# mbortolon97/6dgs

Hardware: AMD Instinct MI355X
Metric: poses/sec (higher is better)
Workload: dtype f32

## Files before the change

### 6dgs_amd/_lib.py

```python
from __future__ import annotations

import ctypes as C
import os

_HERE = os.path.dirname(os.path.abspath(__file__))
LIB_PATH = os.path.join(_HERE, "csrc", "lib6dgs_hip.so")
if os.environ.get("SIXDGS_LIB"):
    LIB_PATH = os.path.abspath(os.environ["SIXDGS_LIB"])

vp = C.c_void_p
i64 = C.c_int64
i32 = C.c_int
sz = C.c_size_t


PROFILE_SLOTS = 128
ABI_VERSION = 10


class Profile(C.Structure):
    _fields_ = [("count", i32), ("start", vp * PROFILE_SLOTS), ("stop", vp * PROFILE_SLOTS),
                ("flops", C.c_double * PROFILE_SLOTS), ("bytes", C.c_double * PROFILE_SLOTS)]


class ScorerWeights(C.Structure):
    _fields_ = [(n, vp) for n in ("w1", "b1", "w2", "b2", "w3", "b3", "w4", "b4", "wk", "bk", "wq", "bq", "m1", "m2", "m3", "m4", "mk", "w4k", "b4k", "m4k", "planes")]


SIGNATURES = {
    "sixdgs_abi_version": (i32, []),
    "sixdgs_error_string": (C.c_char_p, [i32]),
    "sixdgs_mask_degraded": (i32, [vp, i64, i32, vp, vp]),
    "sixdgs_sym_eig_3x3": (i32, [vp, i64, vp, vp, vp]),
    "sixdgs_normals_knn": (i32, [vp, i64, vp, i64, i32, vp, vp, vp]),
    "sixdgs_normals_knn_grid_workspace_bytes": (sz, [i64]),
    "sixdgs_normals_knn_grid": (i32, [vp, i64, vp, i64, i32, vp, vp, vp, sz, vp]),
    "sixdgs_emit_quadricell_count": (i32, [vp, vp, i32, vp, vp, i64, vp, i32, i32, vp, vp, vp, vp]),
    "sixdgs_emit_quadricell_write": (i32, [vp, vp, i32, vp, vp, vp, i32, i32, vp, i64, vp, i32, i32, vp, vp, vp, vp, vp, vp]),
    "sixdgs_quadricell_cell_counts": (i32, [vp, i64, i32, vp, vp, vp, vp]),
    "sixdgs_quadricell_centers": (i32, [vp, i64, i32, i32, vp, vp, vp, vp]),
    "sixdgs_isocell_distribution": (i32, [i32, i32, vp, C.POINTER(i64), vp]),
    "sixdgs_rotate_isocell": (i32, [vp, i64, vp, i64, vp, vp]),
    "sixdgs_emit_isocell": (i32, [vp, vp, i32, vp, vp, vp, i32, i32, vp, i64, vp, vp, i64, vp, vp, vp, vp, vp]),
    "sixdgs_eval_sh_color": (i32, [vp, i32, vp, i64, i32, vp, vp]),
    "sixdgs_splat_views_workspace_bytes": (sz, [i64, i32, i32, i32]),
    "sixdgs_splat_views": (i32, [vp, vp, i32, vp, vp, i32, i32, i64, vp, i32, i32, i32, i32, C.c_float, C.c_float, vp, vp, vp, vp, sz, vp]),
    "sixdgs_packed_weights_floats": (sz, []),
    "sixdgs_pack_weights": (i32, [vp] * 13 + [C.POINTER(ScorerWeights), vp]),
    "sixdgs_ray_encode": (i32, [vp, vp, vp, i64, vp, vp]),
    "sixdgs_ray_keys_workspace_bytes": (sz, [i64, i64]),
    "sixdgs_ray_keys": (i32, [vp, vp, vp, i64, C.POINTER(ScorerWeights), vp, vp, vp, sz, vp]),
    "sixdgs_ray_keys_ex": (i32, [vp, vp, vp, i64, C.POINTER(ScorerWeights), vp, vp, vp, vp, vp, vp, sz, vp, C.POINTER(Profile), i32]),
    "sixdgs_key_planes_f16_bytes": (sz, [i64]),
    "sixdgs_split_planes_f16": (i32, [vp, i64, i64, vp, vp, vp]),
    "sixdgs_score_pass1": (i32, [vp, vp, vp, i32, vp, vp, vp, i64, i32, vp, vp, sz, vp, C.POINTER(Profile), i32]),
    "sixdgs_score_pass2": (i32, [vp, vp, i32, i32, i64, i32, vp, vp, vp, vp, sz, vp, i32]),
    "sixdgs_score_backward_workspace_bytes": (sz, [i32]),
    "sixdgs_score_backward": (i32, [vp, vp, i32, vp, i64, vp, vp, vp, vp, vp, sz, vp]),
    "sixdgs_score_backward_split_workspace_bytes": (sz, [i32, i64, i32]),
    "sixdgs_score_backward_split": (i32, [vp, vp, i32, vp, i64, vp, vp, vp, vp, i32, vp, sz, vp]),
    "sixdgs_score_topk_ex": (i32, [vp, vp, vp, i32, vp, vp, vp, i64, i32, vp, vp, vp, vp, vp, sz, vp, C.POINTER(Profile), i32]),
    "sixdgs_score_select_workspace_bytes": (sz, [i64, i32, i32, i32]),
    "sixdgs_score_select": (i32, [vp, vp, vp, i32, vp, vp, vp, i64, vp, vp, i64, i32, i32, vp, vp, vp, vp, sz, vp, C.POINTER(Profile)]),
    "sixdgs_tok_attention": (i32, [vp, i64, i32, i32, i32, vp, i64, vp]),
    "sixdgs_im2col": (i32, [vp, i64, i64, i64, i64, i32, i32, i32, i32, i32, i32, vp, vp]),
    "sixdgs_u8_to_planar": (i32, [vp, i32, i64, vp, vp, vp]),
    "sixdgs_image_prep": (i32, [vp, i32, i32, i32, vp, i32, i32, i32, i32, i32, vp, vp, vp, vp]),
    "sixdgs_tok_pack_bytes": (sz, [i32, i32]),
    "sixdgs_tok_pack": (i32, [vp, i32, i32, i64, vp, vp, vp]),
    "sixdgs_tok_linear": (i32, [vp, i64, i32, i64, i32, vp, vp, C.c_float, vp, vp, vp, i32, i32, vp, i64, vp, vp, i64, vp]),
    "sixdgs_key_planes_norm_max": (i32, [vp, vp, i64, vp, vp]),
    "sixdgs_select_workspace_bytes": (sz, [i64, i32, i32, i32]),
    "sixdgs_select_candidates_workspace_bytes": (sz, [i64, i32, i32, i32]),
    "sixdgs_select_begin": (i32, [vp, vp, vp, i32, vp, vp, i64, i64, vp, vp, vp, sz, vp]),
    "sixdgs_select_sweep_plan": (i32, [vp, i32, vp, vp, i32]),
    "sixdgs_select_sweep": (i32, [vp, vp, vp, i32, vp, vp, i64, vp, vp, vp, i64, vp, vp, sz, vp, C.POINTER(Profile)]),
    "sixdgs_select_candidates": (i32, [vp, i64, i64, vp, vp, vp, i32, vp, vp, vp, i32, i32, vp, vp, vp, sz, vp]),
    "sixdgs_select_rescore": (i32, [vp, vp, i32, vp, vp, i32, vp, vp, vp, vp, i64, i32, i32, i32, vp, vp, vp, vp, sz, vp]),
    "sixdgs_select_sample_stats": (i32, [vp, vp, vp, i32, vp, vp, i64, vp, vp, sz, vp]),
    "sixdgs_select_prepare": (i32, [vp, vp, i32, i64, i64, vp, vp, vp]),
    "sixdgs_select_topk_u": (i32, [vp, i64, i64, vp, i32, i32, vp, vp, sz, vp]),
    "sixdgs_linear_splitk_workspace_bytes": (sz, [i64, i32, i32]),
    "sixdgs_linear_splitk": (i32, [vp, i64, i32, i64, vp, i64, vp, i32, i32, vp, i64, i32, vp, sz, vp, i32]),
    "sixdgs_linear_ex": (i32, [vp, i64, i32, i64, vp, i64, vp, i32, i32, vp, i64, vp, i32]),
    "sixdgs_profile_collect": (i32, [C.POINTER(Profile), C.POINTER(C.c_double), C.POINTER(C.c_double), C.POINTER(C.c_double),
                                    C.POINTER(i32)]),
    "sixdgs_linear": (i32, [vp, i64, i32, i64, vp, i64, vp, i32, i32, vp, i64, vp]),
    "sixdgs_q_proj": (i32, [vp, vp, i32, C.POINTER(ScorerWeights), vp, vp]),
    "sixdgs_score_topk_workspace_bytes": (sz, [i64, i32, i32]),
    "sixdgs_score_topk_workspace_bytes_ex": (sz, [i64, i32, i32, i32, i32]),
    "sixdgs_score_topk": (i32, [vp, vp, i32, vp, i64, i32, vp, vp, vp, vp, vp, sz, vp]),
    "sixdgs_topk_workspace_bytes": (sz, [i64, i32, i32]),
    "sixdgs_topk": (i32, [vp, i64, i32, i32, vp, vp, vp, sz, vp]),
    "sixdgs_distance_target_workspace_bytes": (sz, [i64]),
    "sixdgs_distance_target": (i32, [vp, vp, i64, vp, i32, vp, vp, vp, sz, vp]),
    "sixdgs_solve_pose": (i32, [vp, vp, i64, vp, vp, i32, vp, vp, i32, vp, vp, vp, vp, vp, vp, vp]),
    "sixdgs_solve_pose_consensus_workspace_bytes": (sz, [i32, i32]),
    "sixdgs_solve_pose_consensus": (i32, [vp, vp, i64, vp, vp, i32, vp, vp, i32, C.c_float, i32] + [vp] * 10 + [vp, sz, vp]),
}

_lib = None


def load():
    global _lib
    if _lib is not None:
        return _lib
    import torch

    if not os.path.exists(LIB_PATH):
        raise RuntimeError(
            f"6dgs_amd: {LIB_PATH} is missing -- build it with `python -m 6dgs_amd.build` / __graft_entry__.build(); "
            "there is no CPU fallback for the product path")
    try:
        lib = C.CDLL(LIB_PATH)
    except OSError as e:
        raise RuntimeError(f"6dgs_amd: cannot load {LIB_PATH}: {e}") from e
    for name, (res, args) in SIGNATURES.items():
        try:
            fn = getattr(lib, name)
        except AttributeError as e:
            raise RuntimeError(f"6dgs_amd: {LIB_PATH} does not export {name}") from e
        fn.restype = res
        fn.argtypes = args
    if lib.sixdgs_abi_version() != ABI_VERSION:
        raise RuntimeError(f"6dgs_amd: ABI version mismatch (library {lib.sixdgs_abi_version()}, binding {ABI_VERSION})")
    _lib = lib
    return lib


def check(status: int, what: str = ""):
    if status != 0:
        msg = load().sixdgs_error_string(int(status)).decode()
        raise RuntimeError(f"6dgs_amd: {what or 'call'} failed: {msg} (status {status})")
```

### 6dgs_amd/build.py

```python
from __future__ import annotations

import os
import subprocess
import sys

HERE = os.path.dirname(os.path.abspath(__file__))
CSRC = os.path.join(HERE, "csrc")
LIB = os.path.join(CSRC, "lib6dgs_hip.so")
HOSTCHECK = os.path.join(CSRC, "libsixdgs_hostcheck.so")
SOURCES = ["geometry.hip", "gemm.hip", "dense.hip", "score.hip", "score_bwd.hip", "pose.hip", "pose_consensus.hip", "vit.hip", "splat.hip"]
HEADERS = ["common.h", "device_math.h", "gemm_kernel.h", "dense.h", os.path.join("..", "..", "include", "sixdgs.h"), "dense_layout.h", "sweep_plan.h", "sweep_layout.h"]
HIPCC = os.environ.get("HIPCC", "/opt/rocm/bin/hipcc")
FLAGS = ["--offload-arch=gfx950", "-O3", "-std=c++17", "-fPIC", "-ffp-contract=off", "-Wall", "-Wno-unused-function"]
FLAGS += os.environ.get("SIXDGS_EXTRA_FLAGS", "").split()


def _stale(target, deps):
    if not os.path.exists(target):
        return True
    t = os.path.getmtime(target)
    return any(os.path.getmtime(d) > t for d in deps)


def build(force: bool = False, verbose: bool = False) -> str:
    deps = [os.path.join(CSRC, s) for s in SOURCES + HEADERS]
    if force or _stale(LIB, deps):
        objs = []
        procs = []
        for s in SOURCES:
            o = os.path.join(CSRC, s.replace(".hip", ".o"))
            objs.append(o)
            cmd = [HIPCC, *FLAGS, "-c", os.path.join(CSRC, s), "-o", o]
            if verbose:
                print(" ".join(cmd))
            procs.append((cmd, subprocess.Popen(cmd, stdout=subprocess.PIPE, stderr=subprocess.STDOUT, text=True)))
        for cmd, p in procs:
            out, _ = p.communicate()
            if p.returncode != 0:
                sys.stderr.write(out)
                raise RuntimeError("hipcc failed: " + " ".join(cmd))
            if verbose and out.strip():
                print(out)
        cmd = [HIPCC, "--offload-arch=gfx950", "-shared", "-fPIC", *objs, "-o", LIB]
        subprocess.check_call(cmd)
    return LIB


def build_hostcheck(force: bool = False) -> str:
    src = os.path.join(CSRC, "hostcheck.cpp")
    deps = [src, os.path.join(CSRC, "device_math.h"), os.path.join(CSRC, "dense_layout.h"), os.path.join(CSRC, "sweep_plan.h"),
            os.path.join(CSRC, "sweep_layout.h")]
    if force or _stale(HOSTCHECK, deps):
        cmd = [HIPCC, "-x", "hip", "--offload-arch=gfx950", "-O2", "-std=c++17", "-fPIC", "-ffp-contract=off", "-shared", src,
               "-o", HOSTCHECK]
        subprocess.check_call(cmd)
    return HOSTCHECK


if __name__ == "__main__":
    print(build(force="--force" in sys.argv, verbose=True))
    print(build_hostcheck(force="--force" in sys.argv))
```

### 6dgs_amd/csrc/hostcheck.cpp

```cpp
#include <stdlib.h>

#include "device_math.h"
#include "sweep_plan.h"
#include "dense_layout.h"
#include "sweep_layout.h"
using namespace sdg;

extern "C" {

void hc_mask_degraded(const float* scale, long long n, int P, unsigned char* mask) {
  for (long long i = 0; i < n; ++i) {
    float side;
    mask[i] = total_rings(scale[3 * i], scale[3 * i + 1], scale[3 * i + 2], (float)P, &side) < (long long)P;
  }
}

long long hc_quadricell_centers(const float* scale, long long E, int P, int res, float* points, long long* eid) {
  long long C = 0;
  float* table = (float*)malloc(sizeof(float) * res);
  for (long long e = 0; e < E; ++e) {
    float a = scale[3 * e], b = scale[3 * e + 1], c = scale[3 * e + 2], side;
    long long rings = total_rings(a, b, c, (float)P, &side);
    for (long long ring = 0; ring < rings; ++ring) {
      Ring rg = ring_params(a, b, c, side, (float)rings, (float)ring);
      int npts = ring_cells(rg);
      if (!npts) continue;
      if (points) {
        double acc = 0.0;
        table[0] = 0.f;
        for (int j = 0; j < res - 1; ++j) { acc += (double)ring_table_increment(rg, j); table[j + 1] = (float)acc; }
        float last = table[res - 1];
        for (int j = 0; j < res; ++j) table[j] = kTwoPi * (table[j] / last);
        for (int j = 0; j < npts; ++j) {
          int pick = ring_table_pick(table, res, (float)j * rg.dtheta);
          V3 p = ring_point(rg, table[pick]);
          points[3 * (C + j)] = p.x; points[3 * (C + j) + 1] = p.y; points[3 * (C + j) + 2] = p.z;
          eid[C + j] = e;
        }
      }
      C += npts;
    }
  }
  free(table);
  return C;
}

long long hc_emit_rays(const float* points, const long long* eid, long long C, const float* normals, const float* centers,
                       const float* rot4, float* ori, float* dir, long long* mid) {
  long long r = 0;
  for (long long i = 0; i < C; ++i) {
    long long e = eid[i];
    float R[9];
    quat_to_rotmat(rot4 + 4 * e, R);
    V3 pw = rotate(R, v3(points[3 * i], points[3 * i + 1], points[3 * i + 2]));
    if (!hemisphere_keep(normals[3 * e], pw)) continue;
    V3 d = normalize_eps(pw);
    ori[3 * r] = pw.x + centers[3 * e]; ori[3 * r + 1] = pw.y + centers[3 * e + 1]; ori[3 * r + 2] = pw.z + centers[3 * e + 2];
    dir[3 * r] = d.x; dir[3 * r + 1] = d.y; dir[3 * r + 2] = d.z;
    mid[r++] = e;
  }
  return r;
}

void hc_sym_eig(const float* mats, long long n, float* vals, float* vecs) {
  for (long long i = 0; i < n; ++i) sym_eig_3x3(mats + 9 * i, vals + 3 * i, vecs ? vecs + 9 * i : nullptr);
}

void hc_normals_from_knn(const float* cloud, const long long* knn, long long nq, int k, float* normals) {
  float* nb = (float*)malloc(sizeof(float) * 3 * k);
  for (long long q = 0; q < nq; ++q) {
    for (int j = 0; j < k; ++j)
      for (int c = 0; c < 3; ++c) nb[3 * j + c] = cloud[3 * knn[q * k + j] + c];
    V3 n = normal_from_neighbours(nb, k);
    normals[3 * q] = n.x; normals[3 * q + 1] = n.y; normals[3 * q + 2] = n.z;
  }
  free(nb);
}

long long hc_isocell_dirs(int target, int n0, float* dirs) {
  int n = isocell_rings(target, n0);
  long long o = 0;
  for (int ring = 1; ring <= n; ++ring)
    for (int j = 0; j < n0 * (2 * ring - 1); ++j, ++o)
      if (dirs) { V3 d = isocell_dir(n, n0, ring, j); dirs[3 * o] = d.x; dirs[3 * o + 1] = d.y; dirs[3 * o + 2] = d.z; }
  return o;
}

void hc_rotate_isocell(const float* dirs, long long K, const float* normals, long long E, float* out) {
  for (long long e = 0; e < E; ++e) {
    float Rm[9];
    isocell_rotation(v3(normals[3 * e], normals[3 * e + 1], normals[3 * e + 2]), Rm);
    for (long long k = 0; k < K; ++k) {
      V3 d = isocell_apply(Rm, v3(dirs[3 * k], dirs[3 * k + 1], dirs[3 * k + 2]));
      float* o = out + 3 * (e * K + k);
      o[0] = d.x; o[1] = d.y; o[2] = d.z;
    }
  }
}

void hc_sh_color(const float* sh, int ncoef, const float* dirs, long long R, int deg, float* rgb) {
  for (long long i = 0; i < R; ++i)
    for (int ch = 0; ch < 3; ++ch)
      rgb[3 * i + ch] = sh_channel(sh + (3 * i + ch) * ncoef, 1, deg, -dirs[3 * i], -dirs[3 * i + 1], -dirs[3 * i + 2]);
}

void hc_ray_input(const float* ori, const float* dir, const float* rgb, long long R, float* x) {
  for (long long i = 0; i < R; ++i)
    for (int c = 0; c < 144; ++c) x[144 * i + c] = ray_input_element(ori + 3 * i, dir + 3 * i, rgb + 3 * i, c);
}

void hc_make_rotation_mat(const float* d, const float* up, float* Rm) { make_rotation_mat(v3(d[0], d[1], d[2]), v3(up[0], up[1], up[2]), Rm); }

int hc_solve_centre(const float* Rm, const float* q, float* c) { return solve_centre(Rm, q, c) ? 1 : 0; }

void hc_pose_errors(const float* gt, const float* pr, float* out2) { pose_errors(gt, pr, out2, out2 + 1); }

void hc_distance_target(const float* pose, const float* ori, const float* dir, long long r, float* out) {
  for (long long i = 0; i < r; ++i)
    out[i] = distance_target(pose, v3(ori[3 * i], ori[3 * i + 1], ori[3 * i + 2]), v3(dir[3 * i], dir[3 * i + 1], dir[3 * i + 2]));
}

int hc_dl_row_perm(int m) { return dl::row_perm(m); }
int hc_dl_acc_row(int lane, int r) { return dl::acc_row(lane, r); }
int hc_dl_acc_feature(int permuted, int lane, int r) { return dl::acc_feature(permuted != 0, lane, r); }
long long hc_dl_plane_offset(int chunk_major, long long ray, int nslab, int slab, int plane, int c) {
  return chunk_major ? dl::cm_offset(ray, nslab, slab, plane, c) : dl::rm_offset(ray, nslab, slab, plane, c);
}
unsigned hc_dl_lds_offset(unsigned row, unsigned plane, unsigned c) { return dl::lds_offset(row, plane, c); }
unsigned hc_dl_frag_offset(unsigned row0, unsigned lane, unsigned ks, unsigned plane) { return dl::frag_offset(row0, lane, ks, plane); }
unsigned hc_dl_load_ray(int chunk_major, unsigned tid, unsigned jp) { return dl::load_ray(chunk_major != 0, tid, jp); }
unsigned hc_dl_load_chunk8(int chunk_major, unsigned tid) { return dl::load_chunk8(chunk_major != 0, tid); }
unsigned hc_dl_cm_src_offset(unsigned ray_in_tile, unsigned chunk8, unsigned granule_stride) {
  return dl::cm_src_offset(ray_in_tile, chunk8 * (unsigned)dl::kChunkRun, granule_stride);
}
int hc_sweep_launch_images(int left, int cap) { return sdg::sweep_launch_images(left, cap); }
int hc_sweep_pack_ints() { return 2 + 2 * sdg::kSweepMaxSlots * sdg::kSlotQuarters + (2 + sdg::kSlotQuarters) * sdg::kSweepMaxLaunchImages; }
int hc_sweep_max_slots() { return sdg::kSweepMaxSlots; }
int hc_sweep_pack(const int* h_n_tok, int batch, int cap, int* out, int max_launches) {
  const std::vector<sdg::SweepSlots> plan = sdg::sweep_pack(h_n_tok, batch, cap);
  const int per = hc_sweep_pack_ints();
  for (size_t l = 0; l < plan.size() && (int)l < max_launches; ++l) {
    const sdg::SweepSlots& t = plan[l];
    int* o = out + (size_t)l * per;
    *o++ = t.n_slots;
    *o++ = t.n_images;
    for (int s = 0; s < sdg::kSweepMaxSlots; ++s)
      for (int w = 0; w < sdg::kSlotQuarters; ++w) *o++ = t.q_img[s][w];
    for (int s = 0; s < sdg::kSweepMaxSlots; ++s)
      for (int w = 0; w < sdg::kSlotQuarters; ++w) *o++ = t.q_lq[s][w];
    for (int i = 0; i < sdg::kSweepMaxLaunchImages; ++i) *o++ = t.img[i];
    for (int i = 0; i < sdg::kSweepMaxLaunchImages; ++i) *o++ = t.img_nq[i];
    for (int i = 0; i < sdg::kSweepMaxLaunchImages; ++i)
      for (int w = 0; w < sdg::kSlotQuarters; ++w) *o++ = t.img_q[i][w];
  }
  return (int)plan.size();
}
int hc_sw_const(int which) {
  const int v[] = {sw::kTokBlocks, sw::kRayBlocks, sw::kBlockBytes, sw::kBflySteps};
  return which >= 0 && which < 4 ? v[which] : -1;
}
int hc_sw_frag_row(int lane) { return sw::frag_row(lane); }
int hc_sw_frag_chunk(int lane, int plane) { return sw::frag_chunk(lane, plane); }
unsigned hc_sw_frag_offset(int row0, int lane, int plane) { return sw::frag_offset(row0, lane, plane); }
int hc_sw_acc_token(int lane, int tb) { return sw::acc_token(lane, tb); }
int hc_sw_acc_ray(int lane, int rb, int reg) { return sw::acc_ray(lane, rb, reg); }
int hc_sw_bfly_partner(int lane, int step) { return sw::bfly_partner(lane, step); }
int hc_sw_bfly_keeps(int lane, int step, int i) { return sw::bfly_keeps(lane, step, i) ? 1 : 0; }
int hc_sw_out_index(int lane, int x) { return sw::out_index(lane, x); }
int hc_sw_out_ray(int lane, int x) { return sw::out_ray(lane, x); }
int hc_sw_part_writes(int lane) { return sw::part_writes(lane) ? 1 : 0; }
int hc_sw_part_row(int wn, int lane) { return sw::part_row(wn, lane); }
int hc_dl_const(int which) {
  const int v[] = {dl::kSlabB, dl::kPRow, dl::kGran, dl::kGranSlab, dl::kChunkRun};
  return which >= 0 && which < 5 ? v[which] : -1;
}

}
```

### 6dgs_amd/csrc/score.hip

```cpp
#include <stdlib.h>

#include <cstdlib>
#include <cstdio>
#include "gemm_kernel.h"
#include "sweep_plan.h"
#include "sweep_layout.h"

using namespace sdg;

namespace {

constexpr int kT = SIXDGS_MAX_TOKENS;
constexpr float kSqrtD = 19.595917942265423f;

struct LogitsArgs {
  const float* q;
  const int* n_tok;
  const float* key;
  float* logits;
  float* partial;
  int64_t r, ldl;
  int tiles_per_group, n_tiles, n_groups;
  int b0;
};

template <int MMA>
__global__ void __launch_bounds__(256, 2) k_logits(LogitsArgs A) {
  __shared__ __attribute__((aligned(16))) char smem[TileSmem<MMA>::kBytes];
  __shared__ float part[2][128][2];
  const int bl = blockIdx.y;
  const int b = A.b0 + bl;
  const unsigned w = xcd_remap(blockIdx.x, gridDim.x);
  const int grp = (int)(w >> 1), m_tile = (int)(w & 1u);
  const int M = A.n_tok[b];
  const int row0 = m_tile * 128;
  float* pout = A.partial + (((int64_t)bl * A.n_groups + grp) * kT + row0) * 2;
  const int tid = threadIdx.x, lane = tid & 63, wave = tid >> 6;
  const int wm = wave >> 1, wn = wave & 1;
  float m_run = -INFINITY, s_run = 0.f;
  if (row0 < M) {
    GemmOperands g = {A.q + (int64_t)b * kT * SIXDGS_D, nullptr, A.key, SIXDGS_D, 0, SIXDGS_D, M, A.r, SIXDGS_D, SIXDGS_D};
    float* lg = A.logits + (int64_t)bl * kT * A.ldl;
    const int t_begin = grp * A.tiles_per_group;
    const int t_end = min(t_begin + A.tiles_per_group, A.n_tiles);
    for (int tile = t_begin; tile < t_end; ++tile) {
      const int64_t col0 = (int64_t)tile * kBN;
      f32x16 acc[2][2];
      gemm_tile<MMA>(g, row0, col0, smem, acc);
      const int64_t c0 = col0 + acc_col(wn, 0, lane), c1 = col0 + acc_col(wn, 1, lane);
      const bool v0 = c0 < A.r, v1 = c1 < A.r;
#pragma unroll
      for (int tm = 0; tm < 2; ++tm)
#pragma unroll
        for (int r = 0; r < 16; ++r) {
          const int row = row0 + acc_row(wm, tm, r, lane);
          const float l0 = acc[tm][0][r] / kSqrtD, l1 = acc[tm][1][r] / kSqrtD;
          if (row < M) {
            if (v0) lg[(int64_t)row * A.ldl + c0] = l0;
            if (v1) lg[(int64_t)row * A.ldl + c1] = l1;
          }
          float mx = fmaxf(v0 ? l0 : -INFINITY, v1 ? l1 : -INFINITY);
#pragma unroll
          for (int o = 16; o > 0; o >>= 1) mx = fmaxf(mx, __shfl_xor(mx, o, 64));
          float sm = 0.f;
          if (mx > -INFINITY) sm = (v0 ? expf(l0 - mx) : 0.f) + (v1 ? expf(l1 - mx) : 0.f);
#pragma unroll
          for (int o = 16; o > 0; o >>= 1) sm += __shfl_xor(sm, o, 64);
          if ((lane & 31) == 0) {
            const int lr = acc_row(wm, tm, r, lane);
            part[wn][lr][0] = mx;
            part[wn][lr][1] = sm;
          }
        }
      __syncthreads();
      if (tid < 128) {
#pragma unroll
        for (int h = 0; h < 2; ++h) {
          const float mt = part[h][tid][0], st = part[h][tid][1];
          if (mt > -INFINITY) {
            const float mn = fmaxf(m_run, mt);
            s_run = s_run * expf(m_run - mn) + st * expf(mt - mn);
            m_run = mn;
          }
        }
      }
    }
  }
  if (tid < 128) {
    pout[2 * tid] = m_run;
    pout[2 * tid + 1] = s_run;
  }
}

typedef __attribute__((address_space(3))) void* lds_ptr_t;
typedef const __attribute__((address_space(1))) void* gbl_ptr_t;
constexpr int kRowBytes = 12 * 3 * 64;
constexpr float kInvSqrtD = 0.05103103630798288f;

typedef _Float16 f16x8 __attribute__((ext_vector_type(8)));
constexpr int kRowF = 12 * 2 * 64;
constexpr int kSlabF = 128;

struct LogitsF16Args {
  const char* qp;
  const int* n_tok;
  const char* kp;
  const float* qinv;
  const float* kinv;
  float* logits;
  float* partial;
  int64_t r, ldl;
  int tiles_per_group, n_tiles, n_groups, b0, nb;
  const float* ctok;
  float* ub;
  int64_t ub_stride;
  int n_sets;
  unsigned* sib_sync;
  int sib_period;
  unsigned sib_extra;
  int q_quarter_scales;
};
constexpr int kOutF32 = 0;
constexpr int kOutL24 = 1;
constexpr int kOutStats = 2;
constexpr int kOutUB = 3;
constexpr int kAllTerms = 3;
constexpr int kOneTerm = 1;

__device__ __forceinline__ float load_uniform(const float* p) {
  return *reinterpret_cast<const __attribute__((address_space(4))) float*>((uintptr_t)p);
}

__device__ __forceinline__ f16x8 lds_read_frag_h_off(unsigned addr, const int imm) {
  f16x8 v;
  asm volatile("ds_read_b128 %0, %1 offset:%2" : "=v"(v) : "v"(addr), "n"(imm));
  return v;
}

constexpr int kBNX = 256;
constexpr int kSiblingSyncDefault = 1;
constexpr int kSibSpinLimit = 1 << 14;
constexpr unsigned kSibReleased = 0x40000000u;
constexpr int kSweepMaxImages = 8;
constexpr bool kPrepassOneTermDefault = true;
constexpr int kPrepassReserveCusOneSlot = 160;
constexpr int kPrepassReserveCus = 64;
constexpr int kSibPeriod = 1;
constexpr int kTileBytes24 = 98304 + 2048;
constexpr int kQStageX = 256 * 64;
constexpr int kKBaseX = 4 * kQStageX;
constexpr int kLdsX = kKBaseX + 6 * kQStageX;

constexpr int kMfma32 = 0;
constexpr int kMfma16 = 1;

template <int TERMS, int OUT, bool PERS = false, int SHAPE = kMfma32>
__global__ void __launch_bounds__(512, 1) k_logits_f16x(LogitsF16Args A) {
  static_assert(TERMS == kAllTerms || TERMS == kOneTerm, "k_logits_f16x: TERMS is 3 or 1");
  static_assert(SHAPE == kMfma32 || (SHAPE == kMfma16 && OUT == kOutUB && TERMS == kAllTerms), "k_logits_f16x: 16x16x32 is the select sweep's shape");
// ... 412 lines not shown
              const f32x2 uu = e0 + e1;
              u[r] = uu.x;
              u[r + 1] = uu.y;
            }
            float v8[8], v4[4], v2[2];
#pragma unroll
            for (int i = 0; i < 8; ++i) {
              const float keep = lb0 ? u[i + 8] : u[i], send = lb0 ? u[i] : u[i + 8];
              v8[i] = keep + __builtin_bit_cast(float, __builtin_amdgcn_mov_dpp(__builtin_bit_cast(int, send), 0xB1, 0xF, 0xF, true));
            }
#pragma unroll
            for (int i = 0; i < 4; ++i) {
              const float keep = lb1 ? v8[i + 4] : v8[i], send = lb1 ? v8[i] : v8[i + 4];
              v4[i] = keep + __builtin_bit_cast(float, __builtin_amdgcn_mov_dpp(__builtin_bit_cast(int, send), 0x4E, 0xF, 0xF, true));
            }
#pragma unroll
            for (int i = 0; i < 2; ++i) {
              const float keep = lb2 ? v4[i + 2] : v4[i], send = lb2 ? v4[i] : v4[i + 2];
              v2[i] = keep + __builtin_bit_cast(float, __builtin_amdgcn_ds_swizzle(__builtin_bit_cast(int, send), 0x101F));
            }
            {
              const float keep = lb3 ? v2[1] : v2[0], send = lb3 ? v2[0] : v2[1];
              fin[tn] = keep + __builtin_bit_cast(float, __builtin_amdgcn_ds_swizzle(__builtin_bit_cast(int, send), 0x201F));
            }
          }
          float o[2];
#pragma unroll
          for (int x = 0; x < 2; ++x) {
            const float keep = lb4 ? fin[2 + x] : fin[x], send = lb4 ? fin[x] : fin[2 + x];
            o[x] = keep + __builtin_bit_cast(float, __builtin_amdgcn_ds_swizzle(__builtin_bit_cast(int, send), 0x401F));
          }
          const int rrev = ((lane & 1) << 3) | ((lane & 2) << 1) | ((lane & 4) >> 1) | ((lane & 8) >> 3);
          const int inhalf = ((lane & 16) << 2) + 8 * (rrev >> 2) + 4 * (lane >> 5) + (rrev & 3);
          float* up = A.ub + ((int64_t)bl * 4 + wm) * A.ub_stride + ((int64_t)tile * kBNX + wn * 128 + inhalf);
          __builtin_nontemporal_store(o[0], up);
          __builtin_nontemporal_store(o[1], up + 32);
        }
      } else if (active) {
        const int t128 = min(2 * tile + wn, n_tiles128 - 1);
        const float cf = (cq * load_uniform(A.kinv + t128)) * kInvSqrtD;
        float* tb = lg + (int64_t)(2 * tile + wn) * (kT * 128);
        const bool ragged = lim_cur < kBNX - 1;
#pragma unroll
        for (int tm = 0; tm < 2; ++tm) {
          float mx = -INFINITY;
#pragma unroll
          for (int tn = 0; tn < 4; ++tn)
#pragma unroll
            for (int rg = 0; rg < 4; ++rg) {
              float4 v;
              v.x = acc[tm][tn][4 * rg + 0] * cf;
              v.y = acc[tm][tn][4 * rg + 1] * cf;
              v.z = acc[tm][tn][4 * rg + 2] * cf;
              v.w = acc[tm][tn][4 * rg + 3] * cf;
              acc[tm][tn][4 * rg + 0] = v.x;
              acc[tm][tn][4 * rg + 1] = v.y;
              acc[tm][tn][4 * rg + 2] = v.z;
              acc[tm][tn][4 * rg + 3] = v.w;
              if (OUT == kOutF32) {
                typedef float f32x4 __attribute__((ext_vector_type(4)));
                __builtin_nontemporal_store(f32x4{v.x, v.y, v.z, v.w}, reinterpret_cast<f32x4*>(tb + tm * 4096 + tn * 1024 + rg * 256));
              }
              mx = fmaxf(mx, fmaxf(fmaxf(v.x, v.y), fmaxf(v.z, v.w)));
            }
          if (L24) {
            typedef unsigned u32x3 __attribute__((ext_vector_type(3)));
            char* t24 = lg24 + (int64_t)(2 * tile + wn) * kTileBytes24 + ((wm * 2 + tm) * 12288 + lane * 12);
#pragma unroll
            for (int tn = 0; tn < 4; ++tn)
#pragma unroll
              for (int rg = 0; rg < 4; ++rg) {
                unsigned d[4];
#pragma unroll
                for (int j = 0; j < 4; ++j)
                  d[j] = (unsigned)__float2uint_rn(fminf((mx - acc[tm][tn][4 * rg + j]) * 524288.f, 16777215.f));
                const u32x3 w3 = {d[0] | (d[1] << 24), (d[1] >> 8) | (d[2] << 16), (d[2] >> 16) | (d[3] << 8)};
                __builtin_nontemporal_store(w3, reinterpret_cast<u32x3*>(t24 + (tn * 8 + 2 * rg) * 384));
                __builtin_amdgcn_sched_barrier(0);
              }
            reinterpret_cast<float*>(lg24 + (int64_t)(2 * tile + wn) * kTileBytes24 + 98304)[((wm * 2 + tm) * 2 + (lane >> 5)) * 32 + (lane & 31)] = mx;
          }
          const float mn = fmaxf(m_run[tm], mx);
          float sum[4] = {0.f, 0.f, 0.f, 0.f};
          if (!ragged) {
#pragma unroll
            for (int tn = 0; tn < 4; ++tn)
#pragma unroll
              for (int r = 0; r < 16; ++r) sum[r & 3] += __expf(acc[tm][tn][r] - mn);
          } else {
            int ray0 = wn * 128 + 4 * (lane >> 5);
            asm volatile("" : "+v"(ray0));
#pragma unroll
            for (int tn = 0; tn < 4; ++tn)
#pragma unroll
              for (int r = 0; r < 16; ++r)
                sum[r & 3] += (ray0 + tn * 32 + 8 * (r >> 2) + (r & 3) <= lim_cur) ? __expf(acc[tm][tn][r] - mn) : 0.f;
          }
          s_run[tm] = s_run[tm] * __expf(m_run[tm] - mn) + ((sum[0] + sum[1]) + (sum[2] + sum[3]));
          m_run[tm] = mn;
        }
      }
      kcur = knext;
      lim_cur = lim_next;
    }
    asm volatile("s_waitcnt vmcnt(0)" ::: "memory");
  }
  __syncthreads();
  float(*part)[256][2] = reinterpret_cast<float(*)[256][2]>(lds);
  if (S16) {
    int lm = lane;
    if (PERS) asm volatile("" : "+v"(lm));
#pragma unroll
    for (int tb = 0; tb < sw::kTokBlocks; ++tb) {
      float z = zs16[tb];
      z += __builtin_bit_cast(float, __builtin_amdgcn_ds_swizzle(__builtin_bit_cast(int, z), 0x401F));
      if (sw::part_writes(lm)) {
        float* pp = part[sw::part_row(wn, lm)][wm * 64 + sw::acc_token(lm, tb)];
        pp[0] = 0.f;
        pp[1] = z;
      }
    }
  } else {
#pragma unroll
  for (int tm = 0; tm < 2; ++tm) {
    float* pp = part[wn * 2 + (lane >> 5)][wm * 64 + tm * 32 + (lane & 31)];
    if (OUT == kOutUB) {
      pp[0] = 0.f;
      pp[1] = (zs[tm][0].x + zs[tm][0].y) + (zs[tm][1].x + zs[tm][1].y);
    } else {
      pp[0] = m_run[tm];
      pp[1] = s_run[tm];
    }
  }
  }
  __syncthreads();
  if (tid < 256) {
    float m = -INFINITY, sres = 0.f;
#pragma unroll
    for (int h = 0; h < 4; ++h) {
      const float mt = part[h][tid][0], st2 = part[h][tid][1];
      if (mt > -INFINITY) {
        const float mn = fmaxf(m, mt);
        sres = sres * __expf(m - mn) + st2 * __expf(mt - mn);
        m = mn;
      }
    }
    pout[2 * tid] = m;
    pout[2 * tid + 1] = sres;
  }
  if (PERS) __syncthreads();
  } while (PERS && (grp += A.n_sets) < A.n_groups);
}

__global__ void __launch_bounds__(256) k_split_tiles_f16(const float* __restrict__ src, int64_t rows, int64_t ld, char* __restrict__ dst,
                                                         float* __restrict__ inv_scale) {
  __shared__ float wmax[4];
  const int64_t row0 = (int64_t)blockIdx.x * 128;
  const int n = (int)min((int64_t)128, rows - row0);
  const float* base = src + row0 * ld;
  float m = 0.f;
  for (int i = threadIdx.x; i < n * 96; i += 256) {
    const int row = i / 96;
    const float4 v = *reinterpret_cast<const float4*>(base + (int64_t)row * ld + (i - row * 96) * 4);
    m = fmaxf(m, fmaxf(fmaxf(fabsf(v.x), fabsf(v.y)), fmaxf(fabsf(v.z), fabsf(v.w))));
  }
  m = sdg_wave_max(m);
  if (sdg_lane() == 0) wmax[sdg_wave()] = m;
  __syncthreads();
  m = fmaxf(fmaxf(wmax[0], wmax[1]), fmaxf(wmax[2], wmax[3]));
  int sh = 0;
  if (m > 0.f && m < INFINITY) {
    int e;
    frexpf(m, &e);
    sh = 14 - e;
    sh = sh > 100 ? 100 : (sh < -100 ? -100 : sh);
  }
  const float sc = ldexpf(1.f, sh);
  if (threadIdx.x == 0) inv_scale[blockIdx.x] = ldexpf(1.f, -sh);
  for (int i = threadIdx.x; i < n * 48; i += 256) {
    const int row = i / 48, k8 = i - row * 48;
    const float* sp = base + (int64_t)row * ld + k8 * 8;
    const float4 lo = *reinterpret_cast<const float4*>(sp);
    const float4 hi = *reinterpret_cast<const float4*>(sp + 4);
    const float x[8] = {lo.x * sc, lo.y * sc, lo.z * sc, lo.w * sc, hi.x * sc, hi.y * sc, hi.z * sc, hi.w * sc};
    f16x8 h, l;
#pragma unroll
    for (int e = 0; e < 8; ++e) {
      const _Float16 hh = (_Float16)x[e];
      h[e] = hh;
      l[e] = (_Float16)(x[e] - (float)hh);
    }
    char* d = dst + (row0 + row) * kRowF + (k8 >> 2) * kSlabF + (k8 & 3) * 16;
    *reinterpret_cast<f16x8*>(d) = h;
    *reinterpret_cast<f16x8*>(d + 64) = l;
  }
}


__global__ void __launch_bounds__(1024) k_merge_stats(const float* __restrict__ partial, int n_groups, float* __restrict__ stats) {
  __shared__ float sm[16][64][2];
  const int bl = blockIdx.x, tl = threadIdx.x & 63, j = threadIdx.x >> 6, t = blockIdx.y * 64 + tl;
  const float* p = partial + (int64_t)bl * n_groups * kT * 2;
  float m = -INFINITY, s = 0.f;
  for (int g = j; g < n_groups; g += 16) {
    const float mt = p[((int64_t)g * kT + t) * 2], st = p[((int64_t)g * kT + t) * 2 + 1];
    if (mt > -INFINITY) {
      const float mn = fmaxf(m, mt);
      s = s * expf(m - mn) + st * expf(mt - mn);
      m = mn;
    }
  }
  sm[j][tl][0] = m;
  sm[j][tl][1] = s;
  __syncthreads();
  if (j == 0) {
    m = -INFINITY;
    s = 0.f;
#pragma unroll
    for (int q = 0; q < 16; ++q) {
      const float mt = sm[q][tl][0], st = sm[q][tl][1];
      if (mt > -INFINITY) {
        const float mn = fmaxf(m, mt);
        s = s * expf(m - mn) + st * expf(mt - mn);
        m = mn;
      }
    }
    stats[((int64_t)bl * kT + t) * 2] = m;
    stats[((int64_t)bl * kT + t) * 2 + 1] = s;
  }
}

__global__ void __launch_bounds__(256) k_score_reduce(const float* __restrict__ logits, int64_t ldl, const float* __restrict__ stats,
                                                       const int* __restrict__ n_tok, int b0, int64_t R, float* __restrict__ scores,
                                                       int64_t score_stride) {
  __shared__ float st[kT][2];
  const int bl = blockIdx.y;
  const int T = n_tok[b0 + bl];
  for (int i = threadIdx.x; i < kT * 2; i += blockDim.x) {
    const float v = stats[(int64_t)bl * kT * 2 + i];
    (&st[0][0])[i] = (i & 1) ? 1.f / v : v;
  }
  __syncthreads();
  const int64_t j = (int64_t)blockIdx.x * blockDim.x + threadIdx.x;
  if (j >= R) return;
  const float* l = logits + (int64_t)bl * kT * ldl + j;
  float s = 0.f;
#pragma unroll 8
  for (int t = 0; t < T; ++t) s += __expf(l[(int64_t)t * ldl] - st[t][0]) * st[t][1];
  scores[(int64_t)bl * score_stride + j] = s;
}

#define FASTEXP(x) __expf(x)
__global__ void __launch_bounds__(256) k_score_reduce_blocked(const float* __restrict__ logits, int64_t ldl, const float* __restrict__ stats,
                                                               const int* __restrict__ n_tok, int b0, int64_t R,
                                                               float* __restrict__ scores, int64_t score_stride) {
  const int bl = blockIdx.y;
  const int T = n_tok[b0 + bl];
  const int lane = threadIdx.x & 63, wave = threadIdx.x >> 6, l31 = lane & 31;
  float mt[8], st[8];
#pragma unroll
  for (int g = 0; g < 8; ++g) {
    const int t = g * 32 + l31;
    mt[g] = stats[((int64_t)bl * kT + t) * 2];
    st[g] = 1.f / stats[((int64_t)bl * kT + t) * 2 + 1];
  }
  const int64_t tile = blockIdx.x;
  const float* tb = logits + (int64_t)bl * kT * ldl + tile * (kT * kBN) + lane * 4;
  float* out = scores + (int64_t)bl * score_stride + tile * kBN;
#pragma unroll
  for (int u = 0; u < 4; ++u) {
    const int p = u * 4 + wave;
    float4 acc = {0.f, 0.f, 0.f, 0.f};
#pragma unroll
    for (int g = 0; g < 8; ++g)
      if (g * 32 + l31 < T) {
        const float4 v = *reinterpret_cast<const float4*>(tb + g * 4096 + p * 256);
        acc.x += FASTEXP(v.x - mt[g]) * st[g];
        acc.y += FASTEXP(v.y - mt[g]) * st[g];
        acc.z += FASTEXP(v.z - mt[g]) * st[g];
        acc.w += FASTEXP(v.w - mt[g]) * st[g];
      }
#pragma unroll
    for (int o = 16; o > 0; o >>= 1) {
      acc.x += __shfl_xor(acc.x, o, 64);
      acc.y += __shfl_xor(acc.y, o, 64);
      acc.z += __shfl_xor(acc.z, o, 64);
      acc.w += __shfl_xor(acc.w, o, 64);
    }
    if (l31 == 0) {
      const int64_t r0 = tile * kBN + p * 8 + (lane >> 5) * 4;
      float* o4 = out + p * 8 + (lane >> 5) * 4;
      if (r0 + 3 < R && ((uintptr_t)o4 & 15) == 0) *reinterpret_cast<float4*>(o4) = acc;
      else {
        if (r0 < R) o4[0] = acc.x;
        if (r0 + 1 < R) o4[1] = acc.y;
        if (r0 + 2 < R) o4[2] = acc.z;
        if (r0 + 3 < R) o4[3] = acc.w;
      }
    }
  }
}

__global__ void __launch_bounds__(256) k_score_reduce_blocked24(const float* __restrict__ logits, int64_t ldl, const float* __restrict__ stats,
                                                               const int* __restrict__ n_tok, int b0, int64_t R,
                                                               float* __restrict__ scores, int64_t score_stride) {
  const int bl = blockIdx.y;
// ... 67 lines not shown
  unsigned remain;
};
__device__ SelectState select_state(const unsigned* hist , int passes, unsigned k, unsigned* sm ) {
  SelectState st = {0u, k};
  for (int p = 0; p < passes; ++p) {
    __syncthreads();
    for (int i = threadIdx.x; i < 256; i += blockDim.x) sm[i] = hist[p * 256 + i];
    __syncthreads();
    unsigned acc = 0, digit = 0, rem = st.remain;
    for (int d = 255; d >= 0; --d) {
      const unsigned c = sm[d];
      if (acc + c >= st.remain) { digit = (unsigned)d; rem = st.remain - acc; break; }
      acc += c;
    }
    st.prefix |= digit << (24 - 8 * p);
    st.remain = rem;
  }
  return st;
}

template <int PASS>
__global__ void __launch_bounds__(256) k_topk_hist(const float* __restrict__ scores, int64_t stride, int64_t R, unsigned k,
                                                    unsigned* __restrict__ hist_all, const int* __restrict__ only) {
  __shared__ unsigned sm[256];
  __shared__ unsigned lh[256];
  const int b = blockIdx.y;
  if (only != nullptr && only[b] == 0) return;
  unsigned* hist = hist_all + (int64_t)b * 4 * 256;
  const SelectState st = select_state(hist, PASS, k, sm);
  for (int i = threadIdx.x; i < 256; i += blockDim.x) lh[i] = 0;
  __syncthreads();
  const float* s = scores + (int64_t)b * stride;
  constexpr unsigned hi_mask = PASS == 0 ? 0u : (0xffffffffu << (32 - 8 * PASS));
  constexpr int shift = 24 - 8 * PASS;
  for (int64_t i = (int64_t)blockIdx.x * blockDim.x + threadIdx.x; i < R; i += (int64_t)gridDim.x * blockDim.x) {
    const unsigned key = score_key(s[i]);
    if ((key & hi_mask) == st.prefix) atomicAdd(&lh[(key >> shift) & 255u], 1u);
  }
  __syncthreads();
  for (int i = threadIdx.x; i < 256; i += blockDim.x)
    if (lh[i]) atomicAdd(&hist[PASS * 256 + i], lh[i]);
}

template <bool WRITE>
__global__ void __launch_bounds__(256) k_topk_gather(const float* __restrict__ scores, int64_t stride, int64_t R, unsigned k,
                                                      const unsigned* __restrict__ hist_all, int64_t span,
                                                      unsigned* __restrict__ counts ,
                                                      const unsigned* __restrict__ offs ,
                                                      unsigned* __restrict__ cand_key, int64_t* __restrict__ cand_idx, int topk,
                                                      const int* __restrict__ only) {
  __shared__ unsigned sm[256];
  __shared__ int sc[2][5];
  const int b = blockIdx.y;
  if (only != nullptr && only[b] == 0) return;
  const SelectState st = select_state(hist_all + (int64_t)b * 4 * 256, 4, k, sm);
  const unsigned thr = st.prefix;
  const float* s = scores + (int64_t)b * stride;
  const int64_t i0 = (int64_t)blockIdx.x * span, i1 = min(i0 + span, R);
  unsigned run_g = 0, run_e = 0;
  unsigned base_g = 0, base_e = 0, n_greater = 0;
  if (WRITE) {
    base_g = offs[((int64_t)b * gridDim.x + blockIdx.x) * 2];
    base_e = offs[((int64_t)b * gridDim.x + blockIdx.x) * 2 + 1];
    n_greater = k - st.remain;
  }
  for (int64_t c0 = i0; c0 < i1; c0 += 256) {
    const int64_t i = c0 + threadIdx.x;
    unsigned key = 0;
    bool gt = false, eq = false;
    if (i < i1) {
      key = score_key(s[i]);
      gt = key > thr;
      eq = key == thr;
    }
    const unsigned long long bg = __ballot(gt), be = __ballot(eq);
    const int lane = sdg_lane(), wv = sdg_wave();
    if (lane == 0) { sc[0][wv] = __popcll(bg); sc[1][wv] = __popcll(be); }
    __syncthreads();
    unsigned og = 0, oe = 0, tg = 0, te = 0;
    for (int w2 = 0; w2 < 4; ++w2) {
      if (w2 < wv) { og += sc[0][w2]; oe += sc[1][w2]; }
      tg += sc[0][w2];
      te += sc[1][w2];
    }
    __syncthreads();
    if (WRITE) {
      const unsigned long long below = (1ull << lane) - 1ull;
      if (gt) {
        const unsigned pos = base_g + run_g + og + __popcll(bg & below);
        if (pos < (unsigned)topk) { cand_key[(int64_t)b * topk + pos] = key; cand_idx[(int64_t)b * topk + pos] = i; }
      } else if (eq) {
        const unsigned re = base_e + run_e + oe + __popcll(be & below);
        if (re < st.remain) {
          const unsigned pos = n_greater + re;
          if (pos < (unsigned)topk) { cand_key[(int64_t)b * topk + pos] = key; cand_idx[(int64_t)b * topk + pos] = i; }
        }
      }
    }
    run_g += tg;
    run_e += te;
  }
  if (!WRITE && threadIdx.x == 0) {
    counts[((int64_t)b * gridDim.x + blockIdx.x) * 2] = run_g;
    counts[((int64_t)b * gridDim.x + blockIdx.x) * 2 + 1] = run_e;
  }
}

__global__ void __launch_bounds__(1024) k_topk_scan(const unsigned* __restrict__ counts, int nb, unsigned* __restrict__ offs, const int* __restrict__ only) {
  __shared__ unsigned sm[17];
  const int b = blockIdx.x;
  if (only != nullptr && only[b] == 0) return;
  for (int comp = 0; comp < 2; ++comp) {
    unsigned base = 0;
    for (int c0 = 0; c0 < nb; c0 += 1024) {
      const int i = c0 + threadIdx.x;
      const unsigned v = i < nb ? counts[((int64_t)b * nb + i) * 2 + comp] : 0u;
      unsigned tot;
      const unsigned ex = sdg_block_exclusive_scan<unsigned, 16>(v, sm, &tot);
      if (i < nb) offs[((int64_t)b * nb + i) * 2 + comp] = base + ex;
      base += tot;
    }
  }
}

__global__ void __launch_bounds__(1024) k_topk_sort(const unsigned* __restrict__ cand_key, const int64_t* __restrict__ cand_idx,
                                                     int topk, int k_eff, int64_t* __restrict__ idx, float* __restrict__ val, const int* __restrict__ only) {
  __shared__ unsigned sk[1024];
  __shared__ long long si[1024];
  const int b = blockIdx.x, t = threadIdx.x;
  if (only != nullptr && only[b] == 0) return;
  if (t < k_eff) { sk[t] = cand_key[(int64_t)b * topk + t]; si[t] = cand_idx[(int64_t)b * topk + t]; }
  else { sk[t] = 0u; si[t] = 0x7fffffffffffffffll; }
  __syncthreads();
  for (int size = 2; size <= 1024; size <<= 1)
    for (int strd = size >> 1; strd > 0; strd >>= 1) {
      const int p = t ^ strd;
      if (p > t) {
        const bool up = (t & size) == 0;
        const unsigned ka = sk[t], kb = sk[p];
        const long long ia = si[t], ib = si[p];
        const bool a_first = ka > kb || (ka == kb && ia < ib);
        if (up ? !a_first : a_first) { sk[t] = kb; sk[p] = ka; si[t] = ib; si[p] = ia; }
      }
      __syncthreads();
    }
  if (t < topk) {
    if (t < k_eff) { idx[(int64_t)b * topk + t] = si[t]; val[(int64_t)b * topk + t] = key_score(sk[t]); }
    else { idx[(int64_t)b * topk + t] = -1; val[(int64_t)b * topk + t] = NAN; }
  }
}

constexpr float kLog2e = 1.4426950408889634f;

__global__ void __launch_bounds__(kT) k_sel_prepare(const float* __restrict__ stats_s, const int* __restrict__ n_tok, int b0, float log2_frac,
                                                    float* __restrict__ ctok) {
  const int bl = blockIdx.x, t = threadIdx.x;
  const float m = stats_s[((int64_t)bl * kT + t) * 2], z = stats_s[((int64_t)bl * kT + t) * 2 + 1];
  const bool ok = t < n_tok[b0 + bl] && z > 0.f && m > -INFINITY && m < INFINITY;
  ctok[(int64_t)bl * kT + t] = ok ? -(m * kLog2e) - (log2f(z) + log2_frac) : -INFINITY;
}

__global__ void __launch_bounds__(256) k_split_q_slots(const float* __restrict__ q, const int* __restrict__ n_tok, const SweepSlots T, char* __restrict__ dst,
                                                       float* __restrict__ inv_scale, const float* __restrict__ ctok, float* __restrict__ ctok_slot,
                                                       int* __restrict__ slot_rows) {
  __shared__ float wmax[4];
  const int slot = blockIdx.x >> 2, w = blockIdx.x & 3;
  const int img = T.q_img[slot][w], lq = T.q_lq[slot][w];
  const int n = img < 0 ? 0 : min(64, max(0, n_tok[img] - 64 * lq));
  const float* base = q + ((int64_t)(img < 0 ? 0 : img) * kT + 64 * (lq < 0 ? 0 : lq)) * SIXDGS_D;
  float m = 0.f;
  for (int i = threadIdx.x; i < n * 96; i += 256) {
    const float4 v = *reinterpret_cast<const float4*>(base + (int64_t)i * 4);
    m = fmaxf(m, fmaxf(fmaxf(fabsf(v.x), fabsf(v.y)), fmaxf(fabsf(v.z), fabsf(v.w))));
  }
  m = sdg_wave_max(m);
  if (sdg_lane() == 0) wmax[sdg_wave()] = m;
  __syncthreads();
  m = fmaxf(fmaxf(wmax[0], wmax[1]), fmaxf(wmax[2], wmax[3]));
  int sh = 0;
  if (m > 0.f && m < INFINITY) {
    int e;
    frexpf(m, &e);
    sh = 14 - e;
    sh = sh > 100 ? 100 : (sh < -100 ? -100 : sh);
  }
  const float sc = ldexpf(1.f, sh);
  if (threadIdx.x == 0) inv_scale[blockIdx.x] = ldexpf(1.f, -sh);
  char* const drow = dst + ((int64_t)slot * kT + 64 * w) * kRowF;
  for (int i = threadIdx.x; i < 64 * 48; i += 256) {
    const int row = i / 48, k8 = i - row * 48;
    f16x8 h, l;
    if (row < n) {
      const float* sp = base + (int64_t)row * SIXDGS_D + k8 * 8;
      const float4 lo = *reinterpret_cast<const float4*>(sp);
      const float4 hi = *reinterpret_cast<const float4*>(sp + 4);
      const float x[8] = {lo.x * sc, lo.y * sc, lo.z * sc, lo.w * sc, hi.x * sc, hi.y * sc, hi.z * sc, hi.w * sc};
#pragma unroll
      for (int e = 0; e < 8; ++e) {
        const _Float16 hh = (_Float16)x[e];
        h[e] = hh;
        l[e] = (_Float16)(x[e] - (float)hh);
      }
    } else {
#pragma unroll
      for (int e = 0; e < 8; ++e) h[e] = l[e] = (_Float16)0.f;
    }
    char* d = drow + (int64_t)row * kRowF + (k8 >> 2) * kSlabF + (k8 & 3) * 16;
    *reinterpret_cast<f16x8*>(d) = h;
    *reinterpret_cast<f16x8*>(d + 64) = l;
  }
  if (ctok_slot != nullptr && threadIdx.x < 64) {
    const int t = threadIdx.x;
    ctok_slot[(int64_t)slot * kT + 64 * w + t] = t < n ? ctok[(int64_t)img * kT + 64 * lq + t] : -INFINITY;
  }
  if (w == 0 && threadIdx.x == 0) {
    int rows = 0;
    for (int x = 0; x < kSlotQuarters; ++x) {
      const int im = T.q_img[slot][x];
      const int nx = im < 0 ? 0 : min(64, max(0, n_tok[im] - 64 * T.q_lq[slot][x]));
      if (nx > 0) rows = 64 * x + nx;
    }
    slot_rows[slot] = rows;
  }
}

__global__ void __launch_bounds__(1024) k_merge_stats_slots(const float* __restrict__ partial, int n_groups, const SweepSlots T, float* __restrict__ stats,
                                                            float* __restrict__ gsum) {
  __shared__ float sm[16][64][2];
  const int k = blockIdx.x, y = blockIdx.y, tl = threadIdx.x & 63, j = threadIdx.x >> 6;
  const int img = T.img[k], sq = y < T.img_nq[k] ? T.img_q[k][y] : -1;
  float m = -INFINITY, s = 0.f;
  if (sq >= 0) {
    const float* p = partial + (int64_t)(sq >> 2) * n_groups * kT * 2;
    const int row = 64 * (sq & 3) + tl;
    for (int g = j; g < n_groups; g += 16) {
      const float mt = p[((int64_t)g * kT + row) * 2], st = p[((int64_t)g * kT + row) * 2 + 1];
      if (mt > -INFINITY) {
        const float mn = fmaxf(m, mt);
        s = s * expf(m - mn) + st * expf(mt - mn);
        m = mn;
      }
    }
  }
  sm[j][tl][0] = m;
  sm[j][tl][1] = s;
  __syncthreads();
  if (j == 0) {
    m = -INFINITY;
    s = 0.f;
#pragma unroll
    for (int qd = 0; qd < 16; ++qd) {
      const float mt = sm[qd][tl][0], st = sm[qd][tl][1];
      if (mt > -INFINITY) {
        const float mn = fmaxf(m, mt);
        s = s * expf(m - mn) + st * expf(mt - mn);
        m = mn;
      }
    }
    const int64_t o = (int64_t)img * kT + 64 * y + tl;
    if (gsum != nullptr) {
      gsum[o] += s;
    } else {
      stats[o * 2] = m;
      stats[o * 2 + 1] = s;
    }
  }
}

__global__ void __launch_bounds__(256) k_sel_finish_slots(const float* __restrict__ ub, int64_t stride, int64_t u_stride, const int* __restrict__ n_tok, const SweepSlots T,
                                                          int64_t R, float* __restrict__ U, float* __restrict__ tmax, int64_t tmax_stride) {
  const int k = blockIdx.y, img = T.img[k];
  const int nq_dev = (min(max(n_tok[img], 0), kT) + 63) >> 6;
  const int nq = min(nq_dev, (int)T.img_nq[k]);
  const int64_t i = ((int64_t)blockIdx.x * blockDim.x + threadIdx.x) * 4;
  float m = -INFINITY;
  if (i < R) {
    float4 a = {0.f, 0.f, 0.f, 0.f};
    const int64_t row[kSlotQuarters] = {T.img_q[k][0], T.img_q[k][1], T.img_q[k][2], T.img_q[k][3]};
#pragma unroll
    for (int y = 0; y < kSlotQuarters; ++y)
      if (y < nq) {
        const float4 v = *reinterpret_cast<const float4*>(ub + row[y] * stride + i);
        a.x += v.x; a.y += v.y; a.z += v.z; a.w += v.w;
      }
    *reinterpret_cast<float4*>(U + (int64_t)img * u_stride + i) = a;
    m = a.x;
    if (i + 1 < R) m = fmaxf(m, a.y);
    if (i + 2 < R) m = fmaxf(m, a.z);
    if (i + 3 < R) m = fmaxf(m, a.w);
  }
  if (tmax != nullptr) {
    m = sdg_wave_max(m);
    const int64_t tile = (i - 4 * sdg_lane()) >> 8;
    if (sdg_lane() == 0 && tile * 256 < R) tmax[(int64_t)img * tmax_stride + tile] = m;
  }
}

__global__ void __launch_bounds__(256) k_plane_norm_max(const char* __restrict__ planes, const float* __restrict__ inv_scale, int64_t rows,
                                                        unsigned* __restrict__ out) {
  const int lane = sdg_lane();
  const int64_t wave0 = (int64_t)blockIdx.x * 4 + sdg_wave(), nw = (int64_t)gridDim.x * 4;
  float best = 0.f;
  for (int64_t row = wave0; row < rows; row += nw) {
    float ss = 0.f;
    if (lane < 48) {
      const char* p = planes + row * kRowF + (lane >> 2) * kSlabF + (lane & 3) * 16;
      const f16x8 h = *reinterpret_cast<const f16x8*>(p), l = *reinterpret_cast<const f16x8*>(p + 64);
#pragma unroll
      for (int e = 0; e < 8; ++e) {
        const float x = (float)h[e] + (float)l[e];
        ss = __builtin_fmaf(x, x, ss);
      }
    }
    ss = sdg_wave_sum(ss);
    best = fmaxf(best, sqrtf(ss) * inv_scale[row >> 7]);
  }
  if (lane == 0 && best > 0.f) atomicMax(out, __float_as_uint(best * 1.000244140625f));
}

constexpr float kEpsPerX = 1.4e-4f, kEpsConst = 1.3e-5f;
__global__ void __launch_bounds__(kT) k_sel_bounds(const float* __restrict__ gsum, const int* __restrict__ n_tok, const float* __restrict__ valU,
                                                   const float* __restrict__ q, const float* __restrict__ key_norm_max, int topk, int k_eff,
                                                   float* __restrict__ info, const int* __restrict__ only) {
  __shared__ float smin[4], smax[4], sq[4];
  const int bl = blockIdx.x, t = threadIdx.x, M = n_tok[bl];
  if (only != nullptr && only[bl] == 0) return;
  const float g = gsum[(int64_t)bl * kT + t];
  float lo = t < M ? g : INFINITY, hi = t < M ? g : -INFINITY;
  bool bad = t < M && !(g > 0.f && g < INFINITY);
  float qn = 0.f;
  if (t < M) {
    const float4* qr = reinterpret_cast<const float4*>(q + ((int64_t)bl * kT + t) * SIXDGS_D);
    float ss = 0.f;
    for (int i = 0; i < SIXDGS_D / 4; ++i) {
      const float4 v = qr[i];
      ss = __builtin_fmaf(v.x, v.x, ss); ss = __builtin_fmaf(v.y, v.y, ss); ss = __builtin_fmaf(v.z, v.z, ss); ss = __builtin_fmaf(v.w, v.w, ss);
    }
    qn = sqrtf(ss) * 1.000244140625f;
  }
#pragma unroll
  for (int o = 32; o > 0; o >>= 1) {
    lo = fminf(lo, __shfl_xor(lo, o, 64));
    hi = fmaxf(hi, __shfl_xor(hi, o, 64));
    qn = fmaxf(qn, __shfl_xor(qn, o, 64));
  }
  const unsigned long long anybad = __ballot(bad);
  if (sdg_lane() == 0) { smin[sdg_wave()] = anybad ? NAN : lo; smax[sdg_wave()] = hi; sq[sdg_wave()] = qn; }
  __syncthreads();
  if (t == 0) {
    float flag = 0.f, thr = INFINITY, eps = 0.f, x = 0.f;
    if (M <= 0) flag = 1.f;
    else {
      float a = smin[0], b = smax[0], qm = sq[0];
      bool nan = a != a;
      for (int w = 1; w < 4; ++w) { nan = nan || smin[w] != smin[w]; a = fminf(a, smin[w]); b = fmaxf(b, smax[w]); qm = fmaxf(qm, sq[w]); }
      const float uk = valU[(int64_t)bl * topk + (k_eff - 1)];
      x = qm * key_norm_max[0] * kInvSqrtD * 1.0000002f;
      eps = x * kEpsPerX + kEpsConst;
      if (nan || !(uk >= 0.f && uk < INFINITY) || !(a > 0.f) || !(eps < 0.25f)) flag = 2.f;
      else thr = (uk * (a / b)) * ((1.f - eps) / (1.f + eps)) * 0.9999998f;
    }
    info[bl * 4 + 0] = thr;
    info[bl * 4 + 1] = flag;
    info[bl * 4 + 2] = eps;
    info[bl * 4 + 3] = x;
  }
}

__global__ void k_sel_need_exact(const int* __restrict__ total, const float* __restrict__ info, int nb, int cmax, int* __restrict__ need) {
  const int bl = blockIdx.x * blockDim.x + threadIdx.x;
  if (bl >= nb) return;
  need[bl] = (info[bl * 4 + 1] == 0.f && total[bl] > cmax) ? 1 : 0;
}

__global__ void k_sel_count(const int* __restrict__ total, const float* __restrict__ info, int nb, int* __restrict__ d_count) {
  const int bl = blockIdx.x * blockDim.x + threadIdx.x;
  if (bl >= nb) return;
  const float flag = info[bl * 4 + 1];
  d_count[bl] = flag == 1.f ? -2 : (flag != 0.f ? -1 : total[bl]);
}

template <bool WRITE>
__global__ void __launch_bounds__(256) k_sel_candidates(const float* __restrict__ U, int64_t stride, int64_t R, const float* __restrict__ info,
                                                        int64_t span, unsigned* __restrict__ counts, const unsigned* __restrict__ offs,
                                                        int64_t* __restrict__ cand, int cmax, const int* __restrict__ only,
                                                        const float* __restrict__ tmax_all) {
  __shared__ int sc[4];
  const int bl = blockIdx.y;
  if (only != nullptr && only[bl] == 0) return;
  const float thr = info[bl * 4 + 0];
  const float* u = U + (int64_t)bl * stride;
  const float* tmax = tmax_all ? tmax_all + (int64_t)bl * (stride >> 8) : nullptr;
  const int64_t i0 = (int64_t)blockIdx.x * span, i1 = min(i0 + span, R);
  unsigned run = 0;
  const unsigned base = WRITE ? offs[(int64_t)bl * gridDim.x + blockIdx.x] : 0u;
  for (int64_t c0 = i0; c0 < i1; c0 += 256) {
    if (tmax != nullptr && !(tmax[c0 >> 8] >= thr)) continue;
    const int64_t i = c0 + threadIdx.x;
    const bool in = i < i1 && u[i] >= thr;
    const unsigned long long bm = __ballot(in);
    const int lane = sdg_lane(), wv = sdg_wave();
    if (lane == 0) sc[wv] = __popcll(bm);
    __syncthreads();
    unsigned before = 0, tot = 0;
    for (int w2 = 0; w2 < 4; ++w2) {
      if (w2 < wv) before += sc[w2];
      tot += sc[w2];
    }
    __syncthreads();
    if (WRITE && in) {
      const unsigned pos = base + run + before + __popcll(bm & ((1ull << lane) - 1ull));
      if (pos < (unsigned)cmax) cand[(int64_t)bl * cmax + pos] = i;
    }
    run += tot;
  }
  if (!WRITE && threadIdx.x == 0) counts[(int64_t)bl * gridDim.x + blockIdx.x] = run;
}
// ... 539 lines not shown
  }
  prof->count = 0;
  if (ms_total) *ms_total = ms;
  if (flops_total) *flops_total = fl;
  if (bytes_total) *bytes_total = by;
  if (launches) *launches = n;
  return rc;
}

}

namespace {
struct SelectPlan {
  int64_t stride;
  int nbc;
  int64_t span;
  size_t o_partial, o_stats, o_qpl, o_ub, o_idxu, o_valu, o_lidx, o_lval, o_info, o_counts, o_offs, o_total, o_cscore, o_slot, per_image, topk_bytes;
};
SelectPlan select_plan(int64_t r, int batch, int topk, int cmax, bool with_ub = true) {
  SelectPlan p;
  p.stride = sdg_cdiv(r > 0 ? r : 1, 256) * 256;
  const TopkPlan tp = topk_plan(r, batch, topk);
  p.nbc = tp.nb;
  p.span = tp.span;
  size_t o = 0;
  auto take = [&](size_t bytes) { const size_t at = o; o += sdg_align(bytes); return at; };
  p.o_partial = take((size_t)1024 * kT * 2 * sizeof(float));
  p.o_stats = take((size_t)kT * 2 * sizeof(float));
  p.o_qpl = take(sdg_align((size_t)kT * kRowF, 1024) + 256);
  p.o_ub = take(with_ub ? (size_t)4 * p.stride * sizeof(float) : 16);
  p.o_idxu = take((size_t)topk * sizeof(int64_t));
  p.o_valu = take((size_t)topk * sizeof(float));
  p.o_lidx = take((size_t)topk * sizeof(int64_t));
  p.o_lval = take((size_t)topk * sizeof(float));
  p.o_info = take(16);
  p.o_counts = take((size_t)p.nbc * sizeof(unsigned));
  p.o_offs = take((size_t)p.nbc * sizeof(unsigned));
  p.o_total = take(16);
  p.o_cscore = take((size_t)cmax * sizeof(float));
  p.o_slot = take((size_t)kT * sizeof(float) + 256);
  p.per_image = o;
  const size_t t2 = topk_plan(cmax, batch, topk).bytes;
  p.topk_bytes = tp.bytes > t2 ? tp.bytes : t2;
  return p;
}
struct SelectWs {
  SelectPlan p;
  char *topk_ws, *qplanes;
  float *partial, *stats, *qinv, *ub, *valU, *lval, *info, *cscore, *ctok_slot;
  int* slot_rows;
  int64_t *idxU, *lidx;
  unsigned *counts, *offs;
  int* total;
  size_t qpl_img;
};
bool select_ws(void* ws, size_t ws_bytes, int64_t r, int nb, int topk, int cmax, SelectWs* w, bool with_ub = true) {
  w->p = select_plan(r, nb, topk, cmax, with_ub);
  if (w->p.topk_bytes + (size_t)nb * w->p.per_image > ws_bytes) return false;
  w->topk_ws = (char*)ws;
  char* img0 = (char*)ws + w->p.topk_bytes;
  auto field = [&](size_t off) { return img0 + off * (size_t)nb; };
  w->partial = (float*)field(w->p.o_partial);
  w->stats = (float*)field(w->p.o_stats);
  w->qplanes = field(w->p.o_qpl);
  w->qpl_img = sdg_align((size_t)kT * kRowF, 1024);
  w->qinv = (float*)(w->qplanes + (size_t)nb * w->qpl_img);
  w->ub = (float*)field(w->p.o_ub);
  w->idxU = (int64_t*)field(w->p.o_idxu);
  w->valU = (float*)field(w->p.o_valu);
  w->lidx = (int64_t*)field(w->p.o_lidx);
  w->lval = (float*)field(w->p.o_lval);
  w->info = (float*)field(w->p.o_info);
  w->counts = (unsigned*)field(w->p.o_counts);
  w->offs = (unsigned*)field(w->p.o_offs);
  w->total = (int*)field(w->p.o_total);
  w->cscore = (float*)field(w->p.o_cscore);
  w->ctok_slot = (float*)field(w->p.o_slot);
  w->slot_rows = (int*)(field(w->p.o_slot) + (size_t)nb * kT * sizeof(float));
  return true;
}

int f16x_groups(int64_t r) {
  const int n_tiles_x = (int)sdg_cdiv(r > 0 ? r : 1, kBNX);
  int g = 1024;
  while (g > 256 && n_tiles_x / g < 16) g -= 256;
  if (g > n_tiles_x) g = n_tiles_x;
  return g;
}

int sibling_sync_mode() {
  static int mode = -1;
  if (mode < 0) {
    const char* e = getenv("SIXDGS_SIBLING_SYNC");
    mode = e ? atoi(e) : kSiblingSyncDefault;
  }
  return mode;
}
bool sweep_mfma16() {
  const char* e = getenv("SIXDGS_SWEEP_MFMA");
  return !(e && atoi(e) == 32);
}
int sibling_sync_cus() {
  static int cus = -1;
  if (cus < 0) {
    const bool on = sibling_sync_mode() != 0;
    int dev = 0;
    hipDeviceProp_t prop;
    cus = (on && hipGetDevice(&dev) == hipSuccess && hipGetDeviceProperties(&prop, dev) == hipSuccess && prop.multiProcessorCount > 0) ? prop.multiProcessorCount : 0;
  }
  return cus;
}

void select_q_planes(const float* q, int nb, const SelectWs& w, hipStream_t s) {
  hipLaunchKernelGGL(k_split_tiles_f16, dim3((unsigned)(2 * nb)), dim3(256), 0, s, q, (int64_t)nb * kT, (int64_t)SIXDGS_D, w.qplanes, w.qinv);
}
LogitsF16Args select_args(const int32_t* d_n_tok, int nb, const SelectWs& w, const void* planes, const float* scale, int64_t r) {
  LogitsF16Args V = {w.qplanes, d_n_tok, (const char*)planes, w.qinv, scale, nullptr, w.partial, r, w.p.stride, 0, 0, 0, 0, nb, nullptr, nullptr, 0};
  V.n_tiles = (int)sdg_cdiv(r, kBNX);
  V.n_groups = f16x_groups(r);
  V.tiles_per_group = (int)sdg_cdiv(V.n_tiles, V.n_groups);
  return V;
}
}

extern "C" {

size_t sixdgs_select_workspace_bytes(int64_t r, int batch, int topk, int max_candidates) {
  if (batch < 1) batch = 1;
  const SelectPlan p = select_plan(r, batch, topk, max_candidates);
  return p.topk_bytes + (size_t)batch * p.per_image;
}

size_t sixdgs_select_candidates_workspace_bytes(int64_t r, int batch, int topk, int max_candidates) {
  if (batch < 1) batch = 1;
  const SelectPlan p = select_plan(r, batch, topk, max_candidates, false);
  return p.topk_bytes + (size_t)batch * p.per_image;
}

static int sweep_slot_cap() {
  static const int cap = [] {
    const char* e = getenv("SIXDGS_SWEEP_MAX_IMAGES");
    const int v = e ? atoi(e) : kSweepMaxImages;
    if (e && v <= 0) fprintf(stderr, "6dgs_amd: SIXDGS_SWEEP_MAX_IMAGES=%s: launches of %d slots (the slot table's limit), a last one of up to %d -- not one launch per batch\n", e, kSweepMaxSlots * 2 / 3, kSweepMaxSlots * 2 / 3 + kSweepMaxSlots / 3);
    return v;
  }();
  return cap;
}

static bool prepass_one_term(int ) {
  static const int forced = [] { const char* e = getenv("SIXDGS_PREPASS_TERMS"); return e ? atoi(e) : 0; }();
  return forced == 1 || (forced != 3 && kPrepassOneTermDefault);
}

int sixdgs_select_sweep_plan(const int32_t* h_n_tok, int batch, int32_t* slots_per_launch, int32_t* images_per_launch, int max_launches) {
  if (batch < 0 || batch > 32767 || max_launches < 0 || (max_launches > 0 && (!slots_per_launch || !images_per_launch))) return SIXDGS_E_BADARG;
  const std::vector<SweepSlots> plan = sweep_pack(h_n_tok, batch, sweep_slot_cap());
  for (size_t l = 0; l < plan.size() && (int)l < max_launches; ++l) {
    slots_per_launch[l] = plan[l].n_slots;
    images_per_launch[l] = plan[l].n_images;
  }
  return (int)plan.size();
}

int sixdgs_select_sample_stats(const float* q, const int32_t* d_n_tok, const int32_t* h_n_tok, int batch, const void* sample_planes,
                               const float* d_sample_scale, int64_t r_sample, float* row_stats, void* ws, size_t ws_bytes, sixdgs_stream_t stream) {
  SDG_CHECK_ARG(batch >= 0 && batch <= 32767 && r_sample >= 1);
  if (batch == 0) return 0;
  SDG_CHECK_ARG(q && d_n_tok && sample_planes && d_sample_scale && row_stats && ws && ((uintptr_t)sample_planes % 16) == 0 &&
                ((uintptr_t)q % 16) == 0 && ((uintptr_t)ws % 256) == 0);
  hipStream_t s = sdg_stream(stream);
  SelectWs w;
  if (!select_ws(ws, ws_bytes, r_sample, batch, 1, 8, &w)) return SIXDGS_E_WORKSPACE;
  const int n_groups = f16x_groups(r_sample);
  for (const SweepSlots& T : sweep_pack(h_n_tok, batch, sweep_slot_cap())) {
    if (T.n_slots > 0) {
      hipLaunchKernelGGL(k_split_q_slots, dim3((unsigned)(4 * T.n_slots)), dim3(256), 0, s, q, d_n_tok, T, w.qplanes, w.qinv, (const float*)nullptr,
                         (float*)nullptr, w.slot_rows);
      LogitsF16Args V = select_args(w.slot_rows, T.n_slots, w, sample_planes, d_sample_scale, r_sample);
      V.q_quarter_scales = 1;
      static const int reserve_env = [] { const char* e = getenv("SIXDGS_PREPASS_RESERVE_CUS"); return e ? atoi(e) : -2; }();
      const int reserve = reserve_env != -2 ? reserve_env : (T.n_slots == 1 ? kPrepassReserveCusOneSlot : kPrepassReserveCus);
      const int cus = sibling_sync_cus();
      if (reserve >= 0 && cus > reserve && (cus - reserve) / T.n_slots >= 1) {
        V.n_sets = (cus - reserve) / T.n_slots < V.n_groups ? (cus - reserve) / T.n_slots : V.n_groups;
        V.sib_sync = nullptr;
        V.sib_extra = 0u;
        V.sib_period = kSibPeriod;
        if (prepass_one_term(T.n_slots)) hipLaunchKernelGGL((k_logits_f16x<kOneTerm, kOutStats, true>), dim3((unsigned)(V.n_sets * T.n_slots)), dim3(512), 0, s, V);
        else hipLaunchKernelGGL((k_logits_f16x<kAllTerms, kOutStats, true>), dim3((unsigned)(V.n_sets * T.n_slots)), dim3(512), 0, s, V);
      } else {
        if (prepass_one_term(T.n_slots)) hipLaunchKernelGGL((k_logits_f16x<kOneTerm, kOutStats>), dim3((unsigned)(V.n_groups * T.n_slots)), dim3(512), 0, s, V);
        else hipLaunchKernelGGL((k_logits_f16x<kAllTerms, kOutStats>), dim3((unsigned)(V.n_groups * T.n_slots)), dim3(512), 0, s, V);
      }
    }
    hipLaunchKernelGGL(k_merge_stats_slots, dim3((unsigned)T.n_images, 4), dim3(1024), 0, s, w.partial, n_groups, T, row_stats, (float*)nullptr);
  }
  SDG_LAUNCH_OK();
  return 0;
}

int sixdgs_select_prepare(const float* row_stats, const int32_t* d_n_tok, int batch, int64_t r_sample, int64_t r_total, float* ctok, float* gsum,
                          sixdgs_stream_t stream) {
  SDG_CHECK_ARG(batch >= 0 && r_sample >= 1 && r_total >= r_sample);
  if (batch == 0) return 0;
  SDG_CHECK_ARG(row_stats && d_n_tok && ctok && gsum);
  hipStream_t s = sdg_stream(stream);
  hipLaunchKernelGGL(k_sel_prepare, dim3((unsigned)batch), dim3(kT), 0, s, row_stats, d_n_tok, 0, log2f((float)((double)r_total / (double)r_sample)), ctok);
  hipError_t e = hipMemsetAsync(gsum, 0, (size_t)batch * kT * sizeof(float), s);
  if (e != hipSuccess) return (int)e;
  SDG_LAUNCH_OK();
  return 0;
}

int sixdgs_select_begin(const float* q, const int32_t* d_n_tok, const int32_t* h_n_tok, int batch, const void* sample_planes, const float* d_sample_scale,
                        int64_t r_sample, int64_t r_total, float* ctok, float* gsum, void* ws, size_t ws_bytes, sixdgs_stream_t stream) {
  SDG_CHECK_ARG(batch >= 0 && r_sample >= 1 && r_total >= r_sample);
  if (batch == 0) return 0;
  SDG_CHECK_ARG(ws && ((uintptr_t)ws % 256) == 0);
  SelectWs w;
  if (!select_ws(ws, ws_bytes, r_sample, batch, 1, 8, &w)) return SIXDGS_E_WORKSPACE;
  const int st = sixdgs_select_sample_stats(q, d_n_tok, h_n_tok, batch, sample_planes, d_sample_scale, r_sample, w.stats, ws, ws_bytes, stream);
  if (st) return st;
  return sixdgs_select_prepare(w.stats, d_n_tok, batch, r_sample, r_total, ctok, gsum, stream);
}

int sixdgs_select_sweep(const float* q, const int32_t* d_n_tok, const int32_t* h_n_tok, int batch, const void* key_planes,
                        const float* d_key_scale, int64_t r, const float* ctok, float* gsum, float* u, int64_t u_stride, float* u_tile_max,
                        void* ws, size_t ws_bytes, sixdgs_stream_t stream, sixdgs_profile* prof) {
  SDG_CHECK_ARG(batch >= 0 && batch <= 32767 && r >= 1 && u_stride >= sdg_cdiv(r, 256) * 256 && (u_stride % 4) == 0 && (!u_tile_max || (u_stride % 256) == 0));
  if (batch == 0) return 0;
  SDG_CHECK_ARG(q && d_n_tok && key_planes && d_key_scale && ctok && gsum && u && ws && ((uintptr_t)key_planes % 16) == 0 &&
                ((uintptr_t)q % 16) == 0 && ((uintptr_t)u % 16) == 0 && ((uintptr_t)ws % 256) == 0);
  hipStream_t s = sdg_stream(stream);
  SelectWs w;
  if (!select_ws(ws, ws_bytes, r, batch, 1, 8, &w)) return SIXDGS_E_WORKSPACE;
  const int n_groups = f16x_groups(r);
  for (const SweepSlots& T : sweep_pack(h_n_tok, batch, sweep_slot_cap())) {
    const int ns = T.n_slots;
    double tok = 0.0;
    for (int k = 0; k < T.n_images; ++k) tok += h_n_tok ? (double)(h_n_tok[T.img[k]] < 0 ? 0 : (h_n_tok[T.img[k]] > kT ? kT : h_n_tok[T.img[k]])) : (double)kT;
    if (ns > 0) {
      hipLaunchKernelGGL(k_split_q_slots, dim3((unsigned)(4 * ns)), dim3(256), 0, s, q, d_n_tok, T, w.qplanes, w.qinv, ctok, w.ctok_slot, w.slot_rows);
      LogitsF16Args V = select_args(w.slot_rows, ns, w, key_planes, d_key_scale, r);
      V.q_quarter_scales = 1;
      V.ctok = w.ctok_slot;
      V.ub = w.ub;
      V.ub_stride = w.p.stride;
      unsigned grid = (unsigned)(V.n_groups * ns);
      const int cus = sibling_sync_cus();
      if (cus > 0 && ns >= 2 && cus / ns >= 1 && (cus % ns) * 16 <= cus && w.p.topk_bytes >= (size_t)(cus / ns) * sizeof(unsigned)) {
        V.n_sets = cus / ns < V.n_groups ? cus / ns : V.n_groups;
        V.sib_sync = sibling_sync_mode() == 2 ? nullptr : reinterpret_cast<unsigned*>(w.topk_ws);
        V.sib_extra = sibling_sync_mode() == 3 ? 1u : 0u;
        V.sib_period = kSibPeriod;
        if (V.sib_sync && hipMemsetAsync(V.sib_sync, 0, (size_t)V.n_sets * sizeof(unsigned), s) != hipSuccess) return (int)hipGetLastError();
        grid = (unsigned)(V.n_sets * ns);
      }
      SdgProfileScope scope(prof, s, 2.0 * tok * SIXDGS_D * (double)r, (double)r * (kRowF + T.n_images * 16.0));
      auto kern = sweep_mfma16() ? (V.n_sets > 0 ? k_logits_f16x<kAllTerms, kOutUB, true, kMfma16> : k_logits_f16x<kAllTerms, kOutUB, false, kMfma16>)
                                 : (V.n_sets > 0 ? k_logits_f16x<kAllTerms, kOutUB, true> : k_logits_f16x<kAllTerms, kOutUB, false>);
      hipLaunchKernelGGL(kern, dim3(grid), dim3(512), 0, s, V);
    }
    hipLaunchKernelGGL(k_merge_stats_slots, dim3((unsigned)T.n_images, 4), dim3(1024), 0, s, w.partial, n_groups, T, (float*)nullptr, gsum);
    hipLaunchKernelGGL(k_sel_finish_slots, dim3((unsigned)sdg_cdiv(r, 1024), (unsigned)T.n_images), dim3(256), 0, s, w.ub, w.p.stride, u_stride, d_n_tok, T, r, u,
                       u_tile_max, u_stride / 256);
  }
  SDG_LAUNCH_OK();
  return 0;
}

int sixdgs_key_planes_norm_max(const void* planes, const float* d_scale, int64_t rows, float* d_norm_max, sixdgs_stream_t stream) {
  SDG_CHECK_ARG(rows >= 0);
  if (rows == 0) return 0;
  SDG_CHECK_ARG(planes && d_scale && d_norm_max && ((uintptr_t)planes % 16) == 0);
  const int64_t blocks = sdg_cdiv(rows, 4);
  hipLaunchKernelGGL(k_plane_norm_max, dim3((unsigned)(blocks < 8192 ? blocks : 8192)), dim3(256), 0, sdg_stream(stream), (const char*)planes, d_scale,
                     rows, reinterpret_cast<unsigned*>(d_norm_max));
  SDG_LAUNCH_OK();
  return 0;
}

int sixdgs_select_topk_u(const float* u, int64_t u_stride, int64_t r, const float* u_tile_max, int batch, int topk, float* val, void* ws,
                         size_t ws_bytes, sixdgs_stream_t stream) {
  SDG_CHECK_ARG(batch >= 0 && r >= 1 && u_stride >= r && topk >= 1 && topk <= 1024);
  if (batch == 0) return 0;
  SDG_CHECK_ARG(u && val && ws && ((uintptr_t)ws % 256) == 0);
  SelectWs w;
  if (!select_ws(ws, ws_bytes, r, batch, topk, 8, &w, false)) return SIXDGS_E_WORKSPACE;
  const int64_t nt = sdg_cdiv(r, 256);
  if (u_tile_max && nt >= 2 * (int64_t)topk) return run_topk(u_tile_max, u_stride / 256, nt, batch, topk, w.idxU, val, w.topk_ws, sdg_stream(stream));
  return run_topk(u, u_stride, r, batch, topk, w.idxU, val, w.topk_ws, sdg_stream(stream));
}

int sixdgs_select_candidates(const float* u, int64_t u_stride, int64_t r, const float* u_tile_max, const float* q, const int32_t* d_n_tok, int batch,
                             const float* gsum, const float* d_key_norm_max, const float* d_uk, int topk, int max_candidates, int64_t* cand,
                             int32_t* d_count, void* ws, size_t ws_bytes, sixdgs_stream_t stream) {
  SDG_CHECK_ARG(batch >= 0 && r >= 1 && u_stride >= r && topk >= 1 && topk <= 1024 && max_candidates >= topk && (max_candidates % 8) == 0);
  if (batch == 0) return 0;
  SDG_CHECK_ARG(u && q && d_n_tok && gsum && d_key_norm_max && cand && d_count && ws && ((uintptr_t)ws % 256) == 0 && ((uintptr_t)q % 16) == 0);
  hipStream_t s = sdg_stream(stream);
  SelectWs w;
  if (!select_ws(ws, ws_bytes, r, batch, topk, max_candidates, &w, false)) return SIXDGS_E_WORKSPACE;
  const int k_eff = (int)(r < topk ? r : topk);
  const dim3 cg((unsigned)w.p.nbc, (unsigned)batch);
  const int64_t nt = sdg_cdiv(r, 256);
  const bool tiles = !d_uk && u_tile_max && nt >= 2 * (int64_t)topk;
  const int* none = nullptr;
  if (d_uk) {
    hipLaunchKernelGGL(k_sel_bounds, dim3((unsigned)batch), dim3(kT), 0, s, gsum, d_n_tok, d_uk, q, d_key_norm_max, 1, 1, w.info, none);
  } else if (!tiles) {
    int st = run_topk(u, u_stride, r, batch, topk, w.idxU, w.valU, w.topk_ws, s);
    if (st) return st;
    hipLaunchKernelGGL(k_sel_bounds, dim3((unsigned)batch), dim3(kT), 0, s, gsum, d_n_tok, w.valU, q, d_key_norm_max, topk, k_eff, w.info, none);
  } else {
    int* need = w.total + batch;
    int st = run_topk(u_tile_max, u_stride / 256, nt, batch, topk, w.idxU, w.valU, w.topk_ws, s);
    if (st) return st;
    hipLaunchKernelGGL(k_sel_bounds, dim3((unsigned)batch), dim3(kT), 0, s, gsum, d_n_tok, w.valU, q, d_key_norm_max, topk, topk, w.info, none);
    hipLaunchKernelGGL(k_sel_candidates<false>, cg, dim3(256), 0, s, u, u_stride, r, w.info, w.p.span, w.counts, w.offs, cand, max_candidates, none, u_tile_max);
    hipLaunchKernelGGL(k_sel_scan, dim3((unsigned)batch), dim3(1024), 0, s, w.counts, w.p.nbc, w.offs, w.total);
    hipLaunchKernelGGL(k_sel_need_exact, dim3((unsigned)sdg_cdiv(batch, 64)), dim3(64), 0, s, w.total, w.info, batch, max_candidates, need);
    st = run_topk(u, u_stride, r, batch, topk, w.idxU, w.valU, w.topk_ws, s, need);
    if (st) return st;
    hipLaunchKernelGGL(k_sel_bounds, dim3((unsigned)batch), dim3(kT), 0, s, gsum, d_n_tok, w.valU, q, d_key_norm_max, topk, k_eff, w.info, need);
    hipLaunchKernelGGL(k_sel_candidates<false>, cg, dim3(256), 0, s, u, u_stride, r, w.info, w.p.span, w.counts, w.offs, cand, max_candidates, need, u_tile_max);
    hipLaunchKernelGGL(k_sel_scan, dim3((unsigned)batch), dim3(1024), 0, s, w.counts, w.p.nbc, w.offs, w.total);
    hipLaunchKernelGGL(k_sel_candidates<true>, cg, dim3(256), 0, s, u, u_stride, r, w.info, w.p.span, w.counts, w.offs, cand, max_candidates, none, u_tile_max);
  }
  if (!tiles) {
    hipLaunchKernelGGL(k_sel_candidates<false>, cg, dim3(256), 0, s, u, u_stride, r, w.info, w.p.span, w.counts, w.offs, cand, max_candidates, none, u_tile_max);
    hipLaunchKernelGGL(k_sel_scan, dim3((unsigned)batch), dim3(1024), 0, s, w.counts, w.p.nbc, w.offs, w.total);
    hipLaunchKernelGGL(k_sel_candidates<true>, cg, dim3(256), 0, s, u, u_stride, r, w.info, w.p.span, w.counts, w.offs, cand, max_candidates, none, u_tile_max);
  }
  hipLaunchKernelGGL(k_sel_count, dim3((unsigned)sdg_cdiv(batch, 64)), dim3(64), 0, s, w.total, w.info, batch, d_count);
  SDG_LAUNCH_OK();
  return 0;
}

int sixdgs_select_rescore(const float* q, const int32_t* d_n_tok, int batch, const void* planes, const float* d_scale, int compact,
                          const float* ctok, const float* gsum, const int64_t* cand, const int32_t* d_count, int64_t r, int topk,
                          int max_candidates, int allow_fewer, int64_t* idx, float* val, int32_t* d_status, void* ws, size_t ws_bytes,
                          sixdgs_stream_t stream) {
  SDG_CHECK_ARG(batch >= 0 && r >= 1 && topk >= 1 && topk <= 1024 && max_candidates >= topk && (max_candidates % 8) == 0);
  if (batch == 0) return 0;
  SDG_CHECK_ARG(q && d_n_tok && planes && d_scale && ctok && gsum && cand && d_count && idx && val && d_status && ws &&
                ((uintptr_t)planes % 16) == 0 && ((uintptr_t)q % 16) == 0 && ((uintptr_t)ws % 256) == 0);
  hipStream_t s = sdg_stream(stream);
  const int cmax = max_candidates;
  SelectWs w;
  if (!select_ws(ws, ws_bytes, cmax, batch, topk, cmax, &w, false)) return SIXDGS_E_WORKSPACE;
  const int k_eff = (int)(r < topk ? r : topk);
  select_q_planes(q, batch, w, s);
  hipLaunchKernelGGL(k_sel_rescore, dim3((unsigned)(cmax / 8), (unsigned)batch), dim3(kT), 0, s, w.qplanes, w.qinv, (const char*)planes, d_scale,
                     d_n_tok, 0, ctok, gsum, cand, d_count, cmax, compact, w.cscore);
  const int st = run_topk(w.cscore, cmax, cmax, batch, topk, w.lidx, w.lval, w.topk_ws, s);
  if (st) return st;
  hipLaunchKernelGGL(k_sel_emit, dim3((unsigned)batch), dim3(1024), 0, s, w.lidx, w.lval, cand, d_count, cmax, topk, k_eff, allow_fewer, idx, val, d_status);
  SDG_LAUNCH_OK();
  return 0;
}

size_t sixdgs_score_select_workspace_bytes(int64_t r, int batch, int topk, int max_candidates) {
  if (batch < 1) batch = 1;
  const size_t stride = (size_t)sdg_cdiv(r > 0 ? r : 1, 256) * 256;
  return sdg_align(sixdgs_select_workspace_bytes(r, batch, topk, max_candidates)) +
         (size_t)batch * (2 * sdg_align(kT * sizeof(float)) + sdg_align(stride * sizeof(float)) + sdg_align(stride / 256 * sizeof(float)) +
                          sdg_align((size_t)max_candidates * sizeof(int64_t)) + 256);
}

int sixdgs_score_select(const float* q, const int32_t* d_n_tok, const int32_t* h_n_tok, int batch, const void* key_planes,
                        const float* d_key_scale, const float* d_key_norm_max, int64_t r, const void* sample_planes, const float* d_sample_scale,
                        int64_t r_sample, int topk, int max_candidates, int64_t* idx, float* val, int32_t* d_status, void* ws, size_t ws_bytes,
                        sixdgs_stream_t stream, sixdgs_profile* prof) {
  SDG_CHECK_ARG(r >= 1 && r_sample >= 1 && r_sample <= r && batch >= 0 && topk >= 1 && topk <= 1024 && max_candidates >= topk &&
                max_candidates <= (1 << 20) && (max_candidates % 8) == 0);
  if (batch == 0) return 0;
  SDG_CHECK_ARG(q && d_n_tok && d_key_norm_max && idx && val && d_status && ws && ((uintptr_t)ws % 256) == 0);
  int64_t bg = batch > 4096 ? 4096 : batch;
  while (bg >= 1 && sixdgs_score_select_workspace_bytes(r, (int)bg, topk, max_candidates) > ws_bytes) --bg;
  if (bg < 1) return SIXDGS_E_WORKSPACE;
  bg = sdg_cdiv(batch, sdg_cdiv(batch, bg));
  const size_t stride = (size_t)sdg_cdiv(r, 256) * 256;
  const size_t stage = sdg_align(sixdgs_select_workspace_bytes(r, (int)bg, topk, max_candidates));
  char* base = (char*)ws + stage;
  float* ctok = (float*)base;                        base += (size_t)bg * sdg_align(kT * sizeof(float));
  float* gsum = (float*)base;                        base += (size_t)bg * sdg_align(kT * sizeof(float));
  float* u = (float*)base;                           base += (size_t)bg * sdg_align(stride * sizeof(float));
  float* utm = (float*)base;                         base += (size_t)bg * sdg_align(stride / 256 * sizeof(float));
  int64_t* cand = (int64_t*)base;                    base += (size_t)bg * sdg_align((size_t)max_candidates * sizeof(int64_t));
  int32_t* count = (int32_t*)base;
  for (int b0 = 0; b0 < batch; b0 += (int)bg) {
    const int nb = (int)((batch - b0) < bg ? (batch - b0) : bg);
    const float* qg = q + (int64_t)b0 * kT * SIXDGS_D;
    const int32_t* ng = d_n_tok + b0;
    int st = sixdgs_select_begin(qg, ng, h_n_tok ? h_n_tok + b0 : nullptr, nb, sample_planes, d_sample_scale, r_sample, r, ctok, gsum, ws, stage, stream);
    if (st) return st;
    st = sixdgs_select_sweep(qg, ng, h_n_tok ? h_n_tok + b0 : nullptr, nb, key_planes, d_key_scale, r, ctok, gsum, u, (int64_t)stride, utm, ws, stage,
                             stream, prof);
    if (st) return st;
    st = sixdgs_select_candidates(u, (int64_t)stride, r, utm, qg, ng, nb, gsum, d_key_norm_max, nullptr, topk, max_candidates, cand, count, ws, stage, stream);
    if (st) return st;
    st = sixdgs_select_rescore(qg, ng, nb, key_planes, d_key_scale, 0, ctok, gsum, cand, count, r, topk, max_candidates, 0,
                               idx + (int64_t)b0 * topk, val + (int64_t)b0 * topk, d_status + b0, ws, stage, stream);
    if (st) return st;
  }
  return 0;
}

}
```

### 6dgs_amd/identification_module.py

```python
from __future__ import annotations

from typing import List, Optional, Sequence

import torch

from . import ops
from .backbone import BackboneWrapper, BatchedTokens
from .camera_direction_network import CameraDirectionPredictor


def _lib_ray_keys_ws(r: int, max_chunk: int = ops.RAY_KEYS_CHUNK) -> int:
    from . import _lib
    return int(_lib.load().sixdgs_ray_keys_workspace_bytes(int(r), int(max_chunk)))


class RayPreprocessor(torch.nn.Module):

    def __init__(self, viewpe=8, pospe=8, rgbpe=6, featureC=128, fea_output=128):
        super().__init__()
        self.in_mlpC = 2 * viewpe * 3 + 3 + 2 * pospe * 3 + 3 + 2 * rgbpe * 3 + 3
        self.mlp = torch.nn.Sequential(torch.nn.Linear(self.in_mlpC, featureC), torch.nn.ReLU(inplace=True),
                                       torch.nn.Linear(featureC, featureC), torch.nn.ReLU(inplace=True))
        self.mlp2 = torch.nn.Sequential(torch.nn.Linear(featureC + self.in_mlpC, featureC), torch.nn.ReLU(inplace=True),
                                        torch.nn.Linear(featureC, fea_output))
        self.viewpe, self.pospe, self.rgbpe = viewpe, pospe, rgbpe


class MultiHeadAttention(torch.nn.Module):

    def __init__(self, ray_fea_size, img_fea_size, embed_dim, num_heads=1):
        super().__init__()
        assert embed_dim % num_heads == 0
        self.embed_dim, self.num_heads, self.head_dim = embed_dim, num_heads, embed_dim // num_heads
        self.q_proj = torch.nn.Linear(img_fea_size, embed_dim)
        self.k_proj = torch.nn.Linear(ray_fea_size, embed_dim)
        torch.nn.init.xavier_uniform_(self.q_proj.weight)
        self.q_proj.bias.data.fill_(0)
        torch.nn.init.xavier_uniform_(self.k_proj.weight)
        self.k_proj.bias.data.fill_(0)


class AttentionMapProxy:

    def __init__(self, n_tokens: int, n_rays: int, builder=None):
        self.shape = torch.Size((n_tokens, n_rays))
        self._builder = builder

    def materialize(self) -> torch.Tensor:
        if self._builder is None:
            raise RuntimeError("attention map not retained")
        return self._builder()


class IdentificationModule(torch.nn.Module):
    def __init__(self, backbone_type: str = "dino", camera_up_output_augmentation=None,
                 target_rays_dirs: Optional[torch.Tensor] = None, augmentation_channels: int = 10,
                 backbone: Optional[torch.nn.Module] = None):
        super().__init__()
        if camera_up_output_augmentation not in (None, 0, "NONE") and getattr(camera_up_output_augmentation, "name", "NONE") != "NONE":
            raise NotImplementedError("camera-up output augmentations are not on the accelerated path "
                                      "(reference default is NONE, identification_module.py:11,35-36)")
        self.backbone_wrapper = BackboneWrapper(backbone_type=backbone_type, backbone=backbone)
        nf = self.backbone_wrapper.img_num_features
        self.ray_preprocessor = RayPreprocessor(featureC=512, fea_output=nf)
        self.camera_up_out_augmentation = None
        self.camera_direction_prediction_network = CameraDirectionPredictor(nf, self.backbone_wrapper.backbone_wh, fea_output=3)
        self.attention = MultiHeadAttention(nf, nf + 14, nf, 1)
        self.hip_autograd = True
        self._packed = None
        self._packed_key = None
        self._key_cache = None
        self._key_cache_id = None
        self._key_cache_rays = None

    def _scorer_params(self):
        rp, at = self.ray_preprocessor, self.attention
        return {
            "ray_preprocessor.mlp.0.weight": rp.mlp[0].weight, "ray_preprocessor.mlp.0.bias": rp.mlp[0].bias,
            "ray_preprocessor.mlp.2.weight": rp.mlp[2].weight, "ray_preprocessor.mlp.2.bias": rp.mlp[2].bias,
            "ray_preprocessor.mlp2.0.weight": rp.mlp2[0].weight, "ray_preprocessor.mlp2.0.bias": rp.mlp2[0].bias,
            "ray_preprocessor.mlp2.2.weight": rp.mlp2[2].weight, "ray_preprocessor.mlp2.2.bias": rp.mlp2[2].bias,
            "attention.k_proj.weight": at.k_proj.weight, "attention.k_proj.bias": at.k_proj.bias,
            "attention.q_proj.weight": at.q_proj.weight, "attention.q_proj.bias": at.q_proj.bias,
        }

    def packed_weights(self, device) -> ops.PackedWeights:
        params = self._scorer_params()
        key = (str(device),) + tuple((p.data_ptr(), p._version) for p in params.values())
        if self._packed is None or self._packed_key != key:
            self._packed = ops.PackedWeights(params, device)
            self._packed_key = key
            self._key_cache = None
        return self._packed

    KEEP_FP32_KEYS_BELOW = 4_000_000

    def _ensure_keys(self, rays_ori, rays_dir, rays_rgb, profile=None, sample_min_rays: Optional[int] = None):
        w = self.packed_weights(rays_ori.device)
        mode = ops.effective_mma_mode()
        fmt = "f16-planes" if mode in ops.F16_MODES else f"f32-keys-mma{mode}"
        smin = ops.SELECT_MIN_RAYS if sample_min_rays is None else int(sample_min_rays)
        ident = (rays_ori.shape[0], rays_ori._version, rays_dir._version, rays_rgb._version, self._packed_key, fmt, rays_ori.shape[0] >= smin)
        held = self._key_cache_rays
        same = (self._key_cache is not None and self._key_cache_id == ident and held is not None
                and all(h is t or (h.data_ptr() == t.data_ptr() and h.shape == t.shape and h.stride() == t.stride())
                        for h, t in zip(held, (rays_ori, rays_dir, rays_rgb))))
        if not same:
            self._key_cache = self._key_cache_rays = None
            if ops.get_arena() is not None:
                self._select_ws = self._stream_sample = None
                ops.get_arena().reset(self)
            r = rays_ori.shape[0]
            planes_mode = mode in ops.F16_MODES
            keep_fp32 = (not planes_mode) or r <= self.KEEP_FP32_KEYS_BELOW
            scale = None
            norm = torch.zeros(1, device=rays_ori.device) if planes_mode else None
            if planes_mode:
                _, key, (planes, scale) = ops.ray_keys(rays_ori, rays_dir, rays_rgb, w, want_key=keep_fp32, profile=profile, want_planes=True, norm_out=norm)
            else:
                _, key = ops.ray_keys(rays_ori, rays_dir, rays_rgb, w, profile=profile)
                planes = None
            sample = None
            if planes_mode and r >= smin:
                si = ops.select_sample_indices(r, rays_ori.device)
                _, _, (s_planes, s_scale) = ops.ray_keys(rays_ori[si], rays_dir[si], rays_rgb[si], w, want_key=False, want_planes=True)
                sample = (s_planes, s_scale)
            self._key_cache, self._key_cache_id = {"key": key, "planes": planes, "scale": scale, "sample": sample, "norm": norm}, ident
            self._key_cache_rays = (rays_ori, rays_dir, rays_rgb)
        return self._key_cache

    def ray_keys(self, rays_ori, rays_dir, rays_rgb, profile=None) -> torch.Tensor:
        c = self._ensure_keys(rays_ori, rays_dir, rays_rgb, profile)
        if c["key"] is None:
            _, key = ops.ray_keys(rays_ori, rays_dir, rays_rgb, self.packed_weights(rays_ori.device))
            return key
        return c["key"]

    def ray_features(self, rays_ori, rays_dir, rays_rgb) -> torch.Tensor:
        feat, _ = ops.ray_keys(rays_ori, rays_dir, rays_rgb, self.packed_weights(rays_ori.device), want_feat=True, want_key=False)
        return feat

    def _full_ntok(self, b, device):
        c = getattr(self, "_ntok_cache", None)
        if c is None or c.shape[0] < b or c.device != device:
            self._ntok_cache = c = torch.full((max(b, 64),), ops.MAX_TOKENS, dtype=torch.int32, device=device)
        return c[:b]

    def _tokens_to_q(self, token_list, device):
        w = self.packed_weights(device)
        if isinstance(token_list, BatchedTokens):
            b, t = token_list.shape[0], token_list.shape[1]
            if t != ops.MAX_TOKENS:
                token_list = token_list.dense()
            else:
                wq, bq = self.attention.q_proj.weight, self.attention.q_proj.bias
                pe = token_list.pe
                c = getattr(self, "_peq", None)
                if c is None or c[0] != self._packed_key or c[1] is not pe or c[2] != pe._version:
                    self._peq = c = (self._packed_key, pe, pe._version, torch.addmm(bq.detach(), pe, wq.detach()[:, ops.D:].t()).contiguous(),
                                     wq.detach()[:, :ops.D].contiguous())
                q = ops.linear(token_list.feats.reshape(b * t, ops.D), c[4]).view(b, t, ops.D)
                q += c[3]
                return q, self._full_ntok(b, device), [t] * b
        if torch.is_tensor(token_list):
            tokens = token_list.contiguous()
            n_host = [tokens.shape[1]] * tokens.shape[0]
            n_tok = self._full_ntok(tokens.shape[0], tokens.device)
        else:
            tokens, n_tok = ops.pad_tokens(token_list, device)
            n_host = [int(t.shape[0]) for t in token_list]
        return ops.q_proj(tokens, n_tok, w), n_tok, n_host

    def invalidate_caches(self):
        self._packed = self._key_cache = self._key_cache_rays = self._select_ws = self._stream_sample = self._peq = None
        if ops.get_arena() is not None:
            ops.get_arena().reset(self)

    @torch.no_grad()
    def image_tokens_u8(self, imgs_u8: torch.Tensor, table256: torch.Tensor):
        bw = self.backbone_wrapper
        norm = bw.preprocess_batch_u8(imgs_u8, table256)
        if norm is None:
            return None
        return bw.assemble_batch(bw.features_from_norm(norm))

    @torch.no_grad()
    def image_tokens(self, imgs: Sequence[torch.Tensor], masks: Sequence[Optional[torch.Tensor]]):
        bw = self.backbone_wrapper
        if all(m is None for m in masks) and all(i.shape == imgs[0].shape for i in imgs):
            stacked = imgs if isinstance(imgs, torch.Tensor) and imgs.dim() == 4 else torch.stack(list(imgs))
            feats = bw.features_from_norm(bw.preprocess_batch(stacked))
            return bw.assemble_batch(feats)
        pre = [bw.preprocess(i, m) for i, m in zip(imgs, masks)]
        feats = bw.features_from_norm(torch.cat([p[0] for p in pre], dim=0))
        toks, fmaps = [], []
        for f, (_, mimg) in zip(feats, pre):
            t_pe, _, fmap = bw.assemble(f, mimg)
            toks.append(t_pe)
            fmaps.append(fmap)
        return toks, torch.stack(fmaps)

    @torch.no_grad()
    def camera_up(self, fmaps: torch.Tensor) -> torch.Tensor:
        up = self.camera_direction_prediction_network(fmaps)
        return torch.nn.functional.normalize(up, dim=-1)

    @torch.no_grad()
    def score_tokens(self, token_list: List[torch.Tensor], rays_ori, rays_dir, rays_rgb, rays_to_output: int = 100,
                     want_scores: bool = True, workspace: Optional[torch.Tensor] = None, images_in_flight: Optional[int] = None,
                     profile=None, defer_status: bool = False):
        rays_to_output = ops.check_topk(rays_to_output)
        kc = self._ensure_keys(rays_ori, rays_dir, rays_rgb)
        w = self.packed_weights(rays_ori.device)
        q, n_tok, n_host = self._tokens_to_q(token_list, rays_ori.device)
        self.last_scoring_path = "two-pass"
        self.pending_select = None
        capturing = torch.cuda.is_current_stream_capturing()
        if (not want_scores and kc.get("sample") is not None and ops.select_enabled() and ops.effective_mma_mode() in ops.F16_MODES
                and rays_to_output <= ops.SELECT_MAX_CANDIDATES and (defer_status or not capturing)):
            b, r = q.shape[0], rays_ori.shape[0]
            need = ops.score_select_workspace_bytes(r, b, rays_to_output, ops.SELECT_MAX_CANDIDATES)
            sw = getattr(self, "_select_ws", None)
            if sw is None or sw.numel() < need or sw.device != q.device:
                if capturing:
                    raise RuntimeError("6dgs_amd: the select workspace must exist before a hipGraph capture (run the batch once eagerly)")
                self._select_ws = sw = None
                self._select_ws = sw = ops.big_empty(need, torch.uint8, q.device)
            idx, val, status = ops.score_select(q, n_tok, kc["planes"], kc["scale"], kc["sample"][0], kc["sample"][1], rays_to_output,
                                                max_candidates=ops.SELECT_MAX_CANDIDATES, workspace=sw, profile=profile, n_tok_host=n_host,
                                                key_norm=kc["norm"])
            self.last_select_launches = ops.select_sweep_plan(n_host)
            self.last_scoring_path = "select"
            pend = dict(status=status, q=q, n_tok=n_tok, k=rays_to_output, workspace=workspace, images_in_flight=images_in_flight,
                        rays=(rays_ori, rays_dir, rays_rgb))
            if defer_status:
                self.pending_select = pend
                return idx, val, None
            idx, val, _ = self.finish_select(idx, val, pend)
            return idx, val, None
        idx, val, scores, _ = ops.score_topk(q, n_tok, kc["key"], rays_to_output, want_scores=want_scores, workspace=workspace,
                                             images_in_flight=images_in_flight, profile=profile, n_tok_host=n_host,
                                             key_planes=kc["planes"], key_scale=kc["scale"])
        return idx, val, scores

    @torch.no_grad()
    def finish_select(self, idx, val, pending=None, status_host=None):
        pend = pending if pending is not None else self.pending_select
        self.pending_select = None
        if pend is None:
            return idx, val, []
        st = pend["status"].tolist() if status_host is None else [int(v) for v in status_host]
        self.last_select_candidates = st
        redo = [i for i, v in enumerate(st) if v < 0]
        self.last_scoring_path = "select" if not redo else f"select+two-pass({len(redo)})"
        if redo:
            kc = self._ensure_keys(*pend["rays"])
            q, n_tok = pend["q"], pend["n_tok"]
            sel = torch.tensor(redo, device=q.device)
            i2, v2, _, _ = ops.score_topk(q[sel].contiguous(), n_tok[sel].contiguous(), kc["key"], pend["k"], want_scores=False,
                                          workspace=pend["workspace"], images_in_flight=pend["images_in_flight"], key_planes=kc["planes"],
                                          key_scale=kc["scale"])
            idx[sel], val[sel] = i2, v2
        return idx, val, redo

    @torch.no_grad()
    def score_tokens_ray_sharded(self, token_list, rays_ori, rays_dir, rays_rgb, ray_offset: int, r_total: int, rays_to_output: int = 100,
                                 group=None, profile=None, use_select: bool = True):
        from . import distributed as dd
        dev, k = rays_ori.device, ops.check_topk(rays_to_output)
        world = dd.world()
        kc = self._ensure_keys(rays_ori, rays_dir, rays_rgb, sample_min_rays=max(4096, ops.SELECT_MIN_RAYS // max(world, 1)))
        q, n_tok, n_host = self._tokens_to_q(token_list, dev)
        f16 = ops.effective_mma_mode() in ops.F16_MODES
        have = torch.tensor([1 if (kc.get("sample") is not None and f16 and use_select and ops.select_enabled()
                                  and k <= ops.SELECT_MAX_CANDIDATES) else 0,
                             0 if kc.get("sample") is None else int(kc["sample"][0].shape[0])], dtype=torch.int64, device=dev)
        if dd.is_dist():
            flag, cnt = have[:1].clone(), have[1:].clone()
            dd._all_reduce(flag, torch.distributed.ReduceOp.MIN, group)
            dd._all_reduce(cnt, torch.distributed.ReduceOp.SUM, group)
            have = torch.cat([flag, cnt])
        use, r_sample_total = bool(int(have[0])), int(have[1])
        b = q.shape[0]
        idx = torch.full((b, k), -1, dtype=torch.int64, device=dev)
        val = torch.full((b, k), float("nan"), device=dev)
        redo = list(range(b))
        self.last_scoring_path = f"ray-sharded x{world} two-pass"
        if use:
            idx, val, st = dd.score_select_ray_sharded(q, n_tok, kc["planes"], kc["scale"], kc["sample"][0], kc["sample"][1], ray_offset, r_total,
                                                       r_sample_total, k, n_tok_host=n_host, profile=profile, group=group, key_norm=kc["norm"])
            self.last_select_candidates = st
            redo = [i for i, v in enumerate(st) if v < 0]
            self.last_scoring_path = f"ray-sharded x{world} select" + (f"+two-pass({len(redo)})" if redo else "")
        if redo:
            sel = torch.tensor(redo, device=dev)
            i2, v2, _ = dd.score_topk_ray_sharded(q[sel].contiguous(), n_tok[sel].contiguous(), kc["key"], ray_offset, k, key_planes=kc["planes"],
                                                  key_scale=kc["scale"], group=group)
            idx[sel], val[sel] = i2, v2
        return idx, val

    @torch.no_grad()
    def score_tokens_streamed(self, token_list, rays_ori, rays_dir, rays_rgb, rays_to_output: int = 100, chunk_rays: int = 8_388_608,
                              profile=None, key_cache_bytes: Optional[int] = None, return_stats: bool = False, use_select: bool = True):
        rays_to_output = ops.check_topk(rays_to_output)
        dev = rays_ori.device
        w = self.packed_weights(dev)
        q, n_tok, n_host = self._tokens_to_q(token_list, dev)
        b, r, k = q.shape[0], rays_ori.shape[0], rays_to_output
        chunk = max(256, (min(chunk_rays, max(r, 1)) + 255) // 256 * 256)
        mode = ops.effective_mma_mode()
        f16 = planes_mode = mode in ops.F16_MODES
        self.last_scoring_path = "streamed two-pass"
        if (f16 and use_select and not return_stats and ops.select_enabled() and r >= ops.SELECT_MIN_RAYS and k <= ops.SELECT_MAX_CANDIDATES
                and not torch.cuda.is_current_stream_capturing()):
            cmax = ops.SELECT_MAX_CANDIDATES
            held = getattr(self, "_stream_sample", None)
            ident = (r, rays_ori._version, rays_dir._version, rays_rgb._version, self._packed_key)
            if not (held is not None and held[0] == ident and all(h.data_ptr() == t.data_ptr() for h, t in zip(held[1], (rays_ori, rays_dir, rays_rgb)))):
                self._stream_sample = held = None
                if ops.get_arena() is not None:
                    self._key_cache = self._key_cache_rays = self._select_ws = None
                    ops.get_arena().reset(self)
                si = ops.select_sample_indices(r, dev)
                _, _, (sp, sscale) = ops.ray_keys(rays_ori[si], rays_dir[si], rays_rgb[si], w, want_key=False, want_planes=True)
                self._stream_sample = held = (ident, (rays_ori, rays_dir, rays_rgb), sp, sscale)
            with ops.arena_scope():
                ss = ops.SelectStream(q, n_tok, r, k, cmax, n_host)
                ss.reserve(max(min(chunk, r), int(held[2].shape[0])))
                ss.begin(held[2], held[3])
                for r0 in range(0, r, chunk):
                    r1 = min(r0 + chunk, r)
                    with ops.arena_scope():
                        _, _, (planes, scale) = ops.ray_keys(rays_ori[r0:r1], rays_dir[r0:r1], rays_rgb[r0:r1], w, want_key=False, want_planes=True,
                                                             norm_out=ss.key_norm)
                        ss.sweep(planes, scale, r0, profile, update_norm=False)
                        del planes, scale
                cand, count = ss.candidates()
                inside = torch.arange(cmax, device=dev)[None, :] < count.clamp(min=0, max=cmax)[:, None]
                ci = torch.where(inside, cand, torch.zeros_like(cand)).reshape(-1)
                _, _, (cp, cs) = ops.ray_keys(rays_ori[ci], rays_dir[ci], rays_rgb[ci], w, want_key=False, want_planes=True)
                idx, val, status = ss.rescore(cp, cs, cand, count, compact=True)
            st = status.tolist()
            self.last_select_candidates = st
            redo = [i for i, v in enumerate(st) if v < 0]
            self.last_scoring_path = "streamed select" if not redo else f"streamed select+two-pass({len(redo)})"
            if redo:
                del ss
                sub = token_list[torch.tensor(redo, device=dev)] if (torch.is_tensor(token_list) or isinstance(token_list, BatchedTokens)) else [token_list[i] for i in redo]
                i2, v2 = self.score_tokens_streamed(sub, rays_ori, rays_dir, rays_rgb, k, chunk_rays, profile, key_cache_bytes, use_select=False)
                sel = torch.tensor(redo, device=dev)
                idx[sel], val[sel] = i2, v2
                self.last_scoring_path = f"streamed select+two-pass({len(redo)})"
            return idx, val
        with ops.arena_scope():
            ws = ops.big_empty(ops.score_topk_workspace_bytes(min(chunk, r), b, k, planes=planes_mode), torch.uint8, dev)
            n_c = min(chunk, r)
            per_ray = 1536 if f16 else 4 * ops.D
            if key_cache_bytes is None:
                transient = n_c * per_ray + int(_lib_ray_keys_ws(n_c, ops.RAY_KEYS_CHUNK_MIN if ops.get_arena() is not None else ops.RAY_KEYS_CHUNK))
                arena = ops.get_arena()
                from_arena = arena is not None and planes_mode and arena.buf.device == dev
                room = (arena.capacity - arena.mark()) if from_arena else torch.cuda.mem_get_info(dev)[0]
                key_cache_bytes = max(0, int(0.7 * (room - transient)))
            kept, kept_bytes = {}, 0

            def chunk_keys(r0):
                r1 = min(r0 + chunk, r)
                o, d, c = rays_ori[r0:r1], rays_dir[r0:r1], rays_rgb[r0:r1]
                if not planes_mode:
                    _, key = ops.ray_keys(o, d, c, w)
                    return (key, None, None)
                _, _, (planes, scale) = ops.ray_keys(o, d, c, w, want_key=False, want_planes=True)
                return (None, planes, scale)

            def chunk_pass1(r0, may_keep):
                nonlocal kept_bytes
                run = lambda ent: ops.score_pass1(q, n_tok, ent[0], ws, k, key_planes=ent[1], key_scale=ent[2], profile=profile, n_tok_host=n_host)
                if r0 in kept:
                    return run(kept.pop(r0))
                nbytes = (min(r0 + chunk, r) - r0) * per_ray
                if may_keep and kept_bytes + nbytes <= key_cache_bytes:
                    kept[r0], kept_bytes = chunk_keys(r0), kept_bytes + nbytes
                    return run(kept[r0])
# ... 122 lines not shown
```

### 6dgs_amd/ops.py

```python
from __future__ import annotations

import ctypes as C
import functools
import os
import threading
from typing import Optional, Tuple

import torch

from . import _lib
from ._lib import Profile, ScorerWeights, check

D = 384
MMA_DEFAULT, MMA_F32, MMA_BF16X6, MMA_F16X3, MMA_F16X3_L32 = -1, 0, 1, 2, 3
F16_MODES = (MMA_F16X3, MMA_F16X3_L32)
MMA_LIBRARY_DEFAULT = MMA_F16X3
_mma_mode = MMA_DEFAULT


def set_mma_mode(mode: int):
    global _mma_mode
    assert mode in (MMA_DEFAULT, MMA_F32, MMA_BF16X6, MMA_F16X3, MMA_F16X3_L32)
    _mma_mode = mode

# ... 588 lines not shown


def ray_keys_workspace_bytes(r: int, max_chunk: int = RAY_KEYS_CHUNK) -> int:
    return int(_lib.load().sixdgs_ray_keys_workspace_bytes(int(r), int(max_chunk)))


@_on_device
def ray_keys(ori, dr, rgb, weights: PackedWeights, want_feat: bool = False, want_key: bool = True, max_chunk: int = RAY_KEYS_CHUNK,
             workspace: Optional[torch.Tensor] = None, profile: Optional["KernelProfile"] = None, want_planes: bool = False,
             norm_out: Optional[torch.Tensor] = None):
    ori, dr, rgb = _f32(ori), _f32(dr), _f32(rgb)
    _need_gpu(ori, dr, rgb)
    lib = _lib.load()
    r = ori.shape[0]
    dev = ori.device
    feat = torch.empty(r, D, device=dev) if want_feat else None
    key = torch.empty(r, D, device=dev) if want_key else None
    mode = effective_mma_mode()
    f16 = want_planes and mode in F16_MODES
    if want_planes and not f16:
        raise RuntimeError("6dgs_amd: key planes exist in the fp16 x 3 modes only (MMA_F32 / MMA_BF16X6 score on fp32 keys)")
    planes = big_empty((r, 1536), torch.uint8, dev) if want_planes else None
    inv = torch.empty((r + 127) // 128, device=dev) if f16 else None
    nbytes = lib.sixdgs_ray_keys_workspace_bytes(r, int(max_chunk))
    if workspace is None or workspace.numel() < nbytes:
        chunk = int(max_chunk)
        room = (_arena.capacity - _arena.off) if (_arena is not None and _arena.buf.device == dev) else 0.5 * _free_bytes(dev)
        while chunk > RAY_KEYS_CHUNK_MIN and nbytes > room:
            chunk //= 2
            nbytes = lib.sixdgs_ray_keys_workspace_bytes(r, chunk)
    if norm_out is not None and not f16:
        raise RuntimeError("6dgs_amd: norm_out needs scaled fp16 key planes (want_planes in MMA_F16X3 mode)")
    with arena_scope():
        ws = workspace if workspace is not None and workspace.numel() >= nbytes else big_empty(nbytes, torch.uint8, dev)
        check(lib.sixdgs_ray_keys_ex(_p(ori), _p(dr), _p(rgb), r, weights.ref, _p(feat), _p(key), _p(planes), _p(inv), _p(norm_out), _p(ws), ws.numel(),
                                     _stream(), profile.ref if profile is not None else None, mode), "ray_keys")
    if want_planes:
        return feat, key, (planes, inv)
    return feat, key


@_on_device
def pad_tokens(token_list, device) -> Tuple[torch.Tensor, torch.Tensor]:
    b = len(token_list)
    tok = torch.zeros(b, MAX_TOKENS, TOK_IN, device=device)
    n = torch.empty(b, dtype=torch.int32)
    for i, t in enumerate(token_list):
        if t.shape[0] > MAX_TOKENS or t.shape[1] != TOK_IN:
            raise RuntimeError(f"6dgs_amd: token block {tuple(t.shape)} does not fit [<=256, 398]")
        tok[i, : t.shape[0]] = t
        n[i] = t.shape[0]
    return tok, n.to(device)


@_on_device
def q_proj(tokens: torch.Tensor, n_tok: torch.Tensor, weights: PackedWeights) -> torch.Tensor:
    tokens = _f32(tokens)
    _need_gpu(tokens, n_tok)
    b = tokens.shape[0]
    q = torch.empty(b, MAX_TOKENS, D, device=tokens.device)
    check(_lib.load().sixdgs_q_proj(_p(tokens), _p(n_tok), b, weights.ref, _p(q), _stream()), "q_proj")
    return q


def score_topk_workspace_bytes(r: int, batch: int, topk: int = 100, planes: bool = False) -> int:
    if planes:
        return int(_lib.load().sixdgs_score_topk_workspace_bytes_ex(int(r), int(batch), int(topk), effective_mma_mode(), 1))
    return int(_lib.load().sixdgs_score_topk_workspace_bytes(int(r), int(batch), int(topk)))


@_on_device
def score_topk(q: torch.Tensor, n_tok: torch.Tensor, key: Optional[torch.Tensor], topk: int = 100, want_scores: bool = True,
               want_stats: bool = False, workspace: Optional[torch.Tensor] = None, images_in_flight: Optional[int] = None,
               profile: Optional["KernelProfile"] = None, n_tok_host=None, key_planes: Optional[torch.Tensor] = None,
               key_scale: Optional[torch.Tensor] = None):
    q = _f32(q)
    key = _f32(key) if key is not None else None
    _need_gpu(q, key, n_tok, key_planes)
    lib = _lib.load()
    r = key.shape[0] if key is not None else key_planes.shape[0]
    b, dev = q.shape[0], q.device
    idx = torch.empty(b, topk, dtype=torch.int64, device=dev)
    val = torch.empty(b, topk, device=dev)
    scores = torch.empty(b, r, device=dev) if want_scores else None
    stats = torch.empty(b, MAX_TOKENS, 2, device=dev) if want_stats else None
    if workspace is None:
        inflight = b if images_in_flight is None else max(1, min(b, images_in_flight))
        workspace = torch.empty(score_topk_workspace_bytes(r, inflight, topk, planes=key_planes is not None), dtype=torch.uint8, device=dev)
    h_n = None
    if profile is not None and n_tok_host is not None:
        h_n = (C.c_int32 * b)(*[int(v) for v in n_tok_host])
    mode = effective_mma_mode()
    if key_planes is not None and mode in F16_MODES:
        if key_planes.shape[1] != 1536 or key_scale is None:
            raise RuntimeError("6dgs_amd: key planes are not in the format of the active MMA mode (scaled fp16 planes [R,1536] + key_scale)")
    elif key_planes is not None:
        if key is None:
            raise RuntimeError("6dgs_amd: MMA_F32 / MMA_BF16X6 score on fp32 keys: pass `key` (key planes are the operand of the fp16 x 3 kernels only)")
        key_planes = key_scale = None
    check(lib.sixdgs_score_topk_ex(_p(q), _p(n_tok), h_n, b, _p(key), _p(key_planes), _p(key_scale), r, int(topk), _p(scores), _p(idx), _p(val), _p(stats),
                                   _p(workspace), workspace.numel(), _stream(), profile.ref if profile is not None else None,
                                   _mma_mode), "score_topk")
    return idx, val, scores, stats


MAX_TOPK = 1024


def check_topk(k, what: str = "rays_to_output") -> int:
    if isinstance(k, bool) or int(k) != k or not 1 <= int(k) <= MAX_TOPK:
        raise ValueError(f"6dgs_amd: {what} = {k!r}: the top-k takes 1 <= k <= MAX_TOPK = {MAX_TOPK}")
    return int(k)


SELECT_MAX_CANDIDATES = 4096
SELECT_SAMPLE_STRIDE = 16
SELECT_SAMPLE_STRIDE_LARGE = 32
SELECT_LARGE_RAYS = 16_000_000
SELECT_SAMPLE_STRIDE_HUGE = 64
SELECT_HUGE_RAYS = 32_000_000
SELECT_MIN_RAYS = 1 << 20
_select_enabled = True


def set_select_enabled(on: bool):
    global _select_enabled
    _select_enabled = bool(on)


def select_enabled() -> bool:
    return _select_enabled


@_on_device
def select_sample_indices(r: int, device, stride: Optional[int] = None) -> torch.Tensor:
    if stride is None:
        stride = SELECT_SAMPLE_STRIDE_HUGE if r >= SELECT_HUGE_RAYS else (SELECT_SAMPLE_STRIDE_LARGE if r >= SELECT_LARGE_RAYS else SELECT_SAMPLE_STRIDE)
    n = r // stride
    i = torch.arange(n, dtype=torch.int64, device=device)
    return i * stride + (((i * 2654435761) & 0xFFFFFFFF) >> 13) % stride


@_on_device
def key_norm_max(planes: torch.Tensor, scale: torch.Tensor, out: Optional[torch.Tensor] = None) -> torch.Tensor:
    _need_gpu(planes, scale, out)
    if planes.shape[1] != 1536:
        raise RuntimeError("6dgs_amd: key_norm_max needs scaled fp16 key planes (MMA_F16X3)")
    if out is None:
        out = torch.zeros(1, device=planes.device)
    check(_lib.load().sixdgs_key_planes_norm_max(_p(planes), _p(scale), planes.shape[0], _p(out), _stream()), "key_planes_norm_max")
    return out


def score_select_workspace_bytes(r: int, batch: int, topk: int = 100, max_candidates: int = SELECT_MAX_CANDIDATES) -> int:
    return int(_lib.load().sixdgs_score_select_workspace_bytes(int(r), int(batch), int(topk), int(max_candidates)))


def select_sweep_plan(n_tok_host, batch: Optional[int] = None):
    lib = _lib.load()
    b = len(n_tok_host) if n_tok_host is not None else int(batch)
    h_n = (C.c_int32 * b)(*[int(v) for v in n_tok_host]) if n_tok_host is not None else None
    cap = max(1, b)
    slots, imgs = (C.c_int32 * cap)(), (C.c_int32 * cap)()
    n = lib.sixdgs_select_sweep_plan(h_n, b, slots, imgs, cap)
    if n < 0:
        check(n, "select_sweep_plan")
    return [(int(slots[i]), int(imgs[i])) for i in range(min(n, cap))]


@_on_device
def score_select(q: torch.Tensor, n_tok: torch.Tensor, key_planes: torch.Tensor, key_scale: torch.Tensor, sample_planes: torch.Tensor,
                 sample_scale: torch.Tensor, topk: int = 100, max_candidates: int = SELECT_MAX_CANDIDATES,
                 workspace: Optional[torch.Tensor] = None, profile: Optional["KernelProfile"] = None, n_tok_host=None,
                 key_norm: Optional[torch.Tensor] = None):
    q = _f32(q)
    _need_gpu(q, n_tok, key_planes, key_scale, sample_planes, sample_scale, key_norm)
    if key_norm is None:
        key_norm = key_norm_max(key_planes, key_scale)
    if key_planes.shape[1] != 1536 or sample_planes.shape[1] != 1536:
        raise RuntimeError("6dgs_amd: score_select needs scaled fp16 key planes (MMA_F16X3)")
    lib = _lib.load()
    b, dev, r, rs = q.shape[0], q.device, key_planes.shape[0], sample_planes.shape[0]
    idx = torch.empty(b, topk, dtype=torch.int64, device=dev)
    val = torch.empty(b, topk, device=dev)
    status = torch.empty(b, dtype=torch.int32, device=dev)
    if workspace is None:
        workspace = torch.empty(score_select_workspace_bytes(r, b, topk, max_candidates), dtype=torch.uint8, device=dev)
    h_n = (C.c_int32 * b)(*[int(v) for v in n_tok_host]) if n_tok_host is not None else None
    check(lib.sixdgs_score_select(_p(q), _p(n_tok), h_n, b, _p(key_planes), _p(key_scale), _p(key_norm), r, _p(sample_planes), _p(sample_scale), rs,
                                  int(topk), int(max_candidates), _p(idx), _p(val), _p(status), _p(workspace), workspace.numel(), _stream(),
                                  profile.ref if profile is not None else None), "score_select")
    return idx, val, status


class SelectStream:

    @_on_device
    def __init__(self, q: torch.Tensor, n_tok: torch.Tensor, r_total: int, topk: int = 100, max_candidates: int = SELECT_MAX_CANDIDATES,
                 n_tok_host=None):
        self.q, self.n_tok = _f32(q), n_tok
        _need_gpu(self.q, n_tok)
        self.b, self.dev = self.q.shape[0], self.q.device
        self.device = self.dev
        self.r, self.topk, self.cmax = int(r_total), int(topk), int(max_candidates)
        self.stride = (self.r + 255) // 256 * 256
        self.ctok = torch.empty(self.b, MAX_TOKENS, device=self.dev)
        self.gsum = torch.empty(self.b, MAX_TOKENS, device=self.dev)
        self.u = big_empty((self.b, self.stride), torch.float32, self.dev)
        self.utm = torch.empty(self.b, self.stride // 256, device=self.dev)
        self.key_norm = torch.zeros(1, device=self.dev)
        self.ws = torch.empty(1, dtype=torch.uint8, device=self.dev)
        self.h_n = (C.c_int32 * self.b)(*[int(v) for v in n_tok_host]) if n_tok_host is not None else None

    def _grow(self, need):
        if self.ws.numel() < need:
            self.ws = None
            self.ws = big_empty(need, torch.uint8, self.dev)

    def reserve(self, chunk_rows: int):
        lib = _lib.load()
        self._grow(max(lib.sixdgs_select_workspace_bytes(int(chunk_rows), self.b, self.topk, self.cmax),
                       lib.sixdgs_select_candidates_workspace_bytes(self.r, self.b, self.topk, self.cmax)))

    @_on_device
    def begin(self, sample_planes, sample_scale):
        _need_gpu(self.q, sample_planes, sample_scale)
        lib = _lib.load()
        self._grow(lib.sixdgs_select_workspace_bytes(sample_planes.shape[0], self.b, self.topk, self.cmax))
        check(lib.sixdgs_select_begin(_p(self.q), _p(self.n_tok), self.h_n, self.b, _p(sample_planes), _p(sample_scale), sample_planes.shape[0], self.r,
                                      _p(self.ctok), _p(self.gsum), _p(self.ws), self.ws.numel(), _stream()), "select_begin")

    @_on_device
    def sample_stats(self, sample_planes, sample_scale) -> torch.Tensor:
        _need_gpu(self.q, sample_planes, sample_scale)
        lib = _lib.load()
        self._grow(lib.sixdgs_select_workspace_bytes(sample_planes.shape[0], self.b, self.topk, self.cmax))
        stats = torch.empty(self.b, MAX_TOKENS, 2, device=self.dev)
        check(lib.sixdgs_select_sample_stats(_p(self.q), _p(self.n_tok), self.h_n, self.b, _p(sample_planes), _p(sample_scale), sample_planes.shape[0],
                                             _p(stats), _p(self.ws), self.ws.numel(), _stream()), "select_sample_stats")
        return stats

    @_on_device
    def prepare(self, stats: torch.Tensor, r_sample_total: int, r_total: int):
        stats = _f32(stats)
        _need_gpu(self.q, stats)
        check(_lib.load().sixdgs_select_prepare(_p(stats), _p(self.n_tok), self.b, int(r_sample_total), int(r_total), _p(self.ctok), _p(self.gsum),
                                                _stream()), "select_prepare")

    @_on_device
    def topk_u(self, exact: bool = False) -> torch.Tensor:
        lib = _lib.load()
        _need_gpu(self.q)
        self._grow(lib.sixdgs_select_candidates_workspace_bytes(self.r, self.b, self.topk, self.cmax))
        val = torch.empty(self.b, self.topk, device=self.dev)
        check(lib.sixdgs_select_topk_u(_p(self.u), self.stride, self.r, None if exact else _p(self.utm), self.b, self.topk, _p(val), _p(self.ws),
                                       self.ws.numel(), _stream()),
              "select_topk_u")
        return val

    @_on_device
    def sweep(self, planes, scale, ray_offset: int, profile: Optional["KernelProfile"] = None, update_norm: bool = True):
        if ray_offset % 256:
            raise RuntimeError("6dgs_amd: select sweep chunks must start at a multiple of 256 rays")
        _need_gpu(self.q, planes, scale)
        lib = _lib.load()
        rc = planes.shape[0]
        self._grow(lib.sixdgs_select_workspace_bytes(rc, self.b, self.topk, self.cmax))
        check(lib.sixdgs_select_sweep(_p(self.q), _p(self.n_tok), self.h_n, self.b, _p(planes), _p(scale), rc,
                                      _p(self.ctok), _p(self.gsum), C.c_void_p(self.u.data_ptr() + 4 * int(ray_offset)), self.stride,
                                      C.c_void_p(self.utm.data_ptr() + 4 * (int(ray_offset) // 256)),
                                      _p(self.ws), self.ws.numel(), _stream(), profile.ref if profile is not None else None), "select_sweep")
        if update_norm:
            key_norm_max(planes, scale, out=self.key_norm)

    @_on_device
    def candidates(self, uk: Optional[torch.Tensor] = None):
        lib = _lib.load()
        _need_gpu(self.q)
        self._grow(lib.sixdgs_select_candidates_workspace_bytes(self.r, self.b, self.topk, self.cmax))
        cand = torch.zeros(self.b, self.cmax, dtype=torch.int64, device=self.dev)
        count = torch.empty(self.b, dtype=torch.int32, device=self.dev)
        uk = _f32(uk) if uk is not None else None
        check(lib.sixdgs_select_candidates(_p(self.u), self.stride, self.r, _p(self.utm), _p(self.q), _p(self.n_tok), self.b, _p(self.gsum), _p(self.key_norm),
                                           _p(uk), self.topk, self.cmax, _p(cand), _p(count), _p(self.ws), self.ws.numel(), _stream()), "select_candidates")
        return cand, count

    @_on_device
    def rescore(self, planes, scale, cand, count, compact: bool, allow_fewer: bool = False):
        lib = _lib.load()
        _need_gpu(self.q, planes, scale, cand, count)
        idx = torch.empty(self.b, self.topk, dtype=torch.int64, device=self.dev)
        val = torch.empty(self.b, self.topk, device=self.dev)
        status = torch.empty(self.b, dtype=torch.int32, device=self.dev)
        self._grow(lib.sixdgs_select_candidates_workspace_bytes(self.r, self.b, self.topk, self.cmax))
        check(lib.sixdgs_select_rescore(_p(self.q), _p(self.n_tok), self.b, _p(planes), _p(scale), 1 if compact else 0, _p(self.ctok),
                                        _p(self.gsum), _p(cand), _p(count), self.r, self.topk, self.cmax, 1 if allow_fewer else 0, _p(idx), _p(val), _p(status),
                                        _p(self.ws), self.ws.numel(), _stream()), "select_rescore")
        return idx, val, status


@_on_device
def score_pass1(q: torch.Tensor, n_tok: torch.Tensor, key: Optional[torch.Tensor], workspace: torch.Tensor, topk: int = 100,
                key_planes: Optional[torch.Tensor] = None, key_scale: Optional[torch.Tensor] = None,
                profile: Optional["KernelProfile"] = None, n_tok_host=None) -> torch.Tensor:
    q = _f32(q)
    key = _f32(key) if key is not None else None
    _need_gpu(q, key, n_tok, key_planes, workspace)
    r = key.shape[0] if key is not None else key_planes.shape[0]
    b = q.shape[0]
    stats = torch.empty(b, MAX_TOKENS, 2, device=q.device)
    h_n = (C.c_int32 * b)(*[int(v) for v in n_tok_host]) if (profile is not None and n_tok_host is not None) else None
    check(_lib.load().sixdgs_score_pass1(_p(q), _p(n_tok), h_n, b, _p(key), _p(key_planes), _p(key_scale), r, int(topk), _p(stats),
                                         _p(workspace), workspace.numel(), _stream(), profile.ref if profile is not None else None,
                                         _mma_mode), "score_pass1")
    return stats


@_on_device
def score_pass2(stats: torch.Tensor, n_tok: torch.Tensor, r: int, workspace: torch.Tensor, topk: int = 100, used_planes: bool = True,
                want_scores: bool = True):
    stats = _f32(stats)
    _need_gpu(stats, n_tok, workspace)
    b, dev = stats.shape[0], stats.device
    idx = torch.empty(b, topk, dtype=torch.int64, device=dev)
    val = torch.empty(b, topk, device=dev)
    scores = torch.empty(b, r, device=dev) if want_scores else None
    check(_lib.load().sixdgs_score_pass2(_p(stats), _p(n_tok), b, 1 if used_planes else 0, int(r), int(topk), _p(scores), _p(idx), _p(val),
                                         _p(workspace), workspace.numel(), _stream(), _mma_mode), "score_pass2")
    return idx, val, scores


def _check_scorer_operands(q: torch.Tensor, n_tok: torch.Tensor, k: torch.Tensor):
    _need_gpu(q, n_tok, k)
    if q.dtype != torch.float32 or k.dtype != torch.float32:
        raise RuntimeError(f"6dgs_amd: q and k must be float32 (got {q.dtype}, {k.dtype})")
    if q.dim() != 3 or tuple(q.shape[1:]) != (MAX_TOKENS, D):
        raise RuntimeError(f"6dgs_amd: q must be [B,{MAX_TOKENS},{D}] (got {tuple(q.shape)})")
    if k.dim() != 2 or k.shape[1] != D or k.shape[0] < 1:
        raise RuntimeError(f"6dgs_amd: k must be [R,{D}] with R >= 1 (got {tuple(k.shape)})")
    if n_tok.dtype != torch.int32 or tuple(n_tok.shape) != (q.shape[0],):
        raise RuntimeError(f"6dgs_amd: n_tok must be int32 [{q.shape[0]}] (got {n_tok.dtype} {tuple(n_tok.shape)})")
    if not (q.is_contiguous() and k.is_contiguous() and n_tok.is_contiguous()):
        raise RuntimeError("6dgs_amd: q, n_tok and k must be contiguous")


@_on_device
def score_backward(q: torch.Tensor, n_tok: torch.Tensor, k: torch.Tensor, row_stats: torch.Tensor, g: torch.Tensor, ray_groups: int = 1):
    ray_groups = int(ray_groups)
    if ray_groups < 0:
        raise ValueError(f"6dgs_amd: ray_groups must be >= 0 (got {ray_groups})")
    _check_scorer_operands(q, n_tok, k)
    b, r = q.shape[0], k.shape[0]
    if tuple(row_stats.shape) != (b, MAX_TOKENS, 2) or tuple(g.shape) != (b, r):
        raise RuntimeError(f"6dgs_amd: row_stats must be [{b},{MAX_TOKENS},2] and g [{b},{r}] (got {tuple(row_stats.shape)}, {tuple(g.shape)})")
    row_stats, g = _f32(row_stats), _f32(g)
    _need_gpu(row_stats, g)
    lib = _lib.load()
    dq = torch.empty_like(q)
    dk = torch.empty_like(k)
    if ray_groups == 1:
        ws = torch.empty(max(1, lib.sixdgs_score_backward_workspace_bytes(b)), dtype=torch.uint8, device=q.device)
        check(lib.sixdgs_score_backward(_p(q), _p(n_tok), b, _p(k), r, _p(row_stats), _p(g), _p(dq), _p(dk), _p(ws), ws.numel(), _stream()),
              "score_backward")
    else:
        ws = torch.empty(max(1, lib.sixdgs_score_backward_split_workspace_bytes(b, r, ray_groups)), dtype=torch.uint8, device=q.device)
        check(lib.sixdgs_score_backward_split(_p(q), _p(n_tok), b, _p(k), r, _p(row_stats), _p(g), _p(dq), _p(dk), ray_groups, _p(ws), ws.numel(),
                                              _stream()), "score_backward_split")
    return dq, dk


@_on_device
def _ray_attention_forward(q: torch.Tensor, n_tok: torch.Tensor, k: torch.Tensor):
    _check_scorer_operands(q, n_tok, k)
    b, r = q.shape[0], k.shape[0]
    planes = effective_mma_mode() in F16_MODES
    kp, ks = split_planes_f16(k) if planes else (None, None)
    ws = torch.empty(score_topk_workspace_bytes(r, b, 1, planes=planes), dtype=torch.uint8, device=q.device)
    stats = score_pass1(q, n_tok, k, ws, 1, key_planes=kp, key_scale=ks)
    _, _, scores = score_pass2(stats, n_tok, r, ws, 1, used_planes=planes)
    return scores, stats


class RayAttentionScores(torch.autograd.Function):

    @staticmethod
    def forward(ctx, q, n_tok, k, ray_groups=1):
        q, k = q.detach(), k.detach()
        scores, stats = _ray_attention_forward(q, n_tok, k)
        ctx.save_for_backward(q, n_tok, k, stats)
        ctx.ray_groups = ray_groups
        return scores

# ... 126 lines not shown
```

### include/sixdgs.h

```cpp
#ifndef SIXDGS_H
#define SIXDGS_H

#include <stddef.h>
#include <stdint.h>

#ifdef __cplusplus
extern "C" {
#endif

#define SIXDGS_ABI_VERSION 10
#define SIXDGS_E_BADARG (-1)
#define SIXDGS_E_WORKSPACE (-2)
#define SIXDGS_E_UNSUPPORTED (-3)

#define SIXDGS_D 384
#define SIXDGS_RAY_IN 141
#define SIXDGS_RAY_IN_PAD 144
#define SIXDGS_HID 512
#define SIXDGS_TOK_IN 398
#define SIXDGS_MAX_TOKENS 256

typedef void* sixdgs_stream_t;

#define SIXDGS_MMA_DEFAULT (-1)
// ... 38 lines not shown
                                 int table_res, const int64_t* d_offsets, float* ori, float* dir, float* rgb,
                                 int64_t* src, sixdgs_stream_t stream);
int sixdgs_quadricell_cell_counts(const float* scale , int64_t e, int target_points,
                                  int64_t* d_counts, int64_t* d_offsets, int64_t* d_total, sixdgs_stream_t stream);
int sixdgs_quadricell_centers(const float* scale , int64_t e, int target_points, int table_res,
                              const int64_t* d_cell_offsets , float* points, int64_t* ellipsoid_id,
                              sixdgs_stream_t stream);

int sixdgs_isocell_distribution(int ray_target, int n0, float* dirs , int64_t* h_count,
                                sixdgs_stream_t stream);
int sixdgs_rotate_isocell(const float* dirs, int64_t k, const float* normals, int64_t e, float* out ,
                          sixdgs_stream_t stream);
int sixdgs_emit_isocell(const float* xyz, const float* scale, int scale_is_log, const float* rot, const float* f_dc,
                        const float* f_rest, int sh_degree, int n_coef, const int64_t* sel, int64_t e,
                        const float* normals, const float* dirs, int64_t k, float* ori, float* dir, float* rgb,
                        int64_t* src, sixdgs_stream_t stream);
int sixdgs_eval_sh_color(const float* sh, int n_coef, const float* dirs, int64_t r, int sh_degree, float* rgb,
                         sixdgs_stream_t stream);

size_t sixdgs_splat_views_workspace_bytes(int64_t n, int views, int width, int height);
int sixdgs_splat_views(const float* xyz, const float* scale, int scale_is_log, const float* f_dc, const float* f_rest,
                       int sh_degree, int n_coef, int64_t n,
                       const float* cams , int views, int width,
                       int height, int channels , float extent, float near_z,
                       const float* background , uint8_t* image ,
                       int32_t* winner , void* ws, size_t ws_bytes,
                       sixdgs_stream_t stream);

typedef struct sixdgs_scorer_weights {
  const float* w1;
  const float* b1;
  const float* w2;
  const float* b2;
  const float* w3;
  const float* b3;
  const float* w4;
  const float* b4;
  const float* wk;
  const float* bk;
  const float* wq;
  const float* bq;
  const float* m1;
  const float* m2;
  const float* m3;
  const float* m4;
  const float* mk;
  const float* w4k;
  const float* b4k;
  const float* m4k;
  const void* planes;
} sixdgs_scorer_weights;

size_t sixdgs_packed_weights_floats(void);
int sixdgs_pack_weights(const float* mlp0_w, const float* mlp0_b, const float* mlp2_w, const float* mlp2_b,
                        const float* mlp2_0_w, const float* mlp2_0_b, const float* mlp2_2_w, const float* mlp2_2_b,
                        const float* kproj_w, const float* kproj_b, const float* qproj_w, const float* qproj_b,
                        float* packed, sixdgs_scorer_weights* out, sixdgs_stream_t stream);

int sixdgs_ray_encode(const float* ori, const float* dir, const float* rgb, int64_t r, float* x, sixdgs_stream_t stream);

size_t sixdgs_ray_keys_workspace_bytes(int64_t r, int64_t max_chunk);
int sixdgs_ray_keys(const float* ori, const float* dir, const float* rgb, int64_t r, const sixdgs_scorer_weights* w,
                    float* feat, float* key, void* ws, size_t ws_bytes, sixdgs_stream_t stream);
int sixdgs_ray_keys_ex(const float* ori, const float* dir, const float* rgb, int64_t r, const sixdgs_scorer_weights* w,
                       float* feat, float* key, void* key_planes, float* key_inv_scale, float* d_key_norm_max, void* ws,
                       size_t ws_bytes, sixdgs_stream_t stream, sixdgs_profile* prof, int mma_mode);
size_t sixdgs_key_planes_f16_bytes(int64_t r);
int sixdgs_split_planes_f16(const float* src, int64_t rows, int64_t ld, void* planes, float* d_inv_scale, sixdgs_stream_t stream);

int sixdgs_linear(const float* x, int64_t m, int k, int64_t ldx, const float* w, int64_t ldw, const float* b, int n,
                  int relu, float* y, int64_t ldy, sixdgs_stream_t stream);
int sixdgs_linear_ex(const float* x, int64_t m, int k, int64_t ldx, const float* w, int64_t ldw, const float* b, int n,
                     int relu, float* y, int64_t ldy, sixdgs_stream_t stream, int mma_mode);
size_t sixdgs_linear_splitk_workspace_bytes(int64_t m, int n, int slices);
int sixdgs_linear_splitk(const float* x, int64_t m, int k, int64_t ldx, const float* w, int64_t ldw, const float* b, int n,
                         int relu, float* y, int64_t ldy, int slices, void* ws, size_t ws_bytes, sixdgs_stream_t stream,
                         int mma_mode);

#define SIXDGS_TOK_A_PLAIN 0
#define SIXDGS_TOK_A_LAYERNORM 1
#define SIXDGS_TOK_EPI_BIAS 0
#define SIXDGS_TOK_EPI_GELU 1
#define SIXDGS_TOK_EPI_RESID 2
size_t sixdgs_tok_pack_bytes(int n, int k);
int sixdgs_tok_pack(const float* w , int n, int k, int64_t ldw, void* planes, float* inv_scale , sixdgs_stream_t stream);
int sixdgs_tok_linear(const float* x, int64_t m, int k, int64_t ldx, int a_mode, const float* ln_weight, const float* ln_bias, float ln_eps,
                      const void* w_planes, const float* w_inv_scale, const float* bias , int n, int epilogue, const float* residual,
                      int64_t ldr, const float* gamma, float* y, int64_t ldy, sixdgs_stream_t stream);

int sixdgs_tok_attention(const float* qkv, int64_t ldq, int images, int tokens, int heads, float* y, int64_t ldy, sixdgs_stream_t stream);

int sixdgs_im2col(const float* x, int64_t stride_b, int64_t stride_c, int64_t stride_y, int64_t stride_x, int batch, int channels, int height, int width, int k,
                  int taps_major, float* a, sixdgs_stream_t stream);

int sixdgs_u8_to_planar(const uint8_t* images, int batch, int64_t pixels, const float* table256, float* out, sixdgs_stream_t stream);

int sixdgs_image_prep(const uint8_t* images, int batch, int height, int width, const float* table256, int resized_h, int resized_w, int crop_top, int crop_left,
                      int out_size, const float* mean3, const float* std3, float* out, sixdgs_stream_t stream);

int sixdgs_q_proj(const float* tokens, const int32_t* d_n_tok, int batch,
                  const sixdgs_scorer_weights* w, float* q, sixdgs_stream_t stream);

size_t sixdgs_score_topk_workspace_bytes(int64_t r, int batch, int topk);
size_t sixdgs_score_topk_workspace_bytes_ex(int64_t r, int batch, int topk, int mma_mode, int with_key_planes);
int sixdgs_score_topk(const float* q , const int32_t* d_n_tok, int batch, const float* key ,
                      int64_t r, int topk, float* scores , int64_t* idx ,
                      float* val , float* row_stats , void* ws,
                      size_t ws_bytes, sixdgs_stream_t stream);
int sixdgs_score_topk_ex(const float* q, const int32_t* d_n_tok, const int32_t* h_n_tok ,
                         int batch, const float* key, const void* key_planes, const float* d_key_scale, int64_t r, int topk,
                         float* scores, int64_t* idx, float* val, float* row_stats, void* ws, size_t ws_bytes,
                         sixdgs_stream_t stream, sixdgs_profile* prof, int mma_mode);

int sixdgs_score_pass1(const float* q, const int32_t* d_n_tok, const int32_t* h_n_tok, int batch, const float* key,
                       const void* key_planes, const float* d_key_scale, int64_t r, int topk, float* row_stats, void* ws,
                       size_t ws_bytes, sixdgs_stream_t stream, sixdgs_profile* prof, int mma_mode);
int sixdgs_score_pass2(const float* row_stats, const int32_t* d_n_tok, int batch, int used_planes, int64_t r, int topk,
                       float* scores, int64_t* idx, float* val, void* ws, size_t ws_bytes, sixdgs_stream_t stream, int mma_mode);
size_t sixdgs_score_backward_workspace_bytes(int batch);
int sixdgs_score_backward(const float* q, const int32_t* d_n_tok, int batch, const float* key , int64_t r,
                          const float* row_stats, const float* g, float* dq, float* dk, void* ws, size_t ws_bytes, sixdgs_stream_t stream);
size_t sixdgs_score_backward_split_workspace_bytes(int batch, int64_t r, int ray_groups);
int sixdgs_score_backward_split(const float* q, const int32_t* d_n_tok, int batch, const float* key , int64_t r,
                                const float* row_stats, const float* g, float* dq, float* dk, int ray_groups, void* ws, size_t ws_bytes,
                                sixdgs_stream_t stream);
size_t sixdgs_score_select_workspace_bytes(int64_t r, int batch, int topk, int max_candidates);
int sixdgs_key_planes_norm_max(const void* planes, const float* d_scale, int64_t rows, float* d_norm_max, sixdgs_stream_t stream);
size_t sixdgs_select_workspace_bytes(int64_t r, int batch, int topk, int max_candidates);
size_t sixdgs_select_candidates_workspace_bytes(int64_t r, int batch, int topk, int max_candidates);
int sixdgs_select_sweep_plan(const int32_t* h_n_tok, int batch, int32_t* slots_per_launch, int32_t* images_per_launch, int max_launches);
int sixdgs_select_begin(const float* q, const int32_t* d_n_tok, const int32_t* h_n_tok, int batch, const void* sample_planes, const float* d_sample_scale,
                        int64_t r_sample, int64_t r_total, float* ctok, float* gsum, void* ws, size_t ws_bytes, sixdgs_stream_t stream);
int sixdgs_select_sample_stats(const float* q, const int32_t* d_n_tok, const int32_t* h_n_tok, int batch, const void* sample_planes, const float* d_sample_scale,
                               int64_t r_sample, float* row_stats , void* ws, size_t ws_bytes, sixdgs_stream_t stream);
int sixdgs_select_prepare(const float* row_stats, const int32_t* d_n_tok, int batch, int64_t r_sample, int64_t r_total, float* ctok, float* gsum,
                          sixdgs_stream_t stream);
int sixdgs_select_topk_u(const float* u, int64_t u_stride, int64_t r, const float* u_tile_max , int batch, int topk, float* val ,
                         void* ws, size_t ws_bytes, sixdgs_stream_t stream);
int sixdgs_select_sweep(const float* q, const int32_t* d_n_tok, const int32_t* h_n_tok, int batch, const void* key_planes,
                        const float* d_key_scale, int64_t r, const float* ctok, float* gsum, float* u, int64_t u_stride, float* u_tile_max,
                        void* ws, size_t ws_bytes, sixdgs_stream_t stream, sixdgs_profile* prof);
int sixdgs_select_candidates(const float* u, int64_t u_stride, int64_t r, const float* u_tile_max , const float* q, const int32_t* d_n_tok, int batch, const float* gsum,
                             const float* d_key_norm_max, const float* d_uk ,
                             int topk, int max_candidates, int64_t* cand, int32_t* d_count, void* ws, size_t ws_bytes, sixdgs_stream_t stream);
int sixdgs_select_rescore(const float* q, const int32_t* d_n_tok, int batch, const void* planes, const float* d_scale, int compact,
                          const float* ctok, const float* gsum, const int64_t* cand, const int32_t* d_count, int64_t r, int topk,
                          int max_candidates, int allow_fewer, int64_t* idx, float* val, int32_t* d_status, void* ws, size_t ws_bytes,
                          sixdgs_stream_t stream);
int sixdgs_score_select(const float* q, const int32_t* d_n_tok, const int32_t* h_n_tok ,
                        int batch, const void* key_planes, const float* d_key_scale, const float* d_key_norm_max, int64_t r,
                        const void* sample_planes, const float* d_sample_scale, int64_t r_sample, int topk, int max_candidates, int64_t* idx ,
                        float* val , int32_t* d_status , void* ws, size_t ws_bytes, sixdgs_stream_t stream,
                        sixdgs_profile* prof);
size_t sixdgs_topk_workspace_bytes(int64_t r, int batch, int topk);
int sixdgs_topk(const float* scores, int64_t r, int batch, int topk, int64_t* idx, float* val, void* ws,
                size_t ws_bytes, sixdgs_stream_t stream);

size_t sixdgs_distance_target_workspace_bytes(int64_t r);
int sixdgs_distance_target(const float* rays_ori, const float* rays_dir, int64_t r, const float* d_pose, int n_tokens,
                           float* target , float* d_sum, void* ws, size_t ws_bytes, sixdgs_stream_t stream);

int sixdgs_solve_pose(const float* rays_ori, const float* rays_dir, int64_t r, const int64_t* idx ,
                      const float* val , int k, const float* up , const float* gt_c2w ,
                      int batch, float* c2w, int32_t* status, float* w_final, int32_t* n_kept, float* centre ,
                      float* errors, sixdgs_stream_t stream);

size_t sixdgs_solve_pose_consensus_workspace_bytes(int batch, int k);
int sixdgs_solve_pose_consensus(const float* rays_ori, const float* rays_dir, int64_t r, const int64_t* idx ,
                                const float* val , int k, const float* up , const float* gt_c2w ,
                                int batch, float tau, int prior, float* c2w, int32_t* status, float* w_final, int32_t* n_kept,
                                float* centre , float* errors, float* support, int32_t* n_inliers, float* rms,
                                int32_t* winner, void* ws, size_t ws_bytes, sixdgs_stream_t stream);

#ifdef __cplusplus
}
#endif
#endif
```

Measured before the change: 74.65.

## Add packed fp16 high-plane prepass for select sample statistics

```diff
diff --git a/6dgs_amd/_lib.py b/6dgs_amd/_lib.py
--- a/6dgs_amd/_lib.py
+++ b/6dgs_amd/_lib.py
@@ -62,6 +62,7 @@
     "sixdgs_score_topk_ex": (i32, [vp, vp, vp, i32, vp, vp, vp, i64, i32, vp, vp, vp, vp, vp, sz, vp, C.POINTER(Profile), i32]),
     "sixdgs_score_select_workspace_bytes": (sz, [i64, i32, i32, i32]),
     "sixdgs_score_select": (i32, [vp, vp, vp, i32, vp, vp, vp, i64, vp, vp, i64, i32, i32, vp, vp, vp, vp, sz, vp, C.POINTER(Profile)]),
+    "sixdgs_score_select_h": (i32, [vp, vp, vp, i32, vp, vp, vp, i64, vp, vp, vp, i64, i32, i32, vp, vp, vp, vp, sz, vp, C.POINTER(Profile)]),
     "sixdgs_tok_attention": (i32, [vp, i64, i32, i32, i32, vp, i64, vp]),
     "sixdgs_im2col": (i32, [vp, i64, i64, i64, i64, i32, i32, i32, i32, i32, i32, vp, vp]),
     "sixdgs_u8_to_planar": (i32, [vp, i32, i64, vp, vp, vp]),
@@ -79,6 +80,9 @@
     "sixdgs_select_rescore": (i32, [vp, vp, i32, vp, vp, i32, vp, vp, vp, vp, i64, i32, i32, i32, vp, vp, vp, vp, sz, vp]),
     "sixdgs_select_sample_stats": (i32, [vp, vp, vp, i32, vp, vp, i64, vp, vp, sz, vp]),
     "sixdgs_select_prepare": (i32, [vp, vp, i32, i64, i64, vp, vp, vp]),
+    "sixdgs_pack_h_planes": (i32, [vp, i64, vp, vp]),
+    "sixdgs_select_begin_h": (i32, [vp, vp, vp, i32, vp, vp, vp, i64, i64, vp, vp, vp, sz, vp]),
+    "sixdgs_select_sample_stats_h": (i32, [vp, vp, vp, i32, vp, vp, vp, i64, vp, vp, sz, vp]),
     "sixdgs_select_topk_u": (i32, [vp, i64, i64, vp, i32, i32, vp, vp, sz, vp]),
     "sixdgs_linear_splitk_workspace_bytes": (sz, [i64, i32, i32]),
     "sixdgs_linear_splitk": (i32, [vp, i64, i32, i64, vp, i64, vp, i32, i32, vp, i64, i32, vp, sz, vp, i32]),
diff --git a/6dgs_amd/build.py b/6dgs_amd/build.py
--- a/6dgs_amd/build.py
+++ b/6dgs_amd/build.py
@@ -9,7 +9,7 @@
 LIB = os.path.join(CSRC, "lib6dgs_hip.so")
 HOSTCHECK = os.path.join(CSRC, "libsixdgs_hostcheck.so")
 SOURCES = ["geometry.hip", "gemm.hip", "dense.hip", "score.hip", "score_bwd.hip", "pose.hip", "pose_consensus.hip", "vit.hip", "splat.hip"]
-HEADERS = ["common.h", "device_math.h", "gemm_kernel.h", "dense.h", os.path.join("..", "..", "include", "sixdgs.h"), "dense_layout.h", "sweep_plan.h", "sweep_layout.h"]
+HEADERS = ["common.h", "device_math.h", "gemm_kernel.h", "dense.h", os.path.join("..", "..", "include", "sixdgs.h"), "dense_layout.h", "sweep_plan.h", "sweep_layout.h", "prepass_layout.h"]
 HIPCC = os.environ.get("HIPCC", "/opt/rocm/bin/hipcc")
 FLAGS = ["--offload-arch=gfx950", "-O3", "-std=c++17", "-fPIC", "-ffp-contract=off", "-Wall", "-Wno-unused-function"]
 FLAGS += os.environ.get("SIXDGS_EXTRA_FLAGS", "").split()
@@ -49,7 +49,7 @@
 def build_hostcheck(force: bool = False) -> str:
     src = os.path.join(CSRC, "hostcheck.cpp")
     deps = [src, os.path.join(CSRC, "device_math.h"), os.path.join(CSRC, "dense_layout.h"), os.path.join(CSRC, "sweep_plan.h"),
-            os.path.join(CSRC, "sweep_layout.h")]
+            os.path.join(CSRC, "sweep_layout.h"), os.path.join(CSRC, "prepass_layout.h")]
     if force or _stale(HOSTCHECK, deps):
         cmd = [HIPCC, "-x", "hip", "--offload-arch=gfx950", "-O2", "-std=c++17", "-fPIC", "-ffp-contract=off", "-shared", src,
                "-o", HOSTCHECK]
diff --git a/6dgs_amd/csrc/hostcheck.cpp b/6dgs_amd/csrc/hostcheck.cpp
--- a/6dgs_amd/csrc/hostcheck.cpp
+++ b/6dgs_amd/csrc/hostcheck.cpp
@@ -4,6 +4,7 @@
 #include "sweep_plan.h"
 #include "dense_layout.h"
 #include "sweep_layout.h"
+#include "prepass_layout.h"
 using namespace sdg;
 
 extern "C" {
@@ -170,6 +171,19 @@
 int hc_sw_out_ray(int lane, int x) { return sw::out_ray(lane, x); }
 int hc_sw_part_writes(int lane) { return sw::part_writes(lane) ? 1 : 0; }
 int hc_sw_part_row(int wn, int lane) { return sw::part_row(wn, lane); }
+int hc_pp_const(int which) {
+  const int v[] = {pp::kSlabs, pp::kSlabK, pp::kRowBytes, pp::kStageBytes, pp::kPieceRows, pp::kPieces, pp::kKSteps, pp::kFullRowBytes};
+  return which >= 0 && which < 8 ? v[which] : -1;
+}
+long long hc_pp_packed_offset(long long row, int slab, int chunk) { return pp::packed_offset(row, slab, chunk); }
+long long hc_pp_full_offset(long long row, int slab, int chunk) { return pp::full_offset(row, slab, chunk); }
+int hc_pp_piece_row(int piece, int lane) { return pp::piece_row(piece, lane); }
+int hc_pp_piece_src_chunk(int row, int lane) { return pp::piece_src_chunk(row, lane); }
+unsigned hc_pp_piece_lds_offset(int piece, int lane) { return pp::piece_lds_offset(piece, lane); }
+int hc_pp_frag_row(int lane) { return pp::frag_row(lane); }
+int hc_pp_frag_chunk(int lane, int ks) { return pp::frag_chunk(lane, ks); }
+unsigned hc_pp_frag_offset(int row0, int lane, int ks) { return pp::frag_offset(row0, lane, ks); }
+int hc_pp_frag_k(int lane, int ks, int j) { return pp::frag_k(lane, ks, j); }
 int hc_dl_const(int which) {
   const int v[] = {dl::kSlabB, dl::kPRow, dl::kGran, dl::kGranSlab, dl::kChunkRun};
   return which >= 0 && which < 5 ? v[which] : -1;
diff --git a/6dgs_amd/csrc/prepass_layout.h b/6dgs_amd/csrc/prepass_layout.h
--- /dev/null
+++ b/6dgs_amd/csrc/prepass_layout.h
@@ -0,0 +1,37 @@
+#pragma once
+#include <hip/hip_runtime.h>
+
+namespace sdg {
+namespace pp {
+
+#define SDG_PP __host__ __device__ __forceinline__ constexpr
+
+constexpr int kSlabs = 6, kSlabK = 64, kSlabBytes = 128, kRowBytes = kSlabs * kSlabBytes;
+constexpr int kFullRowBytes = 1536, kFullSlabBytes = 128;
+constexpr int kTileRows = 256, kStageBytes = kTileRows * kSlabBytes;
+constexpr int kPieceRows = 8, kPieceBytes = kPieceRows * kSlabBytes, kPieces = kTileRows / kPieceRows;
+constexpr int kKSteps = 4;
+
+SDG_PP int swizzle(int row) { return (row >> 1) & 7; }
+
+SDG_PP long long packed_offset(long long row, int slab, int chunk) { return row * kRowBytes + slab * kSlabBytes + chunk * 16; }
+SDG_PP long long full_offset(long long row, int slab, int chunk) {
+  const int k = slab * kSlabK + chunk * 8;
+  return row * kFullRowBytes + (k >> 5) * kFullSlabBytes + (k & 31) * 2;
+}
+
+SDG_PP int piece_row(int piece, int lane) { return piece * kPieceRows + (lane >> 3); }
+SDG_PP int piece_src_chunk(int row, int lane) { return (lane & 7) ^ swizzle(row); }
+SDG_PP unsigned piece_lds_offset(int piece, int lane) { return (unsigned)(piece * kPieceBytes + lane * 16); }
+
+SDG_PP int frag_row(int lane) { return lane & 31; }
+SDG_PP int frag_chunk(int lane, int ks) { return 2 * ks + (lane >> 5); }
+SDG_PP unsigned frag_offset(int row0, int lane, int ks) {
+  const int row = row0 + frag_row(lane);
+  return (unsigned)(row * kSlabBytes + ((frag_chunk(lane, ks) ^ swizzle(row)) << 4));
+}
+SDG_PP int frag_k(int lane, int ks, int j) { return 16 * ks + 8 * (lane >> 5) + j; }
+
+#undef SDG_PP
+}
+}
diff --git a/6dgs_amd/csrc/score.hip b/6dgs_amd/csrc/score.hip
--- a/6dgs_amd/csrc/score.hip
+++ b/6dgs_amd/csrc/score.hip
@@ -5,6 +5,7 @@
 #include "gemm_kernel.h"
 #include "sweep_plan.h"
 #include "sweep_layout.h"
+#include "prepass_layout.h"
 
 using namespace sdg;
 
@@ -723,6 +724,251 @@
   } while (PERS && (grp += A.n_sets) < A.n_groups);
 }
 
+template <bool PERS>
+__global__ void __launch_bounds__(512, 1) k_prepass_h(LogitsF16Args A) {
+  static_assert(2 * pp::kStageBytes == kKBaseX && kKBaseX + 3 * pp::kStageBytes == kLdsX, "k_prepass_h: the rings of k_logits_f16x");
+  __shared__ __attribute__((aligned(1024))) char lds[kLdsX];
+  const unsigned w = xcd_remap(blockIdx.x, gridDim.x);
+  const int bl = (int)(w % (unsigned)A.nb);
+  const int set = (int)(w / (unsigned)A.nb);
+  const int b = A.b0 + bl;
+  const int M = A.n_tok[b];
+  const int tid = threadIdx.x, lane = tid & 63;
+  const int wave = __builtin_amdgcn_readfirstlane(tid >> 6);
+  const int wm = wave >> 1, wn = wave & 1;
+  const float cq = A.q_quarter_scales ? A.qinv[4 * b + wm] : A.qinv[2 * b + (wm >> 1)];
+  const bool active = wm * 64 < M;
+  const int t_base = A.n_tiles / A.n_groups, t_rem = A.n_tiles - t_base * A.n_groups;
+  const int n_tiles128 = (int)((A.r + 127) >> 7);
+  int grp = set;
+  do {
+  float* pout = A.partial + ((int64_t)bl * A.n_groups + grp) * kT * 2;
+  float m_run[2] = {-INFINITY, -INFINITY}, s_run[2] = {0.f, 0.f};
+  const int t_begin = grp * t_base + min(grp, t_rem);
+  const int t_end = t_begin + t_base + (grp < t_rem ? 1 : 0);
+  if (M > 0 && t_begin < t_end) {
+    const unsigned lds0 = (unsigned)(uintptr_t)(lds_ptr_t)lds;
+    int lane_p = lane;
+    if (PERS) asm volatile("" : "+v"(lane_p));
+    unsigned offQ[4], offK[4];
+    int rowK[4];
+#pragma unroll
+    for (int i = 0; i < 4; ++i) {
+      const int row = pp::piece_row(wave * 4 + i, lane_p);
+      const unsigned inrow = (unsigned)(pp::piece_src_chunk(row, lane_p) << 4);
+      offQ[i] = (unsigned)min(row, M - 1) * pp::kRowBytes + inrow;
+      offK[i] = inrow;
+      rowK[i] = row;
+    }
+    const char* qbase = A.qp + (int64_t)b * kT * pp::kRowBytes;
+    auto issue_q = [&](const int s, const int qstage, const int i) {
+      __builtin_amdgcn_global_load_lds((gbl_ptr_t)(qbase + (offQ[i] + (unsigned)(s * pp::kSlabBytes))),
+                                       (lds_ptr_t)(lds + qstage * pp::kStageBytes + (wave * 4 + i) * pp::kPieceBytes), 16, 0, 0);
+    };
+    auto issue_k = [&](const char* kbase, int lim, const int s, const int kstage, const int i) {
+      const unsigned ob = (unsigned)min(rowK[i], lim) * pp::kRowBytes + offK[i] + (unsigned)(s * pp::kSlabBytes);
+      __builtin_amdgcn_global_load_lds((gbl_ptr_t)(kbase + ob),
+                                       (lds_ptr_t)(lds + kKBaseX + kstage * pp::kStageBytes + (wave * 4 + i) * pp::kPieceBytes), 16, 0, 2);
+    };
+    auto tile_lim = [&](int tile) {
+      const int64_t left = A.r - (int64_t)tile * kBNX - 1;
+      return left < kBNX - 1 ? (int)left : kBNX - 1;
+    };
+    unsigned fa[pp::kKSteps], fb[pp::kKSteps], fb2[pp::kKSteps];
+#pragma unroll
+    for (int kk = 0; kk < pp::kKSteps; ++kk) {
+      fa[kk] = lds0 + pp::frag_offset(wm * 64, lane_p, kk);
+      fb[kk] = lds0 + kKBaseX + pp::frag_offset(wn * 128, lane_p, kk);
+      fb2[kk] = fb[kk] + 65536u;
+    }
+    auto read_a = [&](const int t, const int kk, const int qstage) { return lds_read_frag_h_off(fa[kk], qstage * pp::kStageBytes + t * 4096); };
+    auto read_b = [&](const int t, const int kk, const int kstage) {
+      const int off = kstage * pp::kStageBytes + t * 4096;
+      return off < 65536 ? lds_read_frag_h_off(fb[kk], off & 65535) : lds_read_frag_h_off(fb2[kk], off & 65535);
+    };
+    const char* kcur = A.kp + (int64_t)t_begin * kBNX * pp::kRowBytes;
+    int lim_cur = tile_lim(t_begin);
+    f16x8 a0[2], a1[2], b0[2], b1[2];
+    auto wait_lds = [&]() {
+      asm volatile("s_waitcnt lgkmcnt(0)" ::: "memory");
+      __builtin_amdgcn_sched_barrier(0);
+    };
+#pragma unroll
+    for (int i = 0; i < 4; ++i) issue_k(kcur, lim_cur, 0, 0, i);
+#pragma unroll
+    for (int i = 0; i < 4; ++i) issue_q(0, 0, i);
+#pragma unroll
+    for (int i = 0; i < 4; ++i) issue_k(kcur, lim_cur, 1, 1, i);
+#pragma unroll
+    for (int i = 0; i < 4; ++i) issue_q(1, 1, i);
+    asm volatile("s_waitcnt vmcnt(8)" ::: "memory");
+    __builtin_amdgcn_s_barrier();
+#pragma unroll
+    for (int t = 0; t < 2; ++t) {
+      a0[t] = read_a(t, 0, 0);
+      b0[t] = read_b(t, 0, 0);
+    }
+    wait_lds();
+
+    for (int tile = t_begin; tile < t_end; ++tile) {
+      const bool has_next = tile + 1 < t_end;
+      const char* knext = has_next ? kcur + (int64_t)kBNX * pp::kRowBytes : kcur;
+      const int lim_next = has_next ? tile_lim(tile + 1) : lim_cur;
+      asm volatile("" : "+v"(offQ[0]), "+v"(offQ[1]), "+v"(offQ[2]), "+v"(offQ[3]), "+v"(offK[0]), "+v"(offK[1]), "+v"(offK[2]), "+v"(offK[3]));
+      if (!active) {
+        int kst = 2;
+#pragma unroll 1
+        for (int sl = 0; sl < pp::kSlabs; ++sl) {
+          const bool nxt = sl + 2 >= pp::kSlabs;
+          const char* kb = nxt ? knext : kcur;
+          const int kl = nxt ? lim_next : lim_cur, sk = nxt ? sl + 2 - pp::kSlabs : sl + 2;
+#pragma unroll
+          for (int i = 0; i < 4; ++i) issue_k(kb, kl, sk, kst, i);
+          kst = kst == 2 ? 0 : kst + 1;
+          asm volatile("s_waitcnt vmcnt(4)" ::: "memory");
+          __builtin_amdgcn_s_barrier();
+          const int sq = sl + 2 < pp::kSlabs ? sl + 2 : sl + 2 - pp::kSlabs;
+#pragma unroll
+          for (int i = 0; i < 4; ++i) issue_q(sq, sl & 1, i);
+        }
+        kcur = knext;
+        lim_cur = lim_next;
+        continue;
+      }
+      f32x16 acc[2][4];
+#pragma unroll
+      for (int i = 0; i < 2; ++i)
+#pragma unroll
+        for (int j = 0; j < 4; ++j)
+#pragma unroll
+          for (int r = 0; r < 16; ++r) acc[i][j][r] = 0.f;
+      auto mfma_step = [&](f16x8 (&xa)[2], f16x8 (&xb)[2], const int h, auto side) {
+#pragma unroll
+        for (int z = 0; z < 4; ++z) {
+          const int tm = z >> 1, tn = z & 1;
+          side(z);
+          acc[tm][2 * h + tn] = __builtin_amdgcn_mfma_f32_32x32x16_f16(xb[tn], xa[tm], acc[tm][2 * h + tn], 0, 0, 0);
+          __builtin_amdgcn_sched_barrier(0);
+        }
+      };
+#pragma unroll
+      for (int sl = 0; sl < pp::kSlabs; ++sl) {
+        const int qs = sl & 1, ks3 = sl % 3;
+        const int qn = (sl + 1) & 1, kn = (sl + 1) % 3;
+        const int ks2 = (sl + 2) % 3;
+#pragma unroll
+        for (int kk = 0; kk < pp::kKSteps; ++kk) {
+          f16x8(&xa)[2] = (kk & 1) ? a1 : a0;
+          f16x8(&na)[2] = (kk & 1) ? a0 : a1;
+          mfma_step(xa, b0, 0, [&](const int z) {
+            if (z < 2) b1[z] = read_b(2 + z, kk, ks3);
+            if (kk == 0) {
+              if (sl + 2 < pp::kSlabs) issue_k(kcur, lim_cur, sl + 2, ks2, z);
+              else issue_k(knext, lim_next, sl + 2 - pp::kSlabs, ks2, z);
+            }
+          });
+          wait_lds();
+          if (kk + 1 < pp::kKSteps) {
+            mfma_step(xa, b1, 1, [&](const int z) {
+              if (z < 2) na[z] = read_a(z, kk + 1, qs);
+              else b0[z - 2] = read_b(z - 2, kk + 1, ks3);
+            });
+          } else {
+            asm volatile("s_waitcnt vmcnt(4)" ::: "memory");
+            __builtin_amdgcn_s_barrier();
+            mfma_step(xa, b1, 1, [&](const int z) {
+              if (z < 2) na[z] = read_a(z, 0, qn);
+              else b0[z - 2] = read_b(z - 2, 0, kn);
+              issue_q((sl + 2) % pp::kSlabs, qs, z);
+            });
+          }
+          wait_lds();
+        }
+      }
+      {
+        const int t128 = min(2 * tile + wn, n_tiles128 - 1);
+        const float cf = (cq * load_uniform(A.kinv + t128)) * kInvSqrtD;
+        const bool ragged = lim_cur < kBNX - 1;
+#pragma unroll
+        for (int tm = 0; tm < 2; ++tm) {
+          float mx = -INFINITY;
+#pragma unroll
+          for (int tn = 0; tn < 4; ++tn)
+#pragma unroll
+            for (int rg = 0; rg < 4; ++rg) {
+              float4 v;
+              v.x = acc[tm][tn][4 * rg + 0] * cf;
+              v.y = acc[tm][tn][4 * rg + 1] * cf;
+              v.z = acc[tm][tn][4 * rg + 2] * cf;
+              v.w = acc[tm][tn][4 * rg + 3] * cf;
+              acc[tm][tn][4 * rg + 0] = v.x;
+              acc[tm][tn][4 * rg + 1] = v.y;
+              acc[tm][tn][4 * rg + 2] = v.z;
+              acc[tm][tn][4 * rg + 3] = v.w;
+              mx = fmaxf(mx, fmaxf(fmaxf(v.x, v.y), fmaxf(v.z, v.w)));
+            }
+          const float mn = fmaxf(m_run[tm], mx);
+          float sum[4] = {0.f, 0.f, 0.f, 0.f};
+          if (!ragged) {
+#pragma unroll
+            for (int tn = 0; tn < 4; ++tn)
+#pragma unroll
+              for (int r = 0; r < 16; ++r) sum[r & 3] += __expf(acc[tm][tn][r] - mn);
+          } else {
+            int ray0 = wn * 128 + 4 * (lane >> 5);
+            asm volatile("" : "+v"(ray0));
+#pragma unroll
+            for (int tn = 0; tn < 4; ++tn)
+#pragma unroll
+              for (int r = 0; r < 16; ++r)
+                sum[r & 3] += (ray0 + tn * 32 + 8 * (r >> 2) + (r & 3) <= lim_cur) ? __expf(acc[tm][tn][r] - mn) : 0.f;
+          }
+          s_run[tm] = s_run[tm] * __expf(m_run[tm] - mn) + ((sum[0] + sum[1]) + (sum[2] + sum[3]));
+          m_run[tm] = mn;
+        }
+      }
+      kcur = knext;
+      lim_cur = lim_next;
+    }
+    asm volatile("s_waitcnt vmcnt(0)" ::: "memory");
+  }
+  __syncthreads();
+  float(*part)[256][2] = reinterpret_cast<float(*)[256][2]>(lds);
+#pragma unroll
+  for (int tm = 0; tm < 2; ++tm) {
+    float* pp2 = part[wn * 2 + (lane >> 5)][wm * 64 + tm * 32 + (lane & 31)];
+    pp2[0] = m_run[tm];
+    pp2[1] = s_run[tm];
+  }
+  __syncthreads();
+  if (tid < 256) {
+    float m = -INFINITY, sres = 0.f;
+#pragma unroll
+    for (int h = 0; h < 4; ++h) {
+      const float mt = part[h][tid][0], st2 = part[h][tid][1];
+      if (mt > -INFINITY) {
+        const float mn = fmaxf(m, mt);
+        sres = sres * __expf(m - mn) + st2 * __expf(mt - mn);
+        m = mn;
+      }
+    }
+    pout[2 * tid] = m;
+    pout[2 * tid + 1] = sres;
+  }
+  if (PERS) __syncthreads();
+  } while (PERS && (grp += A.n_sets) < A.n_groups);
+}
+
+__global__ void __launch_bounds__(256) k_pack_h_planes(const char* __restrict__ src, int64_t rows, char* __restrict__ dst) {
+  constexpr int kChunks = pp::kRowBytes / 16;
+  const int64_t n = rows * kChunks;
+  for (int64_t i = (int64_t)blockIdx.x * 256 + threadIdx.x; i < n; i += (int64_t)gridDim.x * 256) {
+    const int64_t row = i / kChunks;
+    const int c = (int)(i - row * kChunks);
+    *reinterpret_cast<f16x8*>(dst + pp::packed_offset(row, c >> 3, c & 7)) = *reinterpret_cast<const f16x8*>(src + pp::full_offset(row, c >> 3, c & 7));
+  }
+}
+
 __global__ void __launch_bounds__(256) k_split_tiles_f16(const float* __restrict__ src, int64_t rows, int64_t ld, char* __restrict__ dst,
                                                          float* __restrict__ inv_scale) {
   __shared__ float wmax[4];
@@ -1096,17 +1342,20 @@
 
 constexpr float kLog2e = 1.4426950408889634f;
 
+__device__ __forceinline__ float sel_ctok(float m, float z, bool has_token, float log2_frac) {
+  const bool ok = has_token && z > 0.f && m > -INFINITY && m < INFINITY;
+  return ok ? -(m * kLog2e) - (log2f(z) + log2_frac) : -INFINITY;
+}
 __global__ void __launch_bounds__(kT) k_sel_prepare(const float* __restrict__ stats_s, const int* __restrict__ n_tok, int b0, float log2_frac,
                                                     float* __restrict__ ctok) {
   const int bl = blockIdx.x, t = threadIdx.x;
   const float m = stats_s[((int64_t)bl * kT + t) * 2], z = stats_s[((int64_t)bl * kT + t) * 2 + 1];
-  const bool ok = t < n_tok[b0 + bl] && z > 0.f && m > -INFINITY && m < INFINITY;
-  ctok[(int64_t)bl * kT + t] = ok ? -(m * kLog2e) - (log2f(z) + log2_frac) : -INFINITY;
+  ctok[(int64_t)bl * kT + t] = sel_ctok(m, z, t < n_tok[b0 + bl], log2_frac);
 }
 
 __global__ void __launch_bounds__(256) k_split_q_slots(const float* __restrict__ q, const int* __restrict__ n_tok, const SweepSlots T, char* __restrict__ dst,
                                                        float* __restrict__ inv_scale, const float* __restrict__ ctok, float* __restrict__ ctok_slot,
-                                                       int* __restrict__ slot_rows) {
+                                                       int* __restrict__ slot_rows, int h_only, unsigned* __restrict__ zero, int n_zero) {
   __shared__ float wmax[4];
   const int slot = blockIdx.x >> 2, w = blockIdx.x & 3;
   const int img = T.q_img[slot][w], lq = T.q_lq[slot][w];
@@ -1130,7 +1379,9 @@
   }
   const float sc = ldexpf(1.f, sh);
   if (threadIdx.x == 0) inv_scale[blockIdx.x] = ldexpf(1.f, -sh);
-  char* const drow = dst + ((int64_t)slot * kT + 64 * w) * kRowF;
+  if (zero != nullptr && blockIdx.x == 0)
+    for (int i = threadIdx.x; i < n_zero; i += 256) zero[i] = 0u;
+  char* const drow = dst + ((int64_t)slot * kT + 64 * w) * (h_only ? pp::kRowBytes : kRowF);
   for (int i = threadIdx.x; i < 64 * 48; i += 256) {
     const int row = i / 48, k8 = i - row * 48;
     f16x8 h, l;
@@ -1149,6 +1400,10 @@
 #pragma unroll
       for (int e = 0; e < 8; ++e) h[e] = l[e] = (_Float16)0.f;
     }
+    if (h_only) {
+      *reinterpret_cast<f16x8*>(drow + pp::packed_offset(row, k8 >> 3, k8 & 7)) = h;
+      continue;
+    }
     char* d = drow + (int64_t)row * kRowF + (k8 >> 2) * kSlabF + (k8 & 3) * 16;
     *reinterpret_cast<f16x8*>(d) = h;
     *reinterpret_cast<f16x8*>(d + 64) = l;
@@ -1169,7 +1424,8 @@
 }
 
 __global__ void __launch_bounds__(1024) k_merge_stats_slots(const float* __restrict__ partial, int n_groups, const SweepSlots T, float* __restrict__ stats,
-                                                            float* __restrict__ gsum) {
+                                                            float* __restrict__ gsum, const int* __restrict__ n_tok, float log2_frac,
+                                                            float* __restrict__ ctok, float* __restrict__ gsum_zero) {
   __shared__ float sm[16][64][2];
   const int k = blockIdx.x, y = blockIdx.y, tl = threadIdx.x & 63, j = threadIdx.x >> 6;
   const int img = T.img[k], sq = y < T.img_nq[k] ? T.img_q[k][y] : -1;
@@ -1207,6 +1463,10 @@
     } else {
       stats[o * 2] = m;
       stats[o * 2 + 1] = s;
+      if (ctok != nullptr) {
+        ctok[o] = sel_ctok(m, s, 64 * y + tl < n_tok[img], log2_frac);
+        gsum_zero[o] = 0.f;
+      }
     }
   }
 }
@@ -2052,6 +2312,11 @@
   return forced == 1 || (forced != 3 && kPrepassOneTermDefault);
 }
 
+static bool prepass_fused_tail() {
+  const char* e = getenv("SIXDGS_PREPASS_PLANES");
+  return !(e && atoi(e) == 2);
+}
+
 int sixdgs_select_sweep_plan(const int32_t* h_n_tok, int batch, int32_t* slots_per_launch, int32_t* images_per_launch, int max_launches) {
   if (batch < 0 || batch > 32767 || max_launches < 0 || (max_launches > 0 && (!slots_per_launch || !images_per_launch))) return SIXDGS_E_BADARG;
   const std::vector<SweepSlots> plan = sweep_pack(h_n_tok, batch, sweep_slot_cap());
@@ -2062,21 +2327,34 @@
   return (int)plan.size();
 }
 
-int sixdgs_select_sample_stats(const float* q, const int32_t* d_n_tok, const int32_t* h_n_tok, int batch, const void* sample_planes,
-                               const float* d_sample_scale, int64_t r_sample, float* row_stats, void* ws, size_t ws_bytes, sixdgs_stream_t stream) {
+int sixdgs_pack_h_planes(const void* planes, int64_t rows, void* h_planes, sixdgs_stream_t stream) {
+  SDG_CHECK_ARG(rows >= 0);
+  if (rows == 0) return 0;
+  SDG_CHECK_ARG(planes && h_planes && ((uintptr_t)planes % 16) == 0 && ((uintptr_t)h_planes % 16) == 0);
+  const int64_t blocks = sdg_cdiv(rows * (pp::kRowBytes / 16), 256);
+  hipLaunchKernelGGL(k_pack_h_planes, dim3((unsigned)(blocks < 16384 ? blocks : 16384)), dim3(256), 0, sdg_stream(stream), (const char*)planes, rows,
+                     (char*)h_planes);
+  SDG_LAUNCH_OK();
+  return 0;
+}
+
+static int select_sample_stats(const float* q, const int32_t* d_n_tok, const int32_t* h_n_tok, int batch, const void* sample_planes, const void* sample_h,
+                               const float* d_sample_scale, int64_t r_sample, float* row_stats, float log2_frac, float* ctok, float* gsum, void* ws,
+                               size_t ws_bytes, sixdgs_stream_t stream) {
   SDG_CHECK_ARG(batch >= 0 && batch <= 32767 && r_sample >= 1);
   if (batch == 0) return 0;
   SDG_CHECK_ARG(q && d_n_tok && sample_planes && d_sample_scale && row_stats && ws && ((uintptr_t)sample_planes % 16) == 0 &&
-                ((uintptr_t)q % 16) == 0 && ((uintptr_t)ws % 256) == 0);
+                ((uintptr_t)sample_h % 16) == 0 && ((uintptr_t)q % 16) == 0 && ((uintptr_t)ws % 256) == 0);
   hipStream_t s = sdg_stream(stream);
   SelectWs w;
   if (!select_ws(ws, ws_bytes, r_sample, batch, 1, 8, &w)) return SIXDGS_E_WORKSPACE;
   const int n_groups = f16x_groups(r_sample);
   for (const SweepSlots& T : sweep_pack(h_n_tok, batch, sweep_slot_cap())) {
     if (T.n_slots > 0) {
+      const bool h_only = sample_h != nullptr && prepass_one_term(T.n_slots) && prepass_fused_tail();
       hipLaunchKernelGGL(k_split_q_slots, dim3((unsigned)(4 * T.n_slots)), dim3(256), 0, s, q, d_n_tok, T, w.qplanes, w.qinv, (const float*)nullptr,
-                         (float*)nullptr, w.slot_rows);
-      LogitsF16Args V = select_args(w.slot_rows, T.n_slots, w, sample_planes, d_sample_scale, r_sample);
+                         (float*)nullptr, w.slot_rows, h_only ? 1 : 0, (unsigned*)nullptr, 0);
+      LogitsF16Args V = select_args(w.slot_rows, T.n_slots, w, h_only ? sample_h : sample_planes, d_sample_scale, r_sample);
       V.q_quarter_scales = 1;
       static const int reserve_env = [] { const char* e = getenv("SIXDGS_PREPASS_RESERVE_CUS"); return e ? atoi(e) : -2; }();
       const int reserve = reserve_env != -2 ? reserve_env : (T.n_slots == 1 ? kPrepassReserveCusOneSlot : kPrepassReserveCus);
@@ -2086,17 +2364,32 @@
         V.sib_sync = nullptr;
         V.sib_extra = 0u;
         V.sib_period = kSibPeriod;
-        if (prepass_one_term(T.n_slots)) hipLaunchKernelGGL((k_logits_f16x<kOneTerm, kOutStats, true>), dim3((unsigned)(V.n_sets * T.n_slots)), dim3(512), 0, s, V);
+        if (h_only) hipLaunchKernelGGL(k_prepass_h<true>, dim3((unsigned)(V.n_sets * T.n_slots)), dim3(512), 0, s, V);
+        else if (prepass_one_term(T.n_slots)) hipLaunchKernelGGL((k_logits_f16x<kOneTerm, kOutStats, true>), dim3((unsigned)(V.n_sets * T.n_slots)), dim3(512), 0, s, V);
         else hipLaunchKernelGGL((k_logits_f16x<kAllTerms, kOutStats, true>), dim3((unsigned)(V.n_sets * T.n_slots)), dim3(512), 0, s, V);
       } else {
-        if (prepass_one_term(T.n_slots)) hipLaunchKernelGGL((k_logits_f16x<kOneTerm, kOutStats>), dim3((unsigned)(V.n_groups * T.n_slots)), dim3(512), 0, s, V);
+        if (h_only) hipLaunchKernelGGL(k_prepass_h<false>, dim3((unsigned)(V.n_groups * T.n_slots)), dim3(512), 0, s, V);
+        else if (prepass_one_term(T.n_slots)) hipLaunchKernelGGL((k_logits_f16x<kOneTerm, kOutStats>), dim3((unsigned)(V.n_groups * T.n_slots)), dim3(512), 0, s, V);
         else hipLaunchKernelGGL((k_logits_f16x<kAllTerms, kOutStats>), dim3((unsigned)(V.n_groups * T.n_slots)), dim3(512), 0, s, V);
       }
     }
-    hipLaunchKernelGGL(k_merge_stats_slots, dim3((unsigned)T.n_images, 4), dim3(1024), 0, s, w.partial, n_groups, T, row_stats, (float*)nullptr);
+    hipLaunchKernelGGL(k_merge_stats_slots, dim3((unsigned)T.n_images, 4), dim3(1024), 0, s, w.partial, n_groups, T, row_stats, (float*)nullptr,
+                       (const int*)d_n_tok, log2_frac, ctok, gsum);
   }
   SDG_LAUNCH_OK();
   return 0;
+}
+
+int sixdgs_select_sample_stats_h(const float* q, const int32_t* d_n_tok, const int32_t* h_n_tok, int batch, const void* sample_planes,
+                                 const void* sample_h_planes, const float* d_sample_scale, int64_t r_sample, float* row_stats, void* ws, size_t ws_bytes,
+                                 sixdgs_stream_t stream) {
+  return select_sample_stats(q, d_n_tok, h_n_tok, batch, sample_planes, sample_h_planes, d_sample_scale, r_sample, row_stats, 0.f, nullptr, nullptr, ws,
+                             ws_bytes, stream);
+}
+
+int sixdgs_select_sample_stats(const float* q, const int32_t* d_n_tok, const int32_t* h_n_tok, int batch, const void* sample_planes,
+                               const float* d_sample_scale, int64_t r_sample, float* row_stats, void* ws, size_t ws_bytes, sixdgs_stream_t stream) {
+  return sixdgs_select_sample_stats_h(q, d_n_tok, h_n_tok, batch, sample_planes, nullptr, d_sample_scale, r_sample, row_stats, ws, ws_bytes, stream);
 }
 
 int sixdgs_select_prepare(const float* row_stats, const int32_t* d_n_tok, int batch, int64_t r_sample, int64_t r_total, float* ctok, float* gsum,
@@ -2112,16 +2405,25 @@
   return 0;
 }
 
-int sixdgs_select_begin(const float* q, const int32_t* d_n_tok, const int32_t* h_n_tok, int batch, const void* sample_planes, const float* d_sample_scale,
-                        int64_t r_sample, int64_t r_total, float* ctok, float* gsum, void* ws, size_t ws_bytes, sixdgs_stream_t stream) {
+int sixdgs_select_begin_h(const float* q, const int32_t* d_n_tok, const int32_t* h_n_tok, int batch, const void* sample_planes,
+                          const void* sample_h_planes, const float* d_sample_scale, int64_t r_sample, int64_t r_total, float* ctok, float* gsum, void* ws,
+                          size_t ws_bytes, sixdgs_stream_t stream) {
   SDG_CHECK_ARG(batch >= 0 && r_sample >= 1 && r_total >= r_sample);
   if (batch == 0) return 0;
-  SDG_CHECK_ARG(ws && ((uintptr_t)ws % 256) == 0);
+  SDG_CHECK_ARG(ws && ctok && gsum && ((uintptr_t)ws % 256) == 0);
   SelectWs w;
   if (!select_ws(ws, ws_bytes, r_sample, batch, 1, 8, &w)) return SIXDGS_E_WORKSPACE;
+  if (prepass_fused_tail())
+    return select_sample_stats(q, d_n_tok, h_n_tok, batch, sample_planes, sample_h_planes, d_sample_scale, r_sample, w.stats,
+                               log2f((float)((double)r_total / (double)r_sample)), ctok, gsum, ws, ws_bytes, stream);
   const int st = sixdgs_select_sample_stats(q, d_n_tok, h_n_tok, batch, sample_planes, d_sample_scale, r_sample, w.stats, ws, ws_bytes, stream);
   if (st) return st;
   return sixdgs_select_prepare(w.stats, d_n_tok, batch, r_sample, r_total, ctok, gsum, stream);
+}
+
+int sixdgs_select_begin(const float* q, const int32_t* d_n_tok, const int32_t* h_n_tok, int batch, const void* sample_planes, const float* d_sample_scale,
+                        int64_t r_sample, int64_t r_total, float* ctok, float* gsum, void* ws, size_t ws_bytes, sixdgs_stream_t stream) {
+  return sixdgs_select_begin_h(q, d_n_tok, h_n_tok, batch, sample_planes, nullptr, d_sample_scale, r_sample, r_total, ctok, gsum, ws, ws_bytes, stream);
 }
 
 int sixdgs_select_sweep(const float* q, const int32_t* d_n_tok, const int32_t* h_n_tok, int batch, const void* key_planes,
@@ -2140,7 +2442,6 @@
     double tok = 0.0;
     for (int k = 0; k < T.n_images; ++k) tok += h_n_tok ? (double)(h_n_tok[T.img[k]] < 0 ? 0 : (h_n_tok[T.img[k]] > kT ? kT : h_n_tok[T.img[k]])) : (double)kT;
     if (ns > 0) {
-      hipLaunchKernelGGL(k_split_q_slots, dim3((unsigned)(4 * ns)), dim3(256), 0, s, q, d_n_tok, T, w.qplanes, w.qinv, ctok, w.ctok_slot, w.slot_rows);
       LogitsF16Args V = select_args(w.slot_rows, ns, w, key_planes, d_key_scale, r);
       V.q_quarter_scales = 1;
       V.ctok = w.ctok_slot;
@@ -2153,15 +2454,19 @@
         V.sib_sync = sibling_sync_mode() == 2 ? nullptr : reinterpret_cast<unsigned*>(w.topk_ws);
         V.sib_extra = sibling_sync_mode() == 3 ? 1u : 0u;
         V.sib_period = kSibPeriod;
-        if (V.sib_sync && hipMemsetAsync(V.sib_sync, 0, (size_t)V.n_sets * sizeof(unsigned), s) != hipSuccess) return (int)hipGetLastError();
+        if (V.sib_sync && !prepass_fused_tail() && hipMemsetAsync(V.sib_sync, 0, (size_t)V.n_sets * sizeof(unsigned), s) != hipSuccess) return (int)hipGetLastError();
         grid = (unsigned)(V.n_sets * ns);
       }
+      const bool clear = V.sib_sync && prepass_fused_tail();
+      hipLaunchKernelGGL(k_split_q_slots, dim3((unsigned)(4 * ns)), dim3(256), 0, s, q, d_n_tok, T, w.qplanes, w.qinv, ctok, w.ctok_slot, w.slot_rows, 0,
+                         clear ? V.sib_sync : (unsigned*)nullptr, clear ? V.n_sets : 0);
       SdgProfileScope scope(prof, s, 2.0 * tok * SIXDGS_D * (double)r, (double)r * (kRowF + T.n_images * 16.0));
       auto kern = sweep_mfma16() ? (V.n_sets > 0 ? k_logits_f16x<kAllTerms, kOutUB, true, kMfma16> : k_logits_f16x<kAllTerms, kOutUB, false, kMfma16>)
                                  : (V.n_sets > 0 ? k_logits_f16x<kAllTerms, kOutUB, true> : k_logits_f16x<kAllTerms, kOutUB, false>);
       hipLaunchKernelGGL(kern, dim3(grid), dim3(512), 0, s, V);
     }
-    hipLaunchKernelGGL(k_merge_stats_slots, dim3((unsigned)T.n_images, 4), dim3(1024), 0, s, w.partial, n_groups, T, (float*)nullptr, gsum);
+    hipLaunchKernelGGL(k_merge_stats_slots, dim3((unsigned)T.n_images, 4), dim3(1024), 0, s, w.partial, n_groups, T, (float*)nullptr, gsum,
+                       (const int*)nullptr, 0.f, (float*)nullptr, (float*)nullptr);
     hipLaunchKernelGGL(k_sel_finish_slots, dim3((unsigned)sdg_cdiv(r, 1024), (unsigned)T.n_images), dim3(256), 0, s, w.ub, w.p.stride, u_stride, d_n_tok, T, r, u,
                        u_tile_max, u_stride / 256);
   }
@@ -2268,10 +2573,10 @@
                           sdg_align((size_t)max_candidates * sizeof(int64_t)) + 256);
 }
 
-int sixdgs_score_select(const float* q, const int32_t* d_n_tok, const int32_t* h_n_tok, int batch, const void* key_planes,
-                        const float* d_key_scale, const float* d_key_norm_max, int64_t r, const void* sample_planes, const float* d_sample_scale,
-                        int64_t r_sample, int topk, int max_candidates, int64_t* idx, float* val, int32_t* d_status, void* ws, size_t ws_bytes,
-                        sixdgs_stream_t stream, sixdgs_profile* prof) {
+int sixdgs_score_select_h(const float* q, const int32_t* d_n_tok, const int32_t* h_n_tok, int batch, const void* key_planes,
+                          const float* d_key_scale, const float* d_key_norm_max, int64_t r, const void* sample_planes, const void* sample_h_planes,
+                          const float* d_sample_scale, int64_t r_sample, int topk, int max_candidates, int64_t* idx, float* val, int32_t* d_status,
+                          void* ws, size_t ws_bytes, sixdgs_stream_t stream, sixdgs_profile* prof) {
   SDG_CHECK_ARG(r >= 1 && r_sample >= 1 && r_sample <= r && batch >= 0 && topk >= 1 && topk <= 1024 && max_candidates >= topk &&
                 max_candidates <= (1 << 20) && (max_candidates % 8) == 0);
   if (batch == 0) return 0;
@@ -2293,7 +2598,8 @@
     const int nb = (int)((batch - b0) < bg ? (batch - b0) : bg);
     const float* qg = q + (int64_t)b0 * kT * SIXDGS_D;
     const int32_t* ng = d_n_tok + b0;
-    int st = sixdgs_select_begin(qg, ng, h_n_tok ? h_n_tok + b0 : nullptr, nb, sample_planes, d_sample_scale, r_sample, r, ctok, gsum, ws, stage, stream);
+    int st = sixdgs_select_begin_h(qg, ng, h_n_tok ? h_n_tok + b0 : nullptr, nb, sample_planes, sample_h_planes, d_sample_scale, r_sample, r, ctok, gsum, ws,
+                                   stage, stream);
     if (st) return st;
     st = sixdgs_select_sweep(qg, ng, h_n_tok ? h_n_tok + b0 : nullptr, nb, key_planes, d_key_scale, r, ctok, gsum, u, (int64_t)stride, utm, ws, stage,
                              stream, prof);
@@ -2307,4 +2613,12 @@
   return 0;
 }
 
-}
+int sixdgs_score_select(const float* q, const int32_t* d_n_tok, const int32_t* h_n_tok, int batch, const void* key_planes,
+                        const float* d_key_scale, const float* d_key_norm_max, int64_t r, const void* sample_planes, const float* d_sample_scale,
+                        int64_t r_sample, int topk, int max_candidates, int64_t* idx, float* val, int32_t* d_status, void* ws, size_t ws_bytes,
+                        sixdgs_stream_t stream, sixdgs_profile* prof) {
+  return sixdgs_score_select_h(q, d_n_tok, h_n_tok, batch, key_planes, d_key_scale, d_key_norm_max, r, sample_planes, nullptr, d_sample_scale, r_sample, topk,
+                               max_candidates, idx, val, d_status, ws, ws_bytes, stream, prof);
+}
+
+}
diff --git a/6dgs_amd/identification_module.py b/6dgs_amd/identification_module.py
--- a/6dgs_amd/identification_module.py
+++ b/6dgs_amd/identification_module.py
@@ -124,7 +124,7 @@
             if planes_mode and r >= smin:
                 si = ops.select_sample_indices(r, rays_ori.device)
                 _, _, (s_planes, s_scale) = ops.ray_keys(rays_ori[si], rays_dir[si], rays_rgb[si], w, want_key=False, want_planes=True)
-                sample = (s_planes, s_scale)
+                sample = (s_planes, s_scale, ops.pack_h_planes(s_planes))
             self._key_cache, self._key_cache_id = {"key": key, "planes": planes, "scale": scale, "sample": sample, "norm": norm}, ident
             self._key_cache_rays = (rays_ori, rays_dir, rays_rgb)
         return self._key_cache
@@ -228,7 +228,7 @@
                 self._select_ws = sw = ops.big_empty(need, torch.uint8, q.device)
             idx, val, status = ops.score_select(q, n_tok, kc["planes"], kc["scale"], kc["sample"][0], kc["sample"][1], rays_to_output,
                                                 max_candidates=ops.SELECT_MAX_CANDIDATES, workspace=sw, profile=profile, n_tok_host=n_host,
-                                                key_norm=kc["norm"])
+                                                key_norm=kc["norm"], sample_h=kc["sample"][2])
             self.last_select_launches = ops.select_sweep_plan(n_host)
             self.last_scoring_path = "select"
             pend = dict(status=status, q=q, n_tok=n_tok, k=rays_to_output, workspace=workspace, images_in_flight=images_in_flight,
diff --git a/6dgs_amd/ops.py b/6dgs_amd/ops.py
--- a/6dgs_amd/ops.py
+++ b/6dgs_amd/ops.py
@@ -764,6 +764,25 @@
     return out
 
 
+H_PLANE_ROW_BYTES = 768
+
+
+@_on_device
+def pack_h_planes(planes: torch.Tensor) -> torch.Tensor:
+    _need_gpu(planes)
+    if planes.dim() != 2 or planes.shape[1] != 1536 or planes.dtype != torch.uint8 or not planes.is_contiguous():
+        raise RuntimeError("6dgs_amd: pack_h_planes needs contiguous scaled fp16 planes [R,1536] uint8 (MMA_F16X3)")
+    out = big_empty((planes.shape[0], H_PLANE_ROW_BYTES), torch.uint8, planes.device)
+    check(_lib.load().sixdgs_pack_h_planes(_p(planes), planes.shape[0], _p(out), _stream()), "pack_h_planes")
+    return out
+
+
+def _check_sample_h(sample_planes, sample_h):
+    if sample_h is not None and (sample_h.dim() != 2 or tuple(sample_h.shape) != (sample_planes.shape[0], H_PLANE_ROW_BYTES)
+                                 or sample_h.dtype != torch.uint8 or not sample_h.is_contiguous()):
+        raise RuntimeError(f"6dgs_amd: sample_h must be pack_h_planes(sample_planes): contiguous uint8 [{sample_planes.shape[0]},{H_PLANE_ROW_BYTES}]")
+
+
 def score_select_workspace_bytes(r: int, batch: int, topk: int = 100, max_candidates: int = SELECT_MAX_CANDIDATES) -> int:
     return int(_lib.load().sixdgs_score_select_workspace_bytes(int(r), int(batch), int(topk), int(max_candidates)))
 
@@ -784,9 +803,10 @@
 def score_select(q: torch.Tensor, n_tok: torch.Tensor, key_planes: torch.Tensor, key_scale: torch.Tensor, sample_planes: torch.Tensor,
                  sample_scale: torch.Tensor, topk: int = 100, max_candidates: int = SELECT_MAX_CANDIDATES,
                  workspace: Optional[torch.Tensor] = None, profile: Optional["KernelProfile"] = None, n_tok_host=None,
-                 key_norm: Optional[torch.Tensor] = None):
+                 key_norm: Optional[torch.Tensor] = None, sample_h: Optional[torch.Tensor] = None):
     q = _f32(q)
-    _need_gpu(q, n_tok, key_planes, key_scale, sample_planes, sample_scale, key_norm)
+    _need_gpu(q, n_tok, key_planes, key_scale, sample_planes, sample_scale, key_norm, sample_h)
+    _check_sample_h(sample_planes, sample_h)
     if key_norm is None:
         key_norm = key_norm_max(key_planes, key_scale)
     if key_planes.shape[1] != 1536 or sample_planes.shape[1] != 1536:
@@ -799,9 +819,9 @@
     if workspace is None:
         workspace = torch.empty(score_select_workspace_bytes(r, b, topk, max_candidates), dtype=torch.uint8, device=dev)
     h_n = (C.c_int32 * b)(*[int(v) for v in n_tok_host]) if n_tok_host is not None else None
-    check(lib.sixdgs_score_select(_p(q), _p(n_tok), h_n, b, _p(key_planes), _p(key_scale), _p(key_norm), r, _p(sample_planes), _p(sample_scale), rs,
-                                  int(topk), int(max_candidates), _p(idx), _p(val), _p(status), _p(workspace), workspace.numel(), _stream(),
-                                  profile.ref if profile is not None else None), "score_select")
+    check(lib.sixdgs_score_select_h(_p(q), _p(n_tok), h_n, b, _p(key_planes), _p(key_scale), _p(key_norm), r, _p(sample_planes), _p(sample_h),
+                                    _p(sample_scale), rs, int(topk), int(max_candidates), _p(idx), _p(val), _p(status), _p(workspace), workspace.numel(), _stream(),
+                                    profile.ref if profile is not None else None), "score_select")
     return idx, val, status
 
 
@@ -835,21 +855,23 @@
                        lib.sixdgs_select_candidates_workspace_bytes(self.r, self.b, self.topk, self.cmax)))
 
     @_on_device
-    def begin(self, sample_planes, sample_scale):
-        _need_gpu(self.q, sample_planes, sample_scale)
+    def begin(self, sample_planes, sample_scale, sample_h=None):
+        _need_gpu(self.q, sample_planes, sample_scale, sample_h)
+        _check_sample_h(sample_planes, sample_h)
         lib = _lib.load()
         self._grow(lib.sixdgs_select_workspace_bytes(sample_planes.shape[0], self.b, self.topk, self.cmax))
-        check(lib.sixdgs_select_begin(_p(self.q), _p(self.n_tok), self.h_n, self.b, _p(sample_planes), _p(sample_scale), sample_planes.shape[0], self.r,
-                                      _p(self.ctok), _p(self.gsum), _p(self.ws), self.ws.numel(), _stream()), "select_begin")
+        check(lib.sixdgs_select_begin_h(_p(self.q), _p(self.n_tok), self.h_n, self.b, _p(sample_planes), _p(sample_h), _p(sample_scale),
+                                        sample_planes.shape[0], self.r, _p(self.ctok), _p(self.gsum), _p(self.ws), self.ws.numel(), _stream()), "select_begin")
 
     @_on_device
-    def sample_stats(self, sample_planes, sample_scale) -> torch.Tensor:
-        _need_gpu(self.q, sample_planes, sample_scale)
+    def sample_stats(self, sample_planes, sample_scale, sample_h=None) -> torch.Tensor:
+        _need_gpu(self.q, sample_planes, sample_scale, sample_h)
+        _check_sample_h(sample_planes, sample_h)
         lib = _lib.load()
         self._grow(lib.sixdgs_select_workspace_bytes(sample_planes.shape[0], self.b, self.topk, self.cmax))
         stats = torch.empty(self.b, MAX_TOKENS, 2, device=self.dev)
-        check(lib.sixdgs_select_sample_stats(_p(self.q), _p(self.n_tok), self.h_n, self.b, _p(sample_planes), _p(sample_scale), sample_planes.shape[0],
-                                             _p(stats), _p(self.ws), self.ws.numel(), _stream()), "select_sample_stats")
+        check(lib.sixdgs_select_sample_stats_h(_p(self.q), _p(self.n_tok), self.h_n, self.b, _p(sample_planes), _p(sample_h), _p(sample_scale),
+                                               sample_planes.shape[0], _p(stats), _p(self.ws), self.ws.numel(), _stream()), "select_sample_stats")
         return stats
 
     @_on_device
diff --git a/include/sixdgs.h b/include/sixdgs.h
--- a/include/sixdgs.h
+++ b/include/sixdgs.h
@@ -214,6 +214,17 @@
                         const void* sample_planes, const float* d_sample_scale, int64_t r_sample, int topk, int max_candidates, int64_t* idx ,
                         float* val , int32_t* d_status , void* ws, size_t ws_bytes, sixdgs_stream_t stream,
                         sixdgs_profile* prof);
+int sixdgs_pack_h_planes(const void* planes , int64_t rows, void* h_planes , sixdgs_stream_t stream);
+int sixdgs_select_begin_h(const float* q, const int32_t* d_n_tok, const int32_t* h_n_tok, int batch, const void* sample_planes,
+                          const void* sample_h_planes , const float* d_sample_scale, int64_t r_sample, int64_t r_total, float* ctok, float* gsum,
+                          void* ws, size_t ws_bytes, sixdgs_stream_t stream);
+int sixdgs_select_sample_stats_h(const float* q, const int32_t* d_n_tok, const int32_t* h_n_tok, int batch, const void* sample_planes,
+                                 const void* sample_h_planes , const float* d_sample_scale, int64_t r_sample, float* row_stats ,
+                                 void* ws, size_t ws_bytes, sixdgs_stream_t stream);
+int sixdgs_score_select_h(const float* q, const int32_t* d_n_tok, const int32_t* h_n_tok, int batch, const void* key_planes, const float* d_key_scale,
+                          const float* d_key_norm_max, int64_t r, const void* sample_planes, const void* sample_h_planes ,
+                          const float* d_sample_scale, int64_t r_sample, int topk, int max_candidates, int64_t* idx, float* val, int32_t* d_status,
+                          void* ws, size_t ws_bytes, sixdgs_stream_t stream, sixdgs_profile* prof);
 size_t sixdgs_topk_workspace_bytes(int64_t r, int batch, int topk);
 int sixdgs_topk(const float* scores, int64_t r, int batch, int topk, int64_t* idx, float* val, void* ws,
                 size_t ws_bytes, sixdgs_stream_t stream);
```

Result: no change. 74.85, median of 6 (+0.3%).
